# ViTAE-Transformer/MTP

Hardware: AMD Instinct MI355X
Metric: images/sec pretrain step (ViT-L+RVSA, 224^2, bf16) (higher is better)
Workload: dtype bf16; 1 GPU; ViT-L + RVSA backbone fwd+bwd + grad all-reduce + clip + AdamW, 224x224, batch 64 per GPU (BASELINE configs[2]/[3]); global_batch=64, parallelism=dp1, activation_checkpointing=False, heads=sum_i mean(f_i)

## Files before the change

### include/mtp_hip.h

```cpp
#ifndef MTP_HIP_H_
#define MTP_HIP_H_

#include <stddef.h>
#include <stdint.h>

#ifdef __cplusplus
extern "C" {
#endif

typedef void* mtp_stream_t;

typedef enum { MTP_F32 = 0, MTP_BF16 = 1, MTP_F64 = 2  } mtp_dtype;

enum { MTP_OK = 0, MTP_ERR_ARG = -1, MTP_ERR_UNSUPPORTED = -2 };

typedef enum {
    MTP_EPI_BIAS = 0,
    MTP_EPI_BIAS_GELU = 1,
    MTP_EPI_BIAS_RES = 2,
    MTP_EPI_DGELU = 3,
    MTP_EPI_BIAS_GELU_DG = 4,
    MTP_EPI_MUL = 5
} mtp_epilogue;

typedef enum {
    MTP_GEMM_NT_REG_STAGED = 1,
    MTP_GEMM_ORDER_SHIFT = 1,
    MTP_GEMM_ORDER_PLAIN = 1 << 1,
    MTP_GEMM_ORDER_GROUPED = 2 << 1,
    MTP_GEMM_ORDER_ROW_MAJOR = 3 << 1,
    MTP_GEMM_ORDER_MASK = 3 << 1,
    MTP_GEMM_TNG_PLAIN_ORDER = 1 << 1,
    MTP_GEMM_TN_REG_TRANSPOSE = 1 << 4,
    MTP_GEMM_NT_SB8 = 1 << 5,
    MTP_GEMM_NT_NO_SB8 = 1 << 6,
    MTP_GEMM_NT_P8 = 1 << 8,
    MTP_GEMM_NT_P8_224 = 2 << 8,
    MTP_GEMM_NT_P8_256 = 3 << 8,
    MTP_GEMM_NT_P8_MASK = 3 << 8,
    MTP_GEMM_NT_NO_P8 = 1 << 10,
    MTP_GEMM_NT_PERSIST = 1 << 15,
    MTP_GEMM_TN_TR_FULL_ONLY = 1 << 15,
    MTP_GEMM_NT_NO_PERSIST = 1 << 16,
    MTP_GEMM_NT_STRIP = 1 << 17,
    MTP_GEMM_NT_NO_STRIP = 1 << 18,
    MTP_GEMM_TNG_PLAIN_PHASES = 1 << 19,
    MTP_GEMM_STORE_SHIFT = 20,
    MTP_GEMM_STORE_NT = 1 << 20,
    MTP_GEMM_STORE_SC1 = 2 << 20,
    MTP_GEMM_STORE_PLAIN = 3 << 20,
    MTP_GEMM_STORE_MASK = 3 << 20
} mtp_gemm_variant;

typedef struct {
    const void* A;
    const void* B;
    void* C;
    int64_t M, N, K;
    int64_t lda, ldb, ldc;
    int in_dtype;
    int out_dtype;
    int epilogue;
    const float* bias;
    int64_t bias_mod;
    const float* res;
    int64_t res_ld, res_mod;
    const float* rowscale;
    int64_t rows_per_sample;
    void* aux;
    int64_t aux_ld;
    int split_k;
    int variant;
    float* colsum;
    int defer_sum;
    int pad_;
    void* workspace;
    int64_t workspace_bytes;
} mtp_gemm_args;

int mtp_gemm_nt(const mtp_gemm_args* args, mtp_stream_t stream);
typedef enum {
    MTP_GEMM_NT_FAMILY_SB = 0,
    MTP_GEMM_NT_FAMILY_SB8 = 1,
    MTP_GEMM_NT_FAMILY_REG = 2,
    MTP_GEMM_NT_FAMILY_P8 = 3,
    MTP_GEMM_NT_FAMILY_STRIP = 4
} mtp_gemm_nt_family;
struct mtp_gemm_nt_plan {
    int family;
    int tile_m;
    int order;
    int persistent;
    int store_policy;
};
int mtp_gemm_nt_plan(const mtp_gemm_args* args, int cus, struct mtp_gemm_nt_plan* out);
int mtp_gemm_nt_tile(const mtp_gemm_args* args);
int64_t mtp_gemm_nt_workspace_bytes(void);
int mtp_gemm_tn(const mtp_gemm_args* args, mtp_stream_t stream);
#define MTP_MAX_GROUPED_GEMMS 32
int mtp_gemm_tn_grouped(const mtp_gemm_args* args, int count, mtp_stream_t stream);
int mtp_sum_partials_batch(const float* const* parts, float* const* outs, const int64_t* numel, const int* splits, int count,
                           mtp_stream_t stream);

int mtp_layernorm_fwd(const void* x, int x_dtype, const float* gamma, const float* beta, void* y, int y_dtype,
                      float* mean, float* rstd, int64_t rows, int64_t C, float eps, int fuse_gelu, mtp_stream_t stream);
int64_t mtp_layernorm_bwd_partial_rows(int64_t rows);
int mtp_layernorm_bwd(const void* dy, int dy_dtype, const void* x, int x_dtype, const float* mean, const float* rstd,
                      const float* gamma, const float* beta, int fuse_gelu,
                      const float* dres, const float* extra, void* dx, int dx_dtype,
                      void* dx_copy, int copy_dtype, const float* copy_scale, int64_t rows_per_sample,
                      float* dgamma_part, float* dbeta_part, int64_t part_ld, int64_t rows, int64_t C, mtp_stream_t stream);
int mtp_layernorm_bwd_win(const void* dy, int dy_dtype, const void* x, int x_dtype, const float* mean, const float* rstd,
                          const float* gamma, const float* dres, const float* extra, void* dx, int dx_dtype,
                          void* dx_copy, int copy_dtype, const float* copy_scale, int64_t rows_per_sample,
                          float* dgamma_part, float* dbeta_part, int64_t part_ld, int64_t rows, int64_t C,
                          const float* win_add, int64_t B, int64_t Hp, int64_t Wp, mtp_stream_t stream);
int mtp_layernorm_residual_fwd(const void* h, int dtype, const float* gamma, const float* beta, const float* x, const float* layer_scale,
                               const float* sample_scale, int64_t rows_per_sample, float* out, void* out_act, float* mean, float* rstd,
                               int64_t rows, int64_t C, float eps, mtp_stream_t stream);
int mtp_layernorm_residual_bwd(const float* dout, const void* h, int dtype, const float* mean, const float* rstd, const float* gamma, const float* beta,
                               const float* layer_scale, const float* sample_scale, int64_t rows_per_sample, void* dh, float* part,
                               int64_t rows, int64_t C, mtp_stream_t stream);
int mtp_reduce_rows_f32(const float* part, int64_t ld, float* out, int64_t rows, int64_t C, int accumulate, mtp_stream_t stream);
#define MTP_REDUCE_BATCH_MAX 32
int mtp_reduce_rows_batched_f32(const float* const* parts, float* const* outs, int n, int64_t ld, int64_t rows, int64_t C, int accumulate,
                                mtp_stream_t stream);
int mtp_reduce_rows_t_f32(const float* part, int64_t ld, float* out, int64_t rows, int64_t R, int64_t C, int accumulate, mtp_stream_t stream);
int mtp_reduce_rows_t_batched_f32(const float* const* parts, float* const* outs, int n, int64_t ld, int64_t rows, int64_t R, int64_t C, int accumulate,
                                  mtp_stream_t stream);
int mtp_colsum(const void* dY, int dtype, int64_t ld, float* out, int64_t M, int64_t N, mtp_stream_t stream);
int mtp_colsum_acc(const void* dY, int dtype, int64_t ld, float* out, int64_t M, int64_t N, mtp_stream_t stream);

int mtp_patchify(const float* img, void* cols, int dtype, int64_t B, int64_t Cin, int64_t H, int64_t W, int64_t P, mtp_stream_t stream);
int mtp_unpatchify(const void* cols, int dtype, float* dimg, int64_t B, int64_t Cin, int64_t H, int64_t W, int64_t P, mtp_stream_t stream);
int mtp_preprocess_patchify(const uint8_t* img, void* cols, int dtype, int64_t B, int64_t H, int64_t W, int64_t P, int64_t pad_divisor,
                            const float* mean, const float* std, int bgr_to_rgb, float pad_value, mtp_stream_t stream);
int mtp_cast(const void* src, int src_dtype, void* dst, int dst_dtype, int64_t n, mtp_stream_t stream);
int mtp_transpose_cast(const float* src, void* dst, int dst_dtype, int64_t R, int64_t C, mtp_stream_t stream);
typedef struct {
    const float* src;
    void* w;
    void* wt;
    int64_t R, C;
    int64_t tile0;
    int32_t f32_out;
    float wd;
} mtp_wimg_desc;
int mtp_weight_images(const mtp_wimg_desc* descs_dev, int n, int64_t total_tiles, int act_dtype, mtp_stream_t stream);
int mtp_adamw_weight_images(const mtp_wimg_desc* descs_dev, int n, int64_t total_tiles, int act_dtype, float* p_base, const float* g_base, float* m_base, float* v_base,
                            const float* hyper, const float* sqnorm, float max_norm, float grad_scale, mtp_stream_t stream);
int mtp_adamw_weight_images_lr(const mtp_wimg_desc* descs_dev, const float* desc_lr, int n, int64_t total_tiles, int act_dtype, float* p_base, const float* g_base,
                               float* m_base, float* v_base, const float* hyper, const float* sqnorm, float max_norm, float grad_scale, mtp_stream_t stream);
int mtp_convt_pack(const float* w, void* wg, void* wgT, int dtype, int64_t Cin, int64_t Cout, mtp_stream_t stream);
int mtp_convt_unpack_grad(const float* dwg, float* dw, int64_t Cin, int64_t Cout, mtp_stream_t stream);
int mtp_tokens_to_nchw(const void* x, int x_dtype, void* out, int out_dtype, int64_t B, int64_t Hp, int64_t Wp, int64_t C, int levels, mtp_stream_t stream);
int mtp_nchw_to_tokens(const void* f, int f_dtype, void* out, int out_dtype, int64_t B, int64_t Hp, int64_t Wp, int64_t C, int levels, mtp_stream_t stream);
int mtp_maxpool2_tokens_fwd(const float* x, void* y, int y_dtype, int64_t B, int64_t Hp, int64_t Wp, int64_t C, mtp_stream_t stream);
int mtp_maxpool2_tokens_bwd(const float* x, const void* dy, int dy_dtype, float* dx, int accumulate, int64_t B, int64_t Hp, int64_t Wp, int64_t C, mtp_stream_t stream);
int mtp_axpy_f32(float* y, const float* x, float alpha, int64_t n, mtp_stream_t stream);
#define MTP_MAX_SEGMENTS 12
int mtp_copy_segments_f32(const float* const* src, float* const* dst, const int64_t* count, int n, mtp_stream_t stream);
int mtp_scale_rows_cast(const float* src, void* dst, int dst_dtype, const float* scale, int64_t rows_per_sample, int64_t rows, int64_t C, mtp_stream_t stream);

int mtp_im2col3x3(const void* x, int x_dtype, int64_t sN, int64_t sH, int64_t sW, int64_t sC, void* cols, int cols_dtype,
                  int64_t N, int64_t H, int64_t W, int64_t Cin, int64_t stride, int64_t Kp, mtp_stream_t stream);
int mtp_col2im3x3(const void* dcols, int cols_dtype, float* dx, int64_t sN, int64_t sH, int64_t sW, int64_t sC,
                  int64_t N, int64_t H, int64_t W, int64_t Cin, int64_t stride, int64_t Kp, int accumulate, mtp_stream_t stream);
int mtp_conv3x3_pack(const float* w, void* w2, void* w2t, int dtype, int64_t Cout, int64_t Cin, int64_t Kp, mtp_stream_t stream);
int mtp_conv3x3_unpack_grad(const float* dw2, float* dw, int64_t Cout, int64_t Cin, int64_t Kp, mtp_stream_t stream);
int mtp_pack_rows_padded(const float* w, void* wp, void* wpt, int dtype, int64_t R, int64_t C, int64_t Rp, mtp_stream_t stream);
int mtp_cast_pad_rows(const float* src, int64_t n, void* dst, int dst_dtype, int64_t ld, int64_t rows, mtp_stream_t stream);
int mtp_copy_rows(const void* src, int64_t src_ld, void* dst, int64_t dst_ld, int dtype, int64_t n, int64_t rows, mtp_stream_t stream);
int mtp_dwconv3x3_fwd(const void* x, const float* w, const float* bias, void* y, int dtype, int64_t N, int64_t H, int64_t W, int64_t C, mtp_stream_t stream);
int mtp_dwconv3x3_bwd_dx(const void* dy, int dtype, const float* w, float* dx, int accumulate, int64_t N, int64_t H, int64_t W, int64_t C, mtp_stream_t stream);
int64_t mtp_dwconv3x3_bwd_dw_partial_rows(int64_t N, int64_t H, int64_t W);
int mtp_dwconv3x3_bwd_dw(const void* dy, const void* x, int dtype, float* part, int64_t N, int64_t H, int64_t W, int64_t C, mtp_stream_t stream);
typedef enum { MTP_CONV_OP_IM2COL3X3 = 0, MTP_CONV_OP_COL2IM3X3 = 1, MTP_CONV_OP_DWCONV3X3_FWD = 2, MTP_CONV_OP_DWCONV3X3_BWD_DX = 3, MTP_CONV_OP_DWCONV3X3_BWD_DW = 4 } mtp_conv_op;
typedef enum {
    MTP_CONV_KERNEL_NONE = 0,
    MTP_CONV_KERNEL_ELEMENT = 1,
    MTP_CONV_KERNEL_V8 = 2,
    MTP_CONV_KERNEL_P8 = 3,
    MTP_CONV_KERNEL_PX4 = 4
} mtp_conv_kernel_family;
int mtp_conv_kernel(int op, const void* src, int src_dtype, int64_t sN, int64_t sH, int64_t sW, int64_t sC, const void* dst, int dst_dtype,
                    const float* w, const float* bias, int64_t N, int64_t H, int64_t W, int64_t C, int64_t stride, int64_t Kp);
int mtp_dwconv_fwd(const void* x, const float* w, const float* bias, void* y, int dtype, int64_t N, int64_t H, int64_t W, int64_t C, int k, mtp_stream_t stream);
int mtp_dwconv_bwd_dx(const void* dy, int dtype, const float* w, float* dx, int accumulate, int64_t N, int64_t H, int64_t W, int64_t C, int k, mtp_stream_t stream);
int mtp_dwconv_bwd_dw(const void* dy, const void* x, int dtype, float* dw, float* db, int64_t N, int64_t H, int64_t W, int64_t C, int k, mtp_stream_t stream);
int mtp_center_feature_scale_fwd(const void* y, const void* xp, const void* logits, int64_t ld, void* out, int dtype, int64_t rows, int64_t G, int64_t GC, mtp_stream_t stream);
int mtp_center_feature_scale_bwd(const void* dout, const void* y, const void* xp, const void* logits, int64_t ld, void* dy, float* dxp, void* dlogits, int dtype, int64_t rows,
                                 int64_t G, int64_t GC, mtp_stream_t stream);
int mtp_softmax_groups_fwd(const void* logits, int64_t ld, void* prob, int dtype, int64_t rows, int64_t G, int64_t P, mtp_stream_t stream);
int mtp_softmax_groups_bwd(const void* prob, const float* dprob, void* dlogits, int64_t ld, int dtype, int64_t rows, int64_t G, int64_t P, mtp_stream_t stream);
int mtp_scale_residual_fwd(const float* x, const void* z, int dtype, const float* gamma, const float* sample_scale, int64_t rows_per_sample,
                           float* out, void* out_act, int64_t rows, int64_t C, mtp_stream_t stream);
int64_t mtp_scale_residual_bwd_partial_rows(int64_t rows);
int mtp_scale_residual_bwd(const float* dout, const void* z, int dtype, const float* gamma, const float* sample_scale, int64_t rows_per_sample,
                           void* dz, float* part, int64_t rows, int64_t C, mtp_stream_t stream);

int mtp_full_attn_fwd(const void* qkv, void* o, float* lse, int dtype, const float* rel_h, const float* rel_w,
                      int64_t B, int64_t Hp, int64_t Wp, int64_t heads, int64_t hd, float scale, mtp_stream_t stream);
int64_t mtp_full_attn_bwd_workspace_floats(int64_t B, int64_t Hp, int64_t Wp, int64_t heads);
int mtp_full_attn_bwd(const void* qkv, const void* o, const void* dout, const float* lse, void* dqkv, int dtype,
                      const float* rel_h, const float* rel_w, float* drel_part, float* workspace,
                      int64_t B, int64_t Hp, int64_t Wp, int64_t heads, int64_t hd, float scale, mtp_stream_t stream);

enum {
    MTP_ATTN_KERNEL_NONE = 0,
    MTP_FULL_FWD_V3 = 1,
    MTP_FULL_FWD_FLASH128 = 3,
    MTP_FULL_FWD_FLASH256 = 4,
    MTP_FULL_FWD_GENERIC = 5,
    MTP_FULL_BWD_V3 = 1,
    MTP_FULL_BWD_FLASH = 3,
    MTP_FULL_BWD_THREE_PASS = 4,
    MTP_FULL_BWD_SINGLE_WG = 5,
    MTP_RVSA_FWD_GENERIC = 1,
    MTP_RVSA_FWD_MFMA = 2,
    MTP_RVSA_BWD_GENERIC = 1,
    MTP_RVSA_BWD_MFMA_DENSE = 2,
    MTP_RVSA_BWD_MFMA_ATOMIC = 3
};
int mtp_full_attn_kernel(int dtype, int64_t Hp, int64_t Wp, int backward);
int mtp_rvsa_attn_kernel(int dtype, int64_t Hp, int64_t Wp, int64_t heads, int backward);

int mtp_rvsa_pool_fwd(const void* x, int dtype, float* avg, float* pooled, int64_t B, int64_t Hp, int64_t Wp, int64_t C, mtp_stream_t stream);
int mtp_rvsa_pool_bwd(const float* dpooled, const float* avg, void* dx, int dtype, int accumulate, int64_t B, int64_t Hp, int64_t Wp, int64_t C, mtp_stream_t stream);
int mtp_rvsa_sampling_fwd(const void* x, int dtype, const float* w, const float* bias, float* avg, float* pooled, float* samp,
                          int64_t B, int64_t Hp, int64_t Wp, int64_t C, int64_t N, mtp_stream_t stream);
int mtp_rvsa_sampling_bwd(const float* dsamp, const float* w, const float* avg, void* dx, int dtype,
                          int64_t B, int64_t Hp, int64_t Wp, int64_t C, int64_t N, mtp_stream_t stream);
int mtp_rvsa_sampling_bwd_win(const float* dsamp, const float* w, const float* avg, float* g, int64_t windows, int64_t C, int64_t N, mtp_stream_t stream);
int mtp_small_linear_fwd(const float* x, const float* w, const float* b, float* y, int64_t R, int64_t N, int64_t K, mtp_stream_t stream);
int mtp_small_linear_bwd(const float* x, const float* w, const float* dy, float* dx, float* dw, float* db, int64_t R, int64_t N, int64_t K, mtp_stream_t stream);
int mtp_small_linear_dw_segments(const float* x, const float* dy, int64_t R, int64_t N, int64_t K, int nseg, const int64_t* seg_rows,
                                 float* const* dw, float* const* db, mtp_stream_t stream);
int mtp_small_linear_dw_segments_batched(const float* const* xs, const float* const* dys, int count, int64_t R, int64_t N, int64_t K, int nseg,
                                         const int64_t* seg_rows, float* const* dw, float* const* db, mtp_stream_t stream);
int mtp_rvsa_attn_fwd(const void* qkv, const float* samp, void* o, float* lse, int dtype,
                      const float* rel_h, const float* rel_w, const float* bias_table,
                      int64_t B, int64_t Hp, int64_t Wp, int64_t heads, int64_t hd, float scale, mtp_stream_t stream);
int mtp_rvsa_attn_bwd(const void* qkv, const float* samp, const void* o, const void* dout, const float* lse,
                      void* dqkv, float* dkv_f32, float* dsamp, float* rel_part, float* tab_part, int dtype,
                      const float* rel_h, const float* rel_w, const float* bias_table,
                      int64_t B, int64_t Hp, int64_t Wp, int64_t heads, int64_t hd, float scale, mtp_stream_t stream);

int mtp_zero_segments_f32(float* base, const int64_t* start, const int64_t* count, int n, mtp_stream_t stream);
int mtp_sqnorm_f32(const float* g, float* out, int64_t n, mtp_stream_t stream);
int mtp_sqnorm_segments_f32(const float* base, const int64_t* start, const int64_t* count, int n, float* out, mtp_stream_t stream);
int mtp_adamw_flat(float* p, const float* g, float* m, float* v, int64_t n, const int64_t* seg_start, const float* seg_wd, int nseg,
                   const float* hyper, const float* sqnorm, float max_norm, float grad_scale, mtp_stream_t stream);
int mtp_adamw_flat_lr(float* p, const float* g, float* m, float* v, int64_t n, const int64_t* seg_start, const float* seg_wd, const float* seg_lr, int nseg,
                      const float* hyper, const float* sqnorm, float max_norm, float grad_scale, mtp_stream_t stream);

typedef struct {
    int64_t N, H, W;
    int kernel_h, kernel_w, stride_h, stride_w, pad_h, pad_w, dilation_h, dilation_w;
    int group, group_channels;
    float offset_scale;
    int im2col_step;
    int remove_center;
    int variant;
} mtp_dcnv3_geom;
int mtp_dcnv3_out_size(const mtp_dcnv3_geom* geom, int64_t* Ho, int64_t* Wo);
int mtp_dcnv3_fwd(const void* input, const void* offset, const void* mask, void* output, int dtype, const mtp_dcnv3_geom* geom, mtp_stream_t stream);
int mtp_dcnv3_bwd(const void* input, const void* offset, const void* mask, const void* grad_output, int dtype, float* grad_input, float* grad_offset,
                  float* grad_mask, const mtp_dcnv3_geom* geom, mtp_stream_t stream);
int mtp_dcnv3_bwd_act(const void* input, const void* offset, const void* mask, const void* grad_output, int dtype, float* grad_input, float* grad_offset,
                      float* grad_mask, void* grad_offset_act, int64_t act_ld, const mtp_dcnv3_geom* geom, mtp_stream_t stream);

typedef enum {
    MTP_DCNV3_KERNEL_NONE = 0,
    MTP_DCNV3_FWD9 = 1,
    MTP_DCNV3_FWD_VEC8 = 2,
    MTP_DCNV3_FWD_SCALAR = 3,
    MTP_DCNV3_F64 = 4,
    MTP_DCNV3_BWD_WINDOW_R2 = 5,
    MTP_DCNV3_BWD_WINDOW_R3 = 6,
    MTP_DCNV3_BWD_3X3_OS1 = 7,
    MTP_DCNV3_BWD_3X3_OS2 = 8,
    MTP_DCNV3_BWD_SCATTER_SHFL = 9,
    MTP_DCNV3_BWD_SCATTER_ATOMIC = 10
} mtp_dcnv3_kernel_family;
int mtp_dcnv3_kernel(const void* input, const void* offset, const void* mask, const void* out, const float* grad_input, const float* grad_offset,
                     const float* grad_mask, int dtype, const mtp_dcnv3_geom* geom, int backward);

const char* mtp_version(void);

int mtp_stream_create_low_priority(mtp_stream_t* stream);
int mtp_stream_create_cu_mask(const uint32_t* mask, int words, mtp_stream_t* stream);
int mtp_probe_placement(int32_t* out, int blocks, int64_t spin_clocks, mtp_stream_t stream);
int mtp_stream_destroy(mtp_stream_t stream);

int mtp_comm_unique_id(void* id128);
int mtp_comm_init(const void* id128, int rank, int world, void** comm);
int mtp_comm_allreduce_bucket(void* comm, float* bucket, int64_t count, mtp_stream_t stream);
int mtp_comm_allreduce_bucket_dt(void* comm, void* bucket, int64_t count, int dtype, mtp_stream_t stream);
int mtp_comm_reduce_scatter_bucket(void* comm, void* bucket, int64_t count_per_rank, int rank, int dtype, mtp_stream_t stream);
int mtp_comm_allgather_bucket(void* comm, void* bucket, int64_t count_per_rank, int rank, int dtype, mtp_stream_t stream);
int mtp_comm_info(void* comm, int* info4);
int mtp_comm_destroy(void* comm);

int64_t mtp_bn_partial_rows(int64_t rows);
int mtp_bn_stats(const void* x, int dtype, int64_t ldx, const float* center, float* part, float* sums, int64_t rows, int64_t C, mtp_stream_t stream);
int mtp_bn_finalize(const float* sums, const float* center, double count, float* running_mean, float* running_var, float momentum, float eps, float* mean, float* rstd,
                    int64_t C, mtp_stream_t stream);
int mtp_bn_apply(const void* x, int x_dtype, int64_t ldx, const float* mean, const float* rstd, const float* gamma, const float* beta, int relu,
                 void* y, int y_dtype, int64_t ldy, int64_t rows, int64_t C, mtp_stream_t stream);
int mtp_bn_bwd_stats(const void* dy, int dy_dtype, int64_t lddy, const void* x, int x_dtype, int64_t ldx, const float* mean, const float* rstd,
                     const float* gamma, const float* beta, int relu, float* part, float* sums, int64_t rows, int64_t C, mtp_stream_t stream);
int mtp_bn_bwd_dx(const void* dy, int dy_dtype, int64_t lddy, const void* x, int x_dtype, int64_t ldx, const float* mean, const float* rstd,
                  const float* gamma, const float* beta, int relu, const float* sums, double count, void* dx, int dx_dtype, int64_t lddx,
                  int64_t rows, int64_t C, mtp_stream_t stream);
int mtp_resize_bilinear_fwd(const void* x, int x_dtype, int64_t ldx, void* y, int y_dtype, int64_t ldy, int64_t N, int64_t Hi, int64_t Wi,
                            int64_t Ho, int64_t Wo, int64_t C, int accumulate, mtp_stream_t stream);
int mtp_resize_bilinear_bwd(const void* dy, int dy_dtype, int64_t lddy, float* dx, int64_t lddx, int64_t N, int64_t Hi, int64_t Wi, int64_t Ho,
                            int64_t Wo, int64_t C, int accumulate, mtp_stream_t stream);
int mtp_adaptive_avg_pool_fwd(const void* x, int x_dtype, int64_t ldx, void* y, int y_dtype, int64_t N, int64_t H, int64_t W, int64_t C,
                              int64_t S, mtp_stream_t stream);
int mtp_adaptive_avg_pool_bwd(const void* dy, int dy_dtype, float* dx, int64_t lddx, int64_t N, int64_t H, int64_t W, int64_t C, int64_t S,
                              int accumulate, mtp_stream_t stream);
int mtp_channel_scale(const void* x, int x_dtype, int64_t ldx, const float* mask, int64_t rows_per_sample, void* y, int y_dtype, int64_t ldy,
                      int64_t rows, int64_t C, mtp_stream_t stream);
int64_t mtp_seg_ce_workspace_bytes(int64_t N, int64_t H, int64_t W, int64_t K);
int mtp_seg_ce(const void* logits, int dtype, int64_t ld, int64_t N, int64_t h, int64_t w, int64_t K, const void* labels, int label_bytes, int64_t H,
               int64_t W, int ignore_index, float loss_weight, float* loss, float* dlogits, int64_t ldd, void* workspace, int64_t workspace_bytes,
               mtp_stream_t stream);

int mtp_seg_window_accumulate(const void* logits, int dtype, int64_t ld, int64_t N, int64_t h, int64_t w, int64_t K, float* acc, int64_t lda,
                              int64_t H, int64_t W, int64_t y1, int64_t x1, int64_t Hc, int64_t Wc, mtp_stream_t stream);
int mtp_seg_argmax_areas(float* acc, int64_t lda, int64_t N, int64_t H, int64_t W, int64_t K, const int32_t* cy, const int32_t* cx, int write_back,
                         uint8_t* pred, float* seg_logits, const void* labels, int label_bytes, int ignore_index, int64_t* areas, mtp_stream_t stream);
int mtp_seg_areas(const void* pred, int pred_bytes, const void* labels, int label_bytes, int64_t pixels, int64_t K, int ignore_index, int64_t* areas,
                  mtp_stream_t stream);

typedef enum { MTP_FUSE_CONCAT = 0, MTP_FUSE_SUM = 1, MTP_FUSE_DIFF = 2, MTP_FUSE_ABS_DIFF = 3 } mtp_fuse_policy;
int mtp_fuse_pair_fwd(const void* f, int f_dtype, void* out, int out_dtype, int64_t ld, int64_t N, int64_t C, int64_t H, int64_t W, int policy,
                      mtp_stream_t stream);
int mtp_fuse_pair_bwd(const float* g, int64_t ldg, const void* f, int f_dtype, float* df, int64_t N, int64_t C, int64_t H, int64_t W, int policy,
                      mtp_stream_t stream);
int mtp_unet_up_cat_fwd(const void* x, int64_t ldx, int64_t Cx, const void* skip, int64_t lds, int64_t Cs, int in_dtype, void* y, int y_dtype, int64_t ldy,
                        int64_t N, int64_t h, int64_t w, int64_t hs, int64_t ws, mtp_stream_t stream);
int mtp_unet_up_cat_bwd(const float* dy, int64_t lddy, float* dx, int64_t lddx, int64_t Cx, float* dskip, int64_t ldds, int64_t Cs, int64_t N, int64_t h,
                        int64_t w, int64_t hs, int64_t ws, int accumulate, mtp_stream_t stream);

int mtp_gap_fwd(const void* x, int dtype, float* pooled, int64_t N, int64_t C, int64_t HW, mtp_stream_t stream);
int mtp_gap_bwd(const float* dpooled, void* dx, int dtype, int64_t N, int64_t C, int64_t HW, mtp_stream_t stream);
int mtp_cls_ce(const float* pooled, const float* w, const float* b, const int64_t* labels, float loss_weight, float* logits, float* prob,
               int64_t* pred, float* loss_rows, float* loss, float* dlogits, uint32_t* counter, int64_t N, int64_t C, int64_t K, mtp_stream_t stream);
int mtp_cls_head_bwd(const float* dlogits, const float* pooled, const float* w, float* dw, float* db, float* dpooled, int64_t N, int64_t C, int64_t K,
                     int accumulate, mtp_stream_t stream);
int mtp_cls_hits(const float* scores, const int64_t* labels, int64_t N, int64_t K, const int32_t* topk, int nk, float thr, int use_thr,
                 int64_t* counters, mtp_stream_t stream);

typedef enum { MTP_BOX_ALIGNED = 0 , MTP_BOX_ROTATED = 1  } mtp_box_kind;
typedef enum {
    MTP_ASSIGN_BOX = 0,
    MTP_ASSIGN_RBOX2HBOX = 1,
    MTP_ASSIGN_ROTATED = 2
} mtp_assign_calculator;
int mtp_box_iou(const float* boxes1, const float* boxes2, float* out, int64_t M, int64_t N, int kind, int iof, int aligned, float eps,
                mtp_stream_t stream);
int mtp_nms_mask(const float* boxes, const int64_t* groups, int64_t n, int kind, float iou_threshold, void* mask, int64_t mask_bytes,
                 mtp_stream_t stream);
int mtp_nms_scan(const void* mask, int64_t n, int64_t max_keep, int64_t* keep, int64_t* count, mtp_stream_t stream);
int mtp_max_iou_assign(const float* gts, const float* priors, const int64_t* gt_labels, int64_t K, int64_t N, int calculator, float pos_iou_thr,
                       float neg_iou_lo, float neg_iou_hi, float min_pos_iou, int match_low_quality, int gt_max_assign_all, int64_t* gt_inds,
                       float* max_overlaps, int64_t* labels, void* workspace, int64_t workspace_bytes, mtp_stream_t stream);

#ifdef __cplusplus
}
#endif
#endif
```

### mtp_amd/__init__.py

```python
import os as _os

_HWQ_BEFORE_IMPORT = _os.environ.get("GPU_MAX_HW_QUEUES")
_os.environ.setdefault("GPU_MAX_HW_QUEUES", "8")


def _hip_already_initialised():
    try:
        import torch as _torch
        return bool(_torch.cuda.is_initialized())
    except Exception:
        return False


_HIP_INIT_BEFORE_IMPORT = _hip_already_initialised()
_warned_hwq = False


def hw_queue_note():
    global _warned_hwq
    if _warned_hwq:
        return None
    val = _os.environ.get("GPU_MAX_HW_QUEUES")
    note = None
    if _HIP_INIT_BEFORE_IMPORT and _HWQ_BEFORE_IMPORT is None:
        note = ("HIP was initialised before `import mtp_amd`: GPU_MAX_HW_QUEUES=8 could not take effect, the weight-gradient side stream may share the "
                "compute stream's hardware queue (no overlap, nothing wrong); import mtp_amd or set GPU_MAX_HW_QUEUES=8 before the first CUDA call")
    elif val is not None and val.isdigit() and int(val) < 8:
        note = ("GPU_MAX_HW_QUEUES=%s (set by the environment): with fewer than 8 hardware queues the weight-gradient side stream may share the compute "
                "stream's queue next to the gradient exchange (no overlap, nothing wrong)" % val)
    _warned_hwq = True
    return note

from .backbone import (InternImage, internimage_xl, RVSA_MTP, RVSA_MTP_branches, RVSA_MTP_det, RVSA_MTP_taps, ViT_Win_RVSA_V3_WSZ7, vit_b_rvsa, vit_l_rvsa,
                       window_partition, window_reverse)
from .registry import BACKBONES, MODELS, TASK_UTILS, build_backbone
from .decode_heads import UNetHead, UPerHead
from .necks import FeatureFusionNeck, GlobalAveragePooling
from .cls_heads import LinearClsHead
from .classifiers import ImageClassifier
from .segmentors import EncoderDecoder, SiamEncoderDecoder
from .evaluation import Accuracy, IoUMetric
from .ops_box import batched_nms, bbox_overlaps, box_iou_rotated, nms, nms_rotated
from .task_modules import AssignResult, BboxOverlaps2D, MTP_RD_MaxIoUAssigner, MaxIoUAssigner, RBbox2HBboxOverlaps2D, RBboxOverlaps2D

__version__ = "0.6.0"
```

### mtp_amd/_lib.py

```python
import ctypes as C
import os

_HERE = os.path.dirname(os.path.abspath(__file__))
LIB_PATH = os.environ.get("MTP_HIP_LIB") or os.path.join(_HERE, "libmtp_hip.so")

MTP_F32, MTP_BF16, MTP_F64 = 0, 1, 2
EPI_BIAS, EPI_BIAS_GELU, EPI_BIAS_RES, EPI_DGELU, EPI_BIAS_GELU_DG, EPI_MUL = 0, 1, 2, 3, 4, 5

GEMM_NT_REG_STAGED = 1
GEMM_ORDER_SHIFT, GEMM_ORDER_PLAIN, GEMM_ORDER_GROUPED, GEMM_ORDER_ROW_MAJOR, GEMM_ORDER_MASK = 1, 1 << 1, 2 << 1, 3 << 1, 3 << 1
GEMM_TNG_PLAIN_ORDER = 1 << 1
GEMM_TN_REG_TRANSPOSE = 1 << 4
GEMM_NT_SB8, GEMM_NT_NO_SB8 = 1 << 5, 1 << 6
GEMM_NT_P8, GEMM_NT_P8_224, GEMM_NT_P8_256, GEMM_NT_P8_MASK, GEMM_NT_NO_P8 = 1 << 8, 2 << 8, 3 << 8, 3 << 8, 1 << 10
GEMM_NT_PERSIST, GEMM_TN_TR_FULL_ONLY, GEMM_NT_NO_PERSIST = 1 << 15, 1 << 15, 1 << 16
GEMM_NT_STRIP, GEMM_NT_NO_STRIP = 1 << 17, 1 << 18
GEMM_TNG_PLAIN_PHASES = 1 << 19
GEMM_STORE_SHIFT, GEMM_STORE_NT, GEMM_STORE_SC1, GEMM_STORE_PLAIN, GEMM_STORE_MASK = 20, 1 << 20, 2 << 20, 3 << 20, 3 << 20
GEMM_NT_FAMILY_SB, GEMM_NT_FAMILY_SB8, GEMM_NT_FAMILY_REG, GEMM_NT_FAMILY_P8, GEMM_NT_FAMILY_STRIP = 0, 1, 2, 3, 4

CONV_OP_IM2COL3X3, CONV_OP_COL2IM3X3, CONV_OP_DWCONV3X3_FWD, CONV_OP_DWCONV3X3_BWD_DX, CONV_OP_DWCONV3X3_BWD_DW = 0, 1, 2, 3, 4
CONV_KERNEL_NONE, CONV_KERNEL_ELEMENT, CONV_KERNEL_V8, CONV_KERNEL_P8, CONV_KERNEL_PX4 = 0, 1, 2, 3, 4
DCNV3_KERNEL_NONE, DCNV3_FWD9, DCNV3_FWD_VEC8, DCNV3_FWD_SCALAR, DCNV3_F64 = 0, 1, 2, 3, 4
DCNV3_BWD_WINDOW_R2, DCNV3_BWD_WINDOW_R3, DCNV3_BWD_3X3_OS1, DCNV3_BWD_3X3_OS2, DCNV3_BWD_SCATTER_SHFL, DCNV3_BWD_SCATTER_ATOMIC = 5, 6, 7, 8, 9, 10

BOX_ALIGNED, BOX_ROTATED = 0, 1
ASSIGN_BOX, ASSIGN_RBOX2HBOX, ASSIGN_ROTATED = 0, 1, 2

FUSE_CONCAT, FUSE_SUM, FUSE_DIFF, FUSE_ABS_DIFF = 0, 1, 2, 3

p, i64, i32, f32 = C.c_void_p, C.c_int64, C.c_int, C.c_float


class GemmArgs(C.Structure):
    _fields_ = [("A", p), ("B", p), ("C", p), ("M", i64), ("N", i64), ("K", i64),
                ("lda", i64), ("ldb", i64), ("ldc", i64),
                ("in_dtype", i32), ("out_dtype", i32), ("epilogue", i32),
                ("bias", p), ("bias_mod", i64), ("res", p), ("res_ld", i64), ("res_mod", i64),
                ("rowscale", p), ("rows_per_sample", i64), ("aux", p), ("aux_ld", i64),
                ("split_k", i32), ("variant", i32), ("colsum", p), ("defer_sum", i32), ("pad_", i32),
                ("workspace", p), ("workspace_bytes", i64)]


class GemmNtPlan(C.Structure):
    _fields_ = [("family", i32), ("tile_m", i32), ("order", i32), ("persistent", i32), ("store_policy", i32)]


class WimgDesc(C.Structure):
    _fields_ = [("src", p), ("w", p), ("wt", p), ("R", i64), ("C", i64), ("tile0", i64), ("f32_out", C.c_int32), ("wd", C.c_float)]


class Dcnv3Geom(C.Structure):
    _fields_ = [("N", i64), ("H", i64), ("W", i64), ("kernel_h", C.c_int32), ("kernel_w", C.c_int32), ("stride_h", C.c_int32), ("stride_w", C.c_int32),
                ("pad_h", C.c_int32), ("pad_w", C.c_int32), ("dilation_h", C.c_int32), ("dilation_w", C.c_int32), ("group", C.c_int32),
                ("group_channels", C.c_int32), ("offset_scale", C.c_float), ("im2col_step", C.c_int32), ("remove_center", C.c_int32), ("variant", C.c_int32)]


SIGNATURES = {
    "mtp_weight_images": (i32, [p, i32, i64, i32, p]),
    "mtp_dwconv_fwd": (i32, [p, p, p, p, i32, i64, i64, i64, i64, i32, p]),
    "mtp_dwconv_bwd_dx": (i32, [p, i32, p, p, i32, i64, i64, i64, i64, i32, p]),
    "mtp_dwconv_bwd_dw": (i32, [p, p, i32, p, p, i64, i64, i64, i64, i32, p]),
    "mtp_center_feature_scale_fwd": (i32, [p, p, p, i64, p, i32, i64, i64, i64, p]),
    "mtp_center_feature_scale_bwd": (i32, [p, p, p, p, i64, p, p, p, i32, i64, i64, i64, p]),
    "mtp_dcnv3_out_size": (i32, [C.POINTER(Dcnv3Geom), C.POINTER(i64), C.POINTER(i64)]),
    "mtp_dcnv3_fwd": (i32, [p, p, p, p, i32, C.POINTER(Dcnv3Geom), p]),
    "mtp_dcnv3_bwd": (i32, [p, p, p, p, i32, p, p, p, C.POINTER(Dcnv3Geom), p]),
    "mtp_dcnv3_bwd_act": (i32, [p, p, p, p, i32, p, p, p, p, i64, C.POINTER(Dcnv3Geom), p]),
    "mtp_dcnv3_kernel": (i32, [p, p, p, p, p, p, p, i32, C.POINTER(Dcnv3Geom), i32]),
    "mtp_conv_kernel": (i32, [i32, p, i32, i64, i64, i64, i64, p, i32, p, p, i64, i64, i64, i64, i64, i64]),
    "mtp_gemm_nt": (i32, [C.POINTER(GemmArgs), p]),
    "mtp_gemm_nt_plan": (i32, [C.POINTER(GemmArgs), i32, C.POINTER(GemmNtPlan)]),
    "mtp_gemm_nt_tile": (i32, [C.POINTER(GemmArgs)]),
    "mtp_gemm_nt_workspace_bytes": (i64, []),
    "mtp_gemm_tn": (i32, [C.POINTER(GemmArgs), p]),
    "mtp_gemm_tn_grouped": (i32, [C.POINTER(GemmArgs), i32, p]),
    "mtp_sum_partials_batch": (i32, [p, p, p, p, i32, p]),
    "mtp_layernorm_fwd": (i32, [p, i32, p, p, p, i32, p, p, i64, i64, f32, i32, p]),
    "mtp_layernorm_bwd_partial_rows": (i64, [i64]),
    "mtp_layernorm_bwd": (i32, [p, i32, p, i32, p, p, p, p, i32, p, p, p, i32, p, i32, p, i64, p, p, i64, i64, i64, p]),
    "mtp_reduce_rows_f32": (i32, [p, i64, p, i64, i64, i32, p]),
    "mtp_reduce_rows_batched_f32": (i32, [p, p, i32, i64, i64, i64, i32, p]),
    "mtp_reduce_rows_t_f32": (i32, [p, i64, p, i64, i64, i64, i32, p]),
    "mtp_reduce_rows_t_batched_f32": (i32, [p, p, i32, i64, i64, i64, i64, i32, p]),
    "mtp_copy_segments_f32": (i32, [p, p, p, i32, p]),
    "mtp_colsum": (i32, [p, i32, i64, p, i64, i64, p]),
    "mtp_colsum_acc": (i32, [p, i32, i64, p, i64, i64, p]),
    "mtp_patchify": (i32, [p, p, i32, i64, i64, i64, i64, i64, p]),
    "mtp_preprocess_patchify": (i32, [p, p, i32, i64, i64, i64, i64, i64, C.POINTER(f32), C.POINTER(f32), i32, f32, p]),
    "mtp_unpatchify": (i32, [p, i32, p, i64, i64, i64, i64, i64, p]),
    "mtp_cast": (i32, [p, i32, p, i32, i64, p]),
    "mtp_transpose_cast": (i32, [p, p, i32, i64, i64, p]),
    "mtp_convt_pack": (i32, [p, p, p, i32, i64, i64, p]),
    "mtp_convt_unpack_grad": (i32, [p, p, i64, i64, p]),
    "mtp_tokens_to_nchw": (i32, [p, i32, p, i32, i64, i64, i64, i64, i32, p]),
    "mtp_nchw_to_tokens": (i32, [p, i32, p, i32, i64, i64, i64, i64, i32, p]),
    "mtp_maxpool2_tokens_fwd": (i32, [p, p, i32, i64, i64, i64, i64, p]),
    "mtp_maxpool2_tokens_bwd": (i32, [p, p, i32, p, i32, i64, i64, i64, i64, p]),
    "mtp_axpy_f32": (i32, [p, p, f32, i64, p]),
    "mtp_scale_rows_cast": (i32, [p, p, i32, p, i64, i64, i64, p]),
    "mtp_im2col3x3": (i32, [p, i32, i64, i64, i64, i64, p, i32, i64, i64, i64, i64, i64, i64, p]),
    "mtp_col2im3x3": (i32, [p, i32, p, i64, i64, i64, i64, i64, i64, i64, i64, i64, i64, i32, p]),
    "mtp_conv3x3_pack": (i32, [p, p, p, i32, i64, i64, i64, p]),
    "mtp_conv3x3_unpack_grad": (i32, [p, p, i64, i64, i64, p]),
    "mtp_pack_rows_padded": (i32, [p, p, p, i32, i64, i64, i64, p]),
    "mtp_cast_pad_rows": (i32, [p, i64, p, i32, i64, i64, p]),
    "mtp_copy_rows": (i32, [p, i64, p, i64, i32, i64, i64, p]),
    "mtp_dwconv3x3_fwd": (i32, [p, p, p, p, i32, i64, i64, i64, i64, p]),
    "mtp_dwconv3x3_bwd_dx": (i32, [p, i32, p, p, i32, i64, i64, i64, i64, p]),
    "mtp_dwconv3x3_bwd_dw_partial_rows": (i64, [i64, i64, i64]),
    "mtp_dwconv3x3_bwd_dw": (i32, [p, p, i32, p, i64, i64, i64, i64, p]),
    "mtp_softmax_groups_fwd": (i32, [p, i64, p, i32, i64, i64, i64, p]),
    "mtp_softmax_groups_bwd": (i32, [p, p, p, i64, i32, i64, i64, i64, p]),
    "mtp_scale_residual_fwd": (i32, [p, p, i32, p, p, i64, p, p, i64, i64, p]),
    "mtp_scale_residual_bwd_partial_rows": (i64, [i64]),
    "mtp_scale_residual_bwd": (i32, [p, p, i32, p, p, i64, p, p, i64, i64, p]),
    "mtp_comm_unique_id": (i32, [p]),
    "mtp_comm_init": (i32, [p, i32, i32, C.POINTER(C.c_void_p)]),
    "mtp_comm_allreduce_bucket": (i32, [p, p, i64, p]),
    "mtp_comm_allreduce_bucket_dt": (i32, [p, p, i64, i32, p]),
    "mtp_comm_reduce_scatter_bucket": (i32, [p, p, i64, i32, i32, p]),
    "mtp_comm_allgather_bucket": (i32, [p, p, i64, i32, i32, p]),
    "mtp_comm_info": (i32, [p, p]),
    "mtp_comm_destroy": (i32, [p]),
    "mtp_full_attn_fwd": (i32, [p, p, p, i32, p, p, i64, i64, i64, i64, i64, f32, p]),
    "mtp_full_attn_bwd_workspace_floats": (i64, [i64, i64, i64, i64]),
    "mtp_full_attn_bwd": (i32, [p, p, p, p, p, i32, p, p, p, p, i64, i64, i64, i64, i64, f32, p]),
    "mtp_full_attn_kernel": (i32, [i32, i64, i64, i32]),
    "mtp_rvsa_attn_kernel": (i32, [i32, i64, i64, i64, i32]),
    "mtp_rvsa_pool_fwd": (i32, [p, i32, p, p, i64, i64, i64, i64, p]),
    "mtp_rvsa_pool_bwd": (i32, [p, p, p, i32, i32, i64, i64, i64, i64, p]),
    "mtp_rvsa_sampling_fwd": (i32, [p, i32, p, p, p, p, p, i64, i64, i64, i64, i64, p]),
    "mtp_rvsa_sampling_bwd": (i32, [p, p, p, p, i32, i64, i64, i64, i64, i64, p]),
    "mtp_rvsa_sampling_bwd_win": (i32, [p, p, p, p, i64, i64, i64, p]),
    "mtp_layernorm_residual_fwd": (i32, [p, i32, p, p, p, p, p, i64, p, p, p, p, i64, i64, f32, p]),
    "mtp_layernorm_residual_bwd": (i32, [p, p, i32, p, p, p, p, p, p, i64, p, p, i64, i64, p]),
    "mtp_layernorm_bwd_win": (i32, [p, i32, p, i32, p, p, p, p, p, p, i32, p, i32, p, i64, p, p, i64, i64, i64, p, i64, i64, i64, p]),
    "mtp_small_linear_fwd": (i32, [p, p, p, p, i64, i64, i64, p]),
    "mtp_small_linear_bwd": (i32, [p, p, p, p, p, p, i64, i64, i64, p]),
    "mtp_small_linear_dw_segments": (i32, [p, p, i64, i64, i64, i32, p, p, p, p]),
    "mtp_small_linear_dw_segments_batched": (i32, [p, p, i32, i64, i64, i64, i32, p, p, p, p]),
    "mtp_rvsa_attn_fwd": (i32, [p, p, p, p, i32, p, p, p, i64, i64, i64, i64, i64, f32, p]),
    "mtp_rvsa_attn_bwd": (i32, [p, p, p, p, p, p, p, p, p, p, i32, p, p, p, i64, i64, i64, i64, i64, f32, p]),
    "mtp_zero_segments_f32": (i32, [p, p, p, i32, p]),
    "mtp_sqnorm_f32": (i32, [p, p, i64, p]),
    "mtp_sqnorm_segments_f32": (i32, [p, p, p, i32, p, p]),
    "mtp_adamw_flat": (i32, [p, p, p, p, i64, p, p, i32, p, p, f32, f32, p]),
    "mtp_adamw_weight_images": (i32, [p, i32, i64, i32, p, p, p, p, p, p, f32, f32, p]),
    "mtp_adamw_flat_lr": (i32, [p, p, p, p, i64, p, p, p, i32, p, p, f32, f32, p]),
    "mtp_adamw_weight_images_lr": (i32, [p, p, i32, i64, i32, p, p, p, p, p, p, f32, f32, p]),
    "mtp_bn_partial_rows": (i64, [i64]),
    "mtp_bn_stats": (i32, [p, i32, i64, p, p, p, i64, i64, p]),
    "mtp_bn_finalize": (i32, [p, p, C.c_double, p, p, f32, f32, p, p, i64, p]),
    "mtp_bn_apply": (i32, [p, i32, i64, p, p, p, p, i32, p, i32, i64, i64, i64, p]),
    "mtp_bn_bwd_stats": (i32, [p, i32, i64, p, i32, i64, p, p, p, p, i32, p, p, i64, i64, p]),
    "mtp_bn_bwd_dx": (i32, [p, i32, i64, p, i32, i64, p, p, p, p, i32, p, C.c_double, p, i32, i64, i64, i64, p]),
    "mtp_resize_bilinear_fwd": (i32, [p, i32, i64, p, i32, i64, i64, i64, i64, i64, i64, i64, i32, p]),
    "mtp_resize_bilinear_bwd": (i32, [p, i32, i64, p, i64, i64, i64, i64, i64, i64, i64, i32, p]),
    "mtp_adaptive_avg_pool_fwd": (i32, [p, i32, i64, p, i32, i64, i64, i64, i64, i64, p]),
    "mtp_adaptive_avg_pool_bwd": (i32, [p, i32, p, i64, i64, i64, i64, i64, i64, i32, p]),
    "mtp_channel_scale": (i32, [p, i32, i64, p, i64, p, i32, i64, i64, i64, p]),
    "mtp_seg_ce_workspace_bytes": (i64, [i64, i64, i64, i64]),
    "mtp_seg_ce": (i32, [p, i32, i64, i64, i64, i64, i64, p, i32, i64, i64, i32, f32, p, p, i64, p, i64, p]),
    "mtp_seg_window_accumulate": (i32, [p, i32, i64, i64, i64, i64, i64, p, i64, i64, i64, i64, i64, i64, i64, p]),
    "mtp_seg_argmax_areas": (i32, [p, i64, i64, i64, i64, i64, p, p, i32, p, p, p, i32, i32, p, p]),
    "mtp_seg_areas": (i32, [p, i32, p, i32, i64, i64, i32, p, p]),
    "mtp_fuse_pair_fwd": (i32, [p, i32, p, i32, i64, i64, i64, i64, i64, i32, p]),
    "mtp_fuse_pair_bwd": (i32, [p, i64, p, i32, p, i64, i64, i64, i64, i32, p]),
    "mtp_unet_up_cat_fwd": (i32, [p, i64, i64, p, i64, i64, i32, p, i32, i64, i64, i64, i64, i64, i64, p]),
    "mtp_unet_up_cat_bwd": (i32, [p, i64, p, i64, i64, p, i64, i64, i64, i64, i64, i64, i64, i32, p]),
    "mtp_gap_fwd": (i32, [p, i32, p, i64, i64, i64, p]),
    "mtp_gap_bwd": (i32, [p, p, i32, i64, i64, i64, p]),
    "mtp_cls_ce": (i32, [p, p, p, p, f32, p, p, p, p, p, p, p, i64, i64, i64, p]),
    "mtp_cls_head_bwd": (i32, [p, p, p, p, p, p, i64, i64, i64, i32, p]),
    "mtp_cls_hits": (i32, [p, p, i64, i64, C.POINTER(C.c_int32), i32, f32, i32, p, p]),
    "mtp_box_iou": (i32, [p, p, p, i64, i64, i32, i32, i32, f32, p]),
    "mtp_nms_mask": (i32, [p, p, i64, i32, f32, p, i64, p]),
    "mtp_nms_scan": (i32, [p, i64, i64, p, p, p]),
    "mtp_max_iou_assign": (i32, [p, p, p, i64, i64, i32, f32, f32, f32, f32, i32, i32, p, p, p, p, i64, p]),
    "mtp_version": (C.c_char_p, []),
    "mtp_stream_create_low_priority": (i32, [p]),
    "mtp_stream_create_cu_mask": (i32, [p, i32, p]),
    "mtp_probe_placement": (i32, [p, i32, i64, p]),
    "mtp_stream_destroy": (i32, [p]),
}

_lib = None


class MtpHipError(RuntimeError):
    pass


def load():
    global _lib
    if _lib is not None:
        return _lib
    if not os.path.exists(LIB_PATH):
        raise MtpHipError("libmtp_hip.so not found at %s -- build it first (__graft_entry__.build() or make -C mtp_amd/csrc); "
                          "mtp_amd has no CPU/PyTorch fallback" % LIB_PATH)
    lib = C.CDLL(LIB_PATH)
    ab = bool(os.environ.get("MTP_HIP_LIB"))
    for name, (res, args) in SIGNATURES.items():
        if ab and not hasattr(lib, name):
            continue
        fn = getattr(lib, name)
        fn.restype = res
        fn.argtypes = args
    _lib = lib
    return lib


def check(rc, what):
    if rc != 0:
        kind = {-1: "invalid argument", -2: "unsupported configuration"}.get(rc, "hipError_t %d" % rc)
        raise MtpHipError("%s failed: %s" % (what, kind))
```

### mtp_amd/csrc/gemm.hip

```cpp
#include "gemm_common.h"

namespace {

constexpr int BM = 128;
constexpr int BN = 128;
constexpr int NT_THREADS = 256;
constexpr int ROW_BYTES = 128;
constexpr int OPER_BYTES = BM * ROW_BYTES;
constexpr int STAGE_BYTES = 2 * OPER_BYTES;
constexpr int LDS_BYTES = 2 * STAGE_BYTES;

__device__ __forceinline__ int lds_off(int row, int chunk) { return row * ROW_BYTES + ((chunk ^ (row & 7)) << 4); }

__global__ __launch_bounds__(256) void sum_partials_kernel(const float* __restrict__ part, float* __restrict__ out, int64_t n4, int split) {
    for (int64_t i = (int64_t)blockIdx.x * 256 + threadIdx.x; i < n4; i += (int64_t)gridDim.x * 256) {
        float4 s = *reinterpret_cast<const float4*>(part + 4 * i);
        for (int z = 1; z < split; ++z) {
            const float4 v = *reinterpret_cast<const float4*>(part + 4 * (i + (int64_t)z * n4));
            s.x += v.x; s.y += v.y; s.z += v.z; s.w += v.w;
        }
        *reinterpret_cast<float4*>(out + 4 * i) = s;
    }
}

// ... 320 lines not shown
        __builtin_amdgcn_sched_barrier(0);
        compute_stage<T>(cur, cur + OPER_BYTES, acc, wm, wn, lane);
        __builtin_amdgcn_sched_barrier(0);
        store_tn_regs<T>(r, nxt, tid);
    }
    epilogue<float, MTP_EPI_BIAS, 4>(p, acc, m0 + wm * 64, n0 + wn * 64, lane);
}

typedef short tr_v4s __attribute__((ext_vector_type(4)));
constexpr int TR_ROW_BYTES = 256;

__device__ __forceinline__ void stage_tn_glds(const KArgs& p, char* sA, char* sB, int m0, int n0, int kt, int wave, int lane) {
#pragma unroll
    for (int i = 0; i < 4; ++i) {
        const int rbase = wave * 16 + i * 4;
        const int row = rbase + (lane >> 4);
        const int f = (row & 3) | ((row >> 1) & 4);
        const int chunk = (lane & 15) ^ (f << 1);
        const int64_t t = (int64_t)kt * 64 + row;
        int ca = m0 + chunk * 8, cb = n0 + chunk * 8;
        ca = ca < p.M - 8 ? ca : p.M - 8;
        cb = cb < p.N - 8 ? cb : p.N - 8;
        const char* ga = p.A + (t * p.lda + ca) * 2;
        const char* gb = p.B + (t * p.ldb + cb) * 2;
        __builtin_amdgcn_global_load_lds((const __attribute__((address_space(1))) void*)ga,
                                         (__attribute__((address_space(3))) void*)(sA + rbase * TR_ROW_BYTES), 16, 0, 0);
        __builtin_amdgcn_global_load_lds((const __attribute__((address_space(1))) void*)gb,
                                         (__attribute__((address_space(3))) void*)(sB + rbase * TR_ROW_BYTES), 16, 0, 0);
    }
}

__device__ __forceinline__ uint4 tr_frag(const char* s, int off) {
    const tr_v4s lo = __builtin_amdgcn_ds_read_tr16_b64_v4i16((__attribute__((address_space(3))) tr_v4s*)(s + off));
    const tr_v4s hi = __builtin_amdgcn_ds_read_tr16_b64_v4i16((__attribute__((address_space(3))) tr_v4s*)(s + off + 4 * TR_ROW_BYTES));
    const uint2 l = __builtin_bit_cast(uint2, lo), h = __builtin_bit_cast(uint2, hi);
    return make_uint4(l.x, l.y, h.x, h.y);
}

__device__ __forceinline__ void compute_stage_tr(const char* sA, const char* sB, f32x4_t (&acc)[4][4], int wm, int wn, int lane) {
    const int i = lane & 15, g = lane >> 4;
    const int f = (i >> 2) | ((g & 1) << 2);
    const int rowoff = (8 * g + (i >> 2)) * TR_ROW_BYTES + ((i >> 1) & 1) * 16 + (i & 1) * 8;
#pragma unroll
    for (int ks = 0; ks < 2; ++ks) {
        uint4 a[4], b[4];
#pragma unroll
        for (int q = 0; q < 4; ++q) {
            a[q] = tr_frag(sA, rowoff + (((q | (wm << 2)) ^ f) << 5) + ks * 32 * TR_ROW_BYTES);
            b[q] = tr_frag(sB, rowoff + (((q | (wn << 2)) ^ f) << 5) + ks * 32 * TR_ROW_BYTES);
        }
#pragma unroll
        for (int ni = 0; ni < 4; ++ni)
#pragma unroll
            for (int mi = 0; mi < 4; ++mi) Mma<bf16_t>::run(acc[ni][mi], b[ni], a[mi]);
    }
}

__global__ __launch_bounds__(NT_THREADS) __attribute__((amdgpu_waves_per_eu(4, 4))) void gemm_tn_tr_kernel(KArgs p) {
    extern __shared__ __attribute__((aligned(16))) char smem[];
    const int tid = threadIdx.x, lane = tid & 63, wave = __builtin_amdgcn_readfirstlane(tid >> 6);
    const int wm = wave >> 1, wn = wave & 1;
    const int tile = (p.order & 1) ? (int)blockIdx.x : xcd_remap(blockIdx.x, gridDim.x);
    const int tiles_m = (int)gridDim.x / p.tiles_n;
    const int m0 = ((p.order & 2) ? tile % tiles_m : tile / p.tiles_n) * BM, n0 = ((p.order & 2) ? tile / tiles_m : tile % p.tiles_n) * BN;
    const int kt0 = blockIdx.y * p.k_tiles_per_split;
    int kt1 = kt0 + p.k_tiles_per_split;
    kt1 = kt1 < p.k_tiles ? kt1 : p.k_tiles;
    if (kt0 >= kt1) return;
    p.C += (int64_t)blockIdx.y * p.split_stride * (int64_t)sizeof(float);
    f32x4_t acc[4][4];
#pragma unroll
    for (int i = 0; i < 4; ++i)
#pragma unroll
        for (int j = 0; j < 4; ++j) acc[i][j] = f32x4_t{0.f, 0.f, 0.f, 0.f};
    const bool do_colsum = p.colsum != nullptr && n0 == 0;
    float cs[8] = {0.f, 0.f, 0.f, 0.f, 0.f, 0.f, 0.f, 0.f};
    for (int kt = kt0; kt < kt1; ++kt) {
        stage_tn_glds(p, smem, smem + OPER_BYTES, m0, n0, kt, wave, lane);
        asm volatile("s_waitcnt vmcnt(0)" ::: "memory");
        __syncthreads();
        compute_stage_tr(smem, smem + OPER_BYTES, acc, wm, wn, lane);
        if (do_colsum) {
#pragma unroll
            for (int j = 0; j < 4; ++j) {
                const uint4 v = *reinterpret_cast<const uint4*>(smem + ((tid >> 4) + 16 * j) * TR_ROW_BYTES + (tid & 15) * 16);
                const uint32_t w[4] = {v.x, v.y, v.z, v.w};
#pragma unroll
                for (int e = 0; e < 4; ++e) {
                    cs[2 * e] += __uint_as_float(w[e] << 16);
                    cs[2 * e + 1] += __uint_as_float(w[e] & 0xffff0000u);
                }
            }
        }
        __syncthreads();
    }
    if (do_colsum) {
        float* red = reinterpret_cast<float*>(smem);
        const int rg = tid >> 4, f = (rg & 3) | ((rg >> 1) & 4), chunk = (tid & 15) ^ (f << 1);
        *reinterpret_cast<float4*>(red + rg * BM + chunk * 8) = make_float4(cs[0], cs[1], cs[2], cs[3]);
        *reinterpret_cast<float4*>(red + rg * BM + chunk * 8 + 4) = make_float4(cs[4], cs[5], cs[6], cs[7]);
        __syncthreads();
        if (tid < BM) {
            float s = 0.f;
#pragma unroll
            for (int r = 0; r < 16; ++r) s += red[r * BM + tid];
            if (m0 + tid < p.M) atomicAdd(p.colsum + m0 + tid, s);
        }
    }
    epilogue<float, MTP_EPI_BIAS, 4>(p, acc, m0 + wm * 64, n0 + wn * 64, lane);
}

template <typename T>
int fill_common(const mtp_gemm_args* a, KArgs& k) {
    constexpr int E = Elem<T>::kPerChunk;
    if (!a->A || !a->B || !a->C || a->M <= 0 || a->N <= 0 || a->K <= 0) return MTP_ERR_ARG;
    if (a->M > INT32_MAX || a->N > INT32_MAX || a->K > INT32_MAX) return MTP_ERR_ARG;
    if ((a->lda % E) || (a->ldb % E) || (a->ldc % 4) || (a->N % 4)) return MTP_ERR_ARG;
    if (((uintptr_t)a->A | (uintptr_t)a->B | (uintptr_t)a->C) & 15) return MTP_ERR_ARG;
    k.A = (const char*)a->A; k.B = (const char*)a->B; k.C = (char*)a->C;
    k.M = (int)a->M; k.N = (int)a->N; k.K = (int)a->K;
    k.lda = a->lda; k.ldb = a->ldb; k.ldc = a->ldc;
    k.bias = a->bias; k.bias_mod = (int)a->bias_mod;
    k.res = a->res; k.res_ld = a->res_ld; k.res_mod = (int)a->res_mod;
    k.rowscale = a->rowscale; k.rows_per_sample = (int)(a->rows_per_sample > 0 ? a->rows_per_sample : 1);
    k.aux = (char*)a->aux; k.aux_ld = a->aux_ld;
    k.tiles_n = (int)((a->N + BN - 1) / BN);
    k.k_tiles = (int)((a->K + 8 * E - 1) / (8 * E));
    k.k_tiles_per_split = k.k_tiles;
    k.atomic_out = 0;
    k.order = 0;
    k.split_stride = 0;
    k.colsum = nullptr;
    return 0;
}

NtPlan nt_plan(const mtp_gemm_args* a, const KArgs& k, int cus) {
    const int ord = (a->variant & MTP_GEMM_ORDER_MASK) >> MTP_GEMM_ORDER_SHIFT;
    const int p8_forced = (a->variant & MTP_GEMM_NT_P8_MASK) / MTP_GEMM_NT_P8;
    const int sp_forced = (a->variant & MTP_GEMM_STORE_MASK) >> MTP_GEMM_STORE_SHIFT;
    const bool reg_staged = a->variant & MTP_GEMM_NT_REG_STAGED, sb8_force = a->variant & MTP_GEMM_NT_SB8, sb8_forbid = a->variant & MTP_GEMM_NT_NO_SB8;
    const bool p8_forbid = a->variant & MTP_GEMM_NT_NO_P8, persist_force = a->variant & MTP_GEMM_NT_PERSIST, persist_forbid = a->variant & MTP_GEMM_NT_NO_PERSIST;
    const bool s8_force = a->variant & MTP_GEMM_NT_STRIP, s8_forbid = a->variant & MTP_GEMM_NT_NO_STRIP;

    const bool bf16 = a->in_dtype == MTP_BF16;
    const int64_t tiles = ((a->M + 255) / 256) * ((a->N + 255) / 256) * 256 / cus;
    NtPlan p = {MTP_GEMM_NT_FAMILY_SB, BM, 0, 0, MTP_GEMM_STORE_PLAIN >> MTP_GEMM_STORE_SHIFT};

    if (bf16 && !p8_forbid && !s8_forbid && !p8_forced && mtp_nt_s8_fits(k, a->out_dtype, a->epilogue) && (s8_force || (tiles >= 40 && tiles <= 128))) {
        p.family = MTP_GEMM_NT_FAMILY_STRIP;
        p.order = ord == 1;
        p.persistent = 1;
        p.store_policy = mtp_nt_s8_store_policy(a->out_dtype);
        return p;
    }
    if (bf16 && !p8_forbid && mtp_nt_p8_fits(k, a->out_dtype, a->epilogue) && (p8_forced || tiles >= 72 || (tiles >= 40 && a->K >= 1536))) {
        p.family = MTP_GEMM_NT_FAMILY_P8;
        p.tile_m = p8_forced == 2 ? 224 : p8_forced == 3 ? 256 : mtp_nt_p8_pick_tile_m(k.M, k.N, cus);
        p.order = ord == 1;
        p.persistent = persist_force || (!persist_forbid && p.tile_m == 224 && mtp_nt_p8_tiles(k.M, k.N, p.tile_m) > cus);
        const int sp = sp_forced ? sp_forced : (a->epilogue == MTP_EPI_BIAS_RES ? 2 : 1);
        if (p.tile_m == 224) p.store_policy = sp;
        return p;
    }
    if (reg_staged || a->K % (8 * (bf16 ? 8 : 4))) {
        p.family = MTP_GEMM_NT_FAMILY_REG;
        p.order = ord;
        return p;
    }
    p.order = ord == 0 ? (k.tiles_n > 8 ? 2 : 0) : ord == 1 ? 1 : ord == 2 ? 2 : 0;
    const int tiles8 = ((k.M + NT8_BM - 1) / NT8_BM) * k.tiles_n;
    if (sb8_force || (tiles8 >= 256 && tiles8 <= 512 && !sb8_forbid)) {
        p.family = MTP_GEMM_NT_FAMILY_SB8;
        p.tile_m = NT8_BM;
    }
    return p;
}

template <typename T, typename Tout, int EPI>
int launch_nt(const mtp_gemm_args* a, hipStream_t stream) {
    constexpr int E = Elem<T>::kPerChunk;
    KArgs k;
    int rc = fill_common<T>(a, k);
    if (rc) return rc;
    if (a->K % E) return MTP_ERR_ARG;
    if (EPI == MTP_EPI_BIAS_RES && (!a->res || (a->res_ld % 4))) return MTP_ERR_ARG;
    if ((EPI == MTP_EPI_BIAS_GELU || EPI == MTP_EPI_DGELU || EPI == MTP_EPI_BIAS_GELU_DG || EPI == MTP_EPI_MUL) && (!a->aux || (a->aux_ld % 4))) return MTP_ERR_ARG;
    if (a->bias && a->bias_mod > 0 && (a->bias_mod % 4)) return MTP_ERR_ARG;
    const NtPlan plan = nt_plan(a, k, mtp_stream_cus(stream));
    k.order = plan.order;
    const int tiles = (k.M + plan.tile_m - 1) / plan.tile_m * k.tiles_n;
    switch (plan.family) {
        case MTP_GEMM_NT_FAMILY_STRIP: return mtp_nt_s8_launch(k, a->out_dtype, EPI, plan.order, stream);
        case MTP_GEMM_NT_FAMILY_P8: return mtp_nt_p8_launch(k, a->out_dtype, EPI, plan, stream);
        case MTP_GEMM_NT_FAMILY_SB8: hipLaunchKernelGGL((gemm_nt_sb8_kernel<T, Tout, EPI>), dim3(tiles), dim3(NT8_THREADS), NT8_STAGE_BYTES, stream, k); break;
        case MTP_GEMM_NT_FAMILY_REG: hipLaunchKernelGGL((gemm_nt_kernel<T, Tout, EPI>), dim3(tiles), dim3(NT_THREADS), LDS_BYTES, stream, k); break;
        default: hipLaunchKernelGGL((gemm_nt_sb_kernel<T, Tout, EPI>), dim3(tiles), dim3(NT_THREADS), STAGE_BYTES, stream, k);
    }
    return mtp_launch_status();
}

template <typename T>
int launch_tn(const mtp_gemm_args* a, hipStream_t stream) {
    constexpr int E = Elem<T>::kPerChunk;
    KArgs k;
    int rc = fill_common<T>(a, k);
    if (rc) return rc;
    if (a->out_dtype != MTP_F32 || (a->M % E) || (a->N % E)) return MTP_ERR_ARG;
    const int ord = (a->variant & MTP_GEMM_ORDER_MASK) >> MTP_GEMM_ORDER_SHIFT;
    const bool reg_transpose = a->variant & MTP_GEMM_TN_REG_TRANSPOSE, tr_full_only = a->variant & MTP_GEMM_TN_TR_FULL_ONLY;
    k.bias = nullptr;
    int split = a->split_k > 1 ? a->split_k : 1;
    if (split > k.k_tiles) split = k.k_tiles;
    k.k_tiles_per_split = (k.k_tiles + split - 1) / split;
    split = (k.k_tiles + k.k_tiles_per_split - 1) / k.k_tiles_per_split;
    const bool use_ws = split > 1 && a->aux != nullptr;
    k.atomic_out = split > 1 && !use_ws;
    k.split_stride = 0;
    if (split > 1) {
        if (a->ldc != a->N) return MTP_ERR_ARG;
        if (use_ws) {
            if ((uintptr_t)a->aux & 15) return MTP_ERR_ARG;
            k.C = (char*)a->aux;
            k.split_stride = (int64_t)a->M * a->N;
        } else {
            hipError_t e = hipMemsetAsync(a->C, 0, sizeof(float) * (size_t)a->M * (size_t)a->N, stream);
            if (e != hipSuccess) return (int)e;
        }
    }
    const int tiles_m = (k.M + BM - 1) / BM;
    dim3 grid(tiles_m * k.tiles_n, split), block(NT_THREADS);
    const bool full = (a->K % (8 * E) == 0) && (a->M % BM == 0) && (a->N % BN == 0);
    const bool tr = sizeof(T) == 2 && !reg_transpose && (full || ((a->K % 64 == 0) && (a->M % 8 == 0) && (a->N % 8 == 0) && a->M >= 8 && a->N >= 8 && !tr_full_only));
    k.order = ord;
    if (a->colsum && !tr) {
        rc = mtp_colsum_acc(a->A, a->in_dtype, a->lda, a->colsum, a->K, a->M, stream);
        if (rc) return rc;
    }
    if (tr) {
        k.colsum = a->colsum;
        k.order = ord == 0 ? (a->N > a->M ? 2 : 0) : ord == 1 ? 1 : ord == 2 ? 2 : 0;
        hipLaunchKernelGGL(gemm_tn_tr_kernel, grid, block, STAGE_BYTES, stream, k);
    } else if (full)
        hipLaunchKernelGGL((gemm_tn_kernel<T, true>), grid, block, LDS_BYTES, stream, k);
    else
        hipLaunchKernelGGL((gemm_tn_kernel<T, false>), grid, block, LDS_BYTES, stream, k);
    if (use_ws && !a->defer_sum) {
        const int64_t n4 = (int64_t)a->M * a->N / 4;
        int64_t nb = (n4 + 255) / 256;
        hipLaunchKernelGGL(sum_partials_kernel, dim3((unsigned)(nb > 4096 ? 4096 : nb)), dim3(256), 0, stream, (const float*)a->aux, (float*)a->C, n4, split);
    }
    return mtp_launch_status();
}

struct SumJobs {
    const float* part[MTP_MAX_SEGMENTS];
    float* out[MTP_MAX_SEGMENTS];
    int64_t n4[MTP_MAX_SEGMENTS];
    int split[MTP_MAX_SEGMENTS];
};
__global__ __launch_bounds__(256) void sum_partials_batch_kernel(SumJobs t) {
    const int j = blockIdx.y;
    const float* __restrict__ part = t.part[j];
    float* __restrict__ out = t.out[j];
    const int64_t n4 = t.n4[j];
    const int split = t.split[j];
    for (int64_t i = (int64_t)blockIdx.x * 256 + threadIdx.x; i < n4; i += (int64_t)gridDim.x * 256) {
        float4 s = *reinterpret_cast<const float4*>(part + 4 * i);
        for (int z = 1; z < split; ++z) {
            const float4 v = *reinterpret_cast<const float4*>(part + 4 * (i + (int64_t)z * n4));
            s.x += v.x; s.y += v.y; s.z += v.z; s.w += v.w;
        }
        *reinterpret_cast<float4*>(out + 4 * i) = s;
    }
}

template <typename T, typename Tout>
int dispatch_epi(const mtp_gemm_args* a, hipStream_t s) {
    switch (a->epilogue) {
        case MTP_EPI_BIAS: return launch_nt<T, Tout, MTP_EPI_BIAS>(a, s);
        case MTP_EPI_BIAS_GELU: return launch_nt<T, Tout, MTP_EPI_BIAS_GELU>(a, s);
        case MTP_EPI_DGELU: return launch_nt<T, Tout, MTP_EPI_DGELU>(a, s);
        case MTP_EPI_BIAS_GELU_DG: return launch_nt<T, Tout, MTP_EPI_BIAS_GELU_DG>(a, s);
        case MTP_EPI_MUL: return launch_nt<T, Tout, MTP_EPI_MUL>(a, s);
        default: return MTP_ERR_UNSUPPORTED;
    }
}

}

extern "C" int mtp_gemm_nt(const mtp_gemm_args* a, mtp_stream_t stream) {
    if (!a) return MTP_ERR_ARG;
    hipStream_t s = (hipStream_t)stream;
    if (a->epilogue == MTP_EPI_BIAS_RES) {
        if (a->out_dtype != MTP_F32) return MTP_ERR_ARG;
        return a->in_dtype == MTP_BF16 ? launch_nt<bf16_t, float, MTP_EPI_BIAS_RES>(a, s)
                                      : launch_nt<float, float, MTP_EPI_BIAS_RES>(a, s);
    }
    if (a->in_dtype == MTP_BF16 && a->out_dtype == MTP_BF16) return dispatch_epi<bf16_t, bf16_t>(a, s);
    if (a->in_dtype == MTP_F32 && a->out_dtype == MTP_F32) return dispatch_epi<float, float>(a, s);
    if (a->in_dtype == MTP_BF16 && a->out_dtype == MTP_F32 && a->epilogue == MTP_EPI_BIAS) return launch_nt<bf16_t, float, MTP_EPI_BIAS>(a, s);
    return MTP_ERR_UNSUPPORTED;
}

extern "C" int64_t mtp_gemm_nt_workspace_bytes(void) { return 0; }

extern "C" int mtp_gemm_nt_plan(const mtp_gemm_args* a, int cus, struct mtp_gemm_nt_plan* out) {
    if (!a || !out) return MTP_ERR_ARG;
    KArgs k;
    if (a->in_dtype == MTP_BF16 ? fill_common<bf16_t>(a, k) : fill_common<float>(a, k)) return MTP_ERR_ARG;
    *out = nt_plan(a, k, cus > 0 ? cus : mtp_stream_cus(nullptr));
    return 0;
}

extern "C" int mtp_gemm_nt_tile(const mtp_gemm_args* a) {
    NtPlan p;
    if (const int rc = mtp_gemm_nt_plan(a, 0, &p)) return rc;
    return p.family == MTP_GEMM_NT_FAMILY_P8 ? 256 : p.family == MTP_GEMM_NT_FAMILY_STRIP ? 64 : 128;
}

extern "C" int mtp_sum_partials_batch(const float* const* parts, float* const* outs, const int64_t* numel, const int* splits, int count, mtp_stream_t stream) {
    if (!parts || !outs || !numel || !splits || count <= 0 || count > MTP_MAX_SEGMENTS) return MTP_ERR_ARG;
    SumJobs t;
    int64_t mx = 0;
    for (int i = 0; i < count; ++i) {
        if (!parts[i] || !outs[i] || numel[i] <= 0 || (numel[i] % 4) || splits[i] < 1) return MTP_ERR_ARG;
        t.part[i] = parts[i]; t.out[i] = outs[i]; t.n4[i] = numel[i] / 4; t.split[i] = splits[i];
        mx = t.n4[i] > mx ? t.n4[i] : mx;
    }
    int64_t nb = (mx + 255) / 256;
    hipLaunchKernelGGL(sum_partials_batch_kernel, dim3((unsigned)(nb > 2048 ? 2048 : nb), (unsigned)count), dim3(256), 0, (hipStream_t)stream, t);
    return mtp_launch_status();
}

extern "C" int mtp_gemm_tn(const mtp_gemm_args* a, mtp_stream_t stream) {
    if (!a) return MTP_ERR_ARG;
    hipStream_t s = (hipStream_t)stream;
    return a->in_dtype == MTP_BF16 ? launch_tn<bf16_t>(a, s) : launch_tn<float>(a, s);
}
```

### mtp_amd/csrc/gemm_common.h

```cpp
#pragma once
#include "common.h"

struct KArgs {
    const char* A;
    const char* B;
    char* C;
    int M, N, K;
    int64_t lda, ldb, ldc;
    const float* bias;
    int bias_mod;
    const float* res;
    int64_t res_ld;
    int res_mod;
    const float* rowscale;
    int rows_per_sample;
    char* aux;
    int64_t aux_ld;
    int tiles_n;
    int k_tiles;
    int k_tiles_per_split;
    int atomic_out;
    int order;
    int64_t split_stride;
    float* colsum;
};

typedef struct mtp_gemm_nt_plan NtPlan;

int mtp_nt_p8_launch(const KArgs& k, int out_dtype, int epilogue, const NtPlan& plan, hipStream_t stream);
int mtp_nt_p8_fits(const KArgs& k, int out_dtype, int epilogue);
int mtp_nt_p8_tiles(int64_t M, int64_t N, int tile_m);
int mtp_nt_p8_pick_tile_m(int64_t M, int64_t N, int64_t cus);
int mtp_nt_s8_launch(const KArgs& k, int out_dtype, int epilogue, int order, hipStream_t stream);
int mtp_nt_s8_fits(const KArgs& k, int out_dtype, int epilogue);
int mtp_nt_s8_store_policy(int out_dtype);

namespace {

template <typename T>
struct Mma;
template <>
struct Mma<bf16_t> {
    __device__ static __forceinline__ void run(f32x4_t& acc, const uint4& a, const uint4& b) {
        acc = __builtin_amdgcn_mfma_f32_16x16x32_bf16(__builtin_bit_cast(bf16x8_t, a), __builtin_bit_cast(bf16x8_t, b), acc, 0, 0, 0);
    }
};
template <>
struct Mma<float> {
    __device__ static __forceinline__ void run(f32x4_t& acc, const uint4& a, const uint4& b) {
        acc = __builtin_amdgcn_mfma_f32_16x16x4f32(__uint_as_float(a.x), __uint_as_float(b.x), acc, 0, 0, 0);
        acc = __builtin_amdgcn_mfma_f32_16x16x4f32(__uint_as_float(a.y), __uint_as_float(b.y), acc, 0, 0, 0);
        acc = __builtin_amdgcn_mfma_f32_16x16x4f32(__uint_as_float(a.z), __uint_as_float(b.z), acc, 0, 0, 0);
        acc = __builtin_amdgcn_mfma_f32_16x16x4f32(__uint_as_float(a.w), __uint_as_float(b.w), acc, 0, 0, 0);
    }
};

__device__ __attribute__((aligned(16))) const uint4 g_zero16 = {0u, 0u, 0u, 0u};

__device__ __forceinline__ int xcd_remap(int bid, int nb) {
    int xcd = bid & 7, idx = bid >> 3, q = nb >> 3, r = nb & 7;
    return (xcd < r ? xcd * (q + 1) : r * (q + 1) + (xcd - r) * q) + idx;
}


template <typename Tout, int EPI, int MF>
__device__ __forceinline__ void epilogue(const KArgs& p, f32x4_t (&acc)[4][MF], int mrow0, int ncol0, int lane) {
    const int fr = lane & 15, g = lane >> 4;
    Tout* C = reinterpret_cast<Tout*>(p.C);
    int nn[4];
    bool nok[4];
    float4 bias[4];
#pragma unroll
    for (int ni = 0; ni < 4; ++ni) {
        const int n = ncol0 + ni * 16 + g * 4;
        nok[ni] = n < p.N;
        nn[ni] = nok[ni] ? n : 0;
        const float* bp = (EPI != MTP_EPI_DGELU && EPI != MTP_EPI_MUL && p.bias) ? p.bias + (p.bias_mod > 0 ? nn[ni] % p.bias_mod : nn[ni]) : reinterpret_cast<const float*>(&g_zero16);
        const uint4 b = ldg16(bp);
        bias[ni] = make_float4(__uint_as_float(b.x), __uint_as_float(b.y), __uint_as_float(b.z), __uint_as_float(b.w));
    }
#pragma unroll
    for (int mi = 0; mi < MF; ++mi) {
        const int m = mrow0 + mi * 16 + fr;
        const bool mok = m < p.M;
        const int mc = mok ? m : 0;
        if (p.atomic_out) {
#pragma unroll
            for (int ni = 0; ni < 4; ++ni)
                if (mok && nok[ni]) {
                    float* c = reinterpret_cast<float*>(p.C) + (int64_t)m * p.ldc + nn[ni];
                    atomicAdd(c + 0, acc[ni][mi][0]); atomicAdd(c + 1, acc[ni][mi][1]); atomicAdd(c + 2, acc[ni][mi][2]); atomicAdd(c + 3, acc[ni][mi][3]);
                }
            continue;
        }
        float rs = 1.0f;
        float4 side[4];
        if (EPI == MTP_EPI_BIAS_RES) {
            const float* rsp = p.rowscale ? p.rowscale + mc / p.rows_per_sample : nullptr;
            const float* resrow = p.res + (int64_t)(p.res_mod > 0 ? mc % p.res_mod : mc) * p.res_ld;
#pragma unroll
            for (int ni = 0; ni < 4; ++ni) {
                const uint4 r = ldg16(resrow + nn[ni]);
                side[ni] = make_float4(__uint_as_float(r.x), __uint_as_float(r.y), __uint_as_float(r.z), __uint_as_float(r.w));
            }
            if (rsp) rs = *rsp;
        } else if (EPI == MTP_EPI_DGELU || EPI == MTP_EPI_MUL) {
#pragma unroll
            for (int ni = 0; ni < 4; ++ni) side[ni] = load4(reinterpret_cast<const Tout*>(p.aux) + (int64_t)mc * p.aux_ld + nn[ni]);
        }
#pragma unroll
        for (int ni = 0; ni < 4; ++ni) {
            float4 v = make_float4(acc[ni][mi][0] + bias[ni].x, acc[ni][mi][1] + bias[ni].y, acc[ni][mi][2] + bias[ni].z, acc[ni][mi][3] + bias[ni].w);
            const bool ok = mok && nok[ni];
            if (EPI == MTP_EPI_BIAS_GELU) {
                if (ok) store4(reinterpret_cast<Tout*>(p.aux) + (int64_t)m * p.aux_ld + nn[ni], v);
                v = make_float4(gelu_f(v.x), gelu_f(v.y), gelu_f(v.z), gelu_f(v.w));
            } else if (EPI == MTP_EPI_BIAS_GELU_DG) {
                float4 d;
                gelu_pair_f(v.x, v.x, d.x); gelu_pair_f(v.y, v.y, d.y); gelu_pair_f(v.z, v.z, d.z); gelu_pair_f(v.w, v.w, d.w);
                if (ok) store4(reinterpret_cast<Tout*>(p.aux) + (int64_t)m * p.aux_ld + nn[ni], d);
            } else if (EPI == MTP_EPI_DGELU) {
                v = make_float4(v.x * dgelu_f(side[ni].x), v.y * dgelu_f(side[ni].y), v.z * dgelu_f(side[ni].z), v.w * dgelu_f(side[ni].w));
            } else if (EPI == MTP_EPI_MUL) {
                v = make_float4(v.x * side[ni].x, v.y * side[ni].y, v.z * side[ni].z, v.w * side[ni].w);
            } else if (EPI == MTP_EPI_BIAS_RES) {
                v = make_float4(side[ni].x + rs * v.x, side[ni].y + rs * v.y, side[ni].z + rs * v.z, side[ni].w + rs * v.w);
            }
            if (ok) store4(C + (int64_t)m * p.ldc + nn[ni], v);
        }
    }
}

}
```

### mtp_amd/csrc/gemm_p8.hip

```cpp
#include "gemm_p8.h"

namespace {

struct P8Ctx {
    uint32_t addrA[2][2];
    uint32_t addrA1[2][2];
    uint32_t addrB[2][2];
    uint32_t voffA, voffB;
    const char* pA[2][2];
    const char* pB[2][2];
    uint32_t m0base;
};

template <int IMM>
__device__ __forceinline__ void dsr(u32x4_t& d, uint32_t addr) {
    asm volatile("ds_read_b128 %0, %1 offset:%2" : "=v"(d) : "v"(addr), "i"(IMM));
}

template <int SK, int SBUF>
__device__ __forceinline__ void nt_stage(const P8Ctx& c) {
    constexpr int h = (SK == KA1 || SK == KB1) ? 1 : 0;
    const uint32_t l0 = c.m0base + SBUF * P8_BUF + SK * P8_HALF;
    if constexpr (SK == KA0 || SK == KA1)
        glds2(c.voffA, c.pA[h][0], c.pA[h][1], l0, l0 + 1024);
    else
        glds2(c.voffB, c.pB[h][0], c.pB[h][1], l0, l0 + 1024);
}

template <int K, int BUF, int MI>
__device__ __forceinline__ void nt_read_a(const P8Ctx& c, u32x4_t (&a)[2][4]) {
    constexpr int o = K * P8_HALF;
    const uint32_t a0 = K == KA1 ? c.addrA1[BUF][0] : c.addrA[BUF][0], a1 = K == KA1 ? c.addrA1[BUF][1] : c.addrA[BUF][1];
    dsr<o + 0 * 2048>(a[0][0], a0); dsr<o + 1 * 2048>(a[0][1], a0); dsr<o + 2 * 2048>(a[0][2], a0);
    if constexpr (MI == 4) dsr<o + 3 * 2048>(a[0][3], a0);
    dsr<o + 0 * 2048>(a[1][0], a1); dsr<o + 1 * 2048>(a[1][1], a1); dsr<o + 2 * 2048>(a[1][2], a1);
    if constexpr (MI == 4) dsr<o + 3 * 2048>(a[1][3], a1);
}
template <int K, int BUF>
__device__ __forceinline__ void nt_read_b(const P8Ctx& c, u32x4_t (&b)[2][2]) {
    constexpr int o = K * P8_HALF;
    dsr<o + 0 * 2048>(b[0][0], c.addrB[BUF][0]); dsr<o + 1 * 2048>(b[0][1], c.addrB[BUF][0]);
    dsr<o + 0 * 2048>(b[1][0], c.addrB[BUF][1]); dsr<o + 1 * 2048>(b[1][1], c.addrB[BUF][1]);
}
template <int MI>
__device__ __forceinline__ void wait_a(u32x4_t (&a)[2][4]) {
    if constexpr (MI == 4)
        asm volatile("s_waitcnt lgkmcnt(0)"
                     : "+v"(a[0][0]), "+v"(a[0][1]), "+v"(a[0][2]), "+v"(a[0][3]), "+v"(a[1][0]), "+v"(a[1][1]), "+v"(a[1][2]), "+v"(a[1][3]));
    else
        asm volatile("s_waitcnt lgkmcnt(0)" : "+v"(a[0][0]), "+v"(a[0][1]), "+v"(a[0][2]), "+v"(a[1][0]), "+v"(a[1][1]), "+v"(a[1][2]));
}
__device__ __forceinline__ void wait_b(u32x4_t (&b)[2][2]) {
    asm volatile("s_waitcnt lgkmcnt(0)" : "+v"(b[0][0]), "+v"(b[0][1]), "+v"(b[1][0]), "+v"(b[1][1]));
}

template <int MI1>
struct NtOps {
    typedef P8Ctx Ctx;
    static constexpr int kLoadsPerPiecePair = 2;
    static constexpr int kMi1 = MI1;
    template <int K, int BUF> static __device__ __forceinline__ void read_a(Ctx& c, u32x4_t (&a)[2][4]) { nt_read_a<K, BUF, (K == KA1 ? MI1 : 4)>(c, a); }
    template <int K, int BUF> static __device__ __forceinline__ void read_b(Ctx& c, u32x4_t (&b)[2][2]) { nt_read_b<K, BUF>(c, b); }
    template <int SK, int SBUF> static __device__ __forceinline__ void stage(Ctx& c) { nt_stage<SK, SBUF>(c); }
    template <int K, int BUF> static __device__ __forceinline__ void retire_a(Ctx&, u32x4_t (&a)[2][4]) { wait_a<(K == KA1 ? MI1 : 4)>(a); }
    static __device__ __forceinline__ void retire_b(u32x4_t (&b)[2][2]) { wait_b(b); }
    static __device__ __forceinline__ void next_ktile(Ctx& c) { c.voffA += 128; c.voffB += 128; }
};

template <int MI1>
__device__ __forceinline__ void p8_tile_sources(const KArgs& p, P8Ctx& c, int wave, int m0, int n0, uint32_t voffA0, uint32_t voffB0) {
    constexpr int WROWS = 64 + 16 * MI1;
#pragma unroll
    for (int i = 0; i < 2; ++i) {
        const int q = wave * 2 + i;
        int ra0 = m0 + (q >> 3) * WROWS + (q & 7) * 8;
        const int qw = q / (2 * MI1), qx = q - qw * (2 * MI1);
        int ra1 = qw < 2 ? m0 + qw * WROWS + 64 + qx * 8 : m0;
        ra0 = ra0 < p.M - 8 ? ra0 : p.M - 8;
        ra1 = ra1 < p.M - 8 ? ra1 : p.M - 8;
        c.pA[0][i] = p.A + (int64_t)ra0 * p.lda * 2;
        c.pA[1][i] = p.A + (int64_t)ra1 * p.lda * 2;
#pragma unroll
        for (int h = 0; h < 2; ++h) {
            int rb = n0 + (q >> 2) * 64 + h * 32 + (q & 3) * 8;
            rb = rb < p.N - 8 ? rb : p.N - 8;
            c.pB[h][i] = p.B + (int64_t)rb * p.ldb * 2;
        }
    }
    c.voffA = voffA0;
    c.voffB = voffB0;
}
__device__ __forceinline__ void p8_issue_prologue(P8Ctx& c) {
    nt_stage<KB1, 0>(c); nt_stage<KA0, 0>(c); nt_stage<KB0, 0>(c); nt_stage<KA1, 0>(c);
    c.voffA += 128; c.voffB += 128;
    nt_stage<KB0, 1>(c); nt_stage<KA0, 1>(c); nt_stage<KB1, 1>(c); nt_stage<KA1, 1>(c);
    c.voffA += 128; c.voffB += 128;
}

template <typename Tout, int EPI, int MI1, int XP, int PS, int SP = 0>
__global__ __launch_bounds__(P8_THREADS) __attribute__((amdgpu_waves_per_eu(2, 2))) void gemm_nt_p8_kernel(KArgs p) {
    extern __shared__ __attribute__((aligned(16))) char smem[];
    constexpr int WROWS = 64 + 16 * MI1, BM = 2 * WROWS;
    const int tid = threadIdx.x, lane = tid & 63;
    const int wave = __builtin_amdgcn_readfirstlane(tid >> 6);
    const int wr = wave >> 2, wc = wave & 3;
    const int fr = lane & 15, g = lane >> 4;
    const uint32_t lds0 = (uint32_t)(uintptr_t)(__attribute__((address_space(3))) char*)(smem);
    const int tiles_m = (p.M + BM - 1) / BM, tiles_n = p.tiles_n, ntiles = tiles_m * tiles_n;
    const int plain = p.order & 1;
    const int pairs = p.k_tiles >> 1;

    P8Ctx c;
    {
        const uint32_t lanepart = (uint32_t)(fr * 128 + ((g ^ (fr & 7)) << 4));
#pragma unroll
        for (int b = 0; b < 2; ++b) {
            c.addrA[b][0] = lds0 + b * P8_BUF + wr * 8192 + lanepart;
            c.addrA[b][1] = lds0 + b * P8_BUF + wr * 8192 + (lanepart ^ 64u);
            c.addrA1[b][0] = lds0 + b * P8_BUF + wr * (MI1 * 2048) + lanepart;
            c.addrA1[b][1] = lds0 + b * P8_BUF + wr * (MI1 * 2048) + (lanepart ^ 64u);
            c.addrB[b][0] = lds0 + b * P8_BUF + wc * 4096 + lanepart;
            c.addrB[b][1] = lds0 + b * P8_BUF + wc * 4096 + (lanepart ^ 64u);
        }
        c.m0base = lds0 + wave * 2048;
    }
    const uint32_t lanesrc = (uint32_t)(((lane & 7) ^ (lane >> 3)) << 4);
    const uint32_t voffA0 = (uint32_t)((lane >> 3) * (int)p.lda * 2) + lanesrc;
    const uint32_t voffB0 = (uint32_t)((lane >> 3) * (int)p.ldb * 2) + lanesrc;

    int tile = blockIdx.x;
    int tm, tn;
    tile_coords(plain ? tile : xcd_remap(tile, ntiles), tiles_m, tiles_n, plain, tm, tn);
    int m0 = tm * BM, n0 = tn * P8_BN;
    p8_tile_sources<MI1>(p, c, wave, m0, n0, voffA0, voffB0);
    p8_issue_prologue(c);

    u32x4_t a[2][4], b0[2][2], b1[2][2];
    f32x4_t acc[4][8];
    for (;;) {
#pragma unroll
        for (int i = 0; i < 4; ++i)
#pragma unroll
            for (int j = 0; j < 8; ++j) acc[i][j] = f32x4_t{0.f, 0.f, 0.f, 0.f};

        wait_vm<12>();
        __builtin_amdgcn_sched_barrier(0);
        __builtin_amdgcn_s_barrier();
        __builtin_amdgcn_sched_barrier(0);
        nt_read_b<KB1, 0>(c, b1);
        wait_b(b1);
        __builtin_amdgcn_sched_barrier(0);
        __builtin_amdgcn_s_barrier();
        if (!(XP & 2) && wr == 1) __builtin_amdgcn_s_barrier();
        __builtin_amdgcn_sched_barrier(0);

        for (int it = 0; it < pairs - 1; ++it) two_tiles<NtOps<MI1>, false, XP>(c, a, b0, b1, acc);
        two_tiles<NtOps<MI1>, true, XP>(c, a, b0, b1, acc);

        __builtin_amdgcn_sched_barrier(0);
        if (!(XP & 2) && wr == 0) __builtin_amdgcn_s_barrier();
        __builtin_amdgcn_sched_barrier(0);

        if constexpr (PS) {
            const int em0 = m0, en0 = n0;
            tile += gridDim.x;
            const bool more = tile < ntiles;
            if (more) {
                tile_coords(plain ? tile : xcd_remap(tile, ntiles), tiles_m, tiles_n, plain, tm, tn);
                m0 = tm * BM; n0 = tn * P8_BN;
                p8_tile_sources<MI1>(p, c, wave, m0, n0, voffA0, voffB0);
                p8_issue_prologue(c);
            }
            __builtin_amdgcn_sched_barrier(0);
            epilogue_lds16<Tout, EPI, WROWS, SP>(p, acc, smem + P8_LDS + wave * 4096, em0 + wr * WROWS, en0 + wc * 64, lane);
            if (!more) break;
            __builtin_amdgcn_sched_barrier(0);
            wait_vm<0>();
        } else {
            if constexpr (SP != 0) {
                epilogue_lds16<Tout, EPI, WROWS, SP>(p, acc, smem + P8_LDS + wave * 4096, m0 + wr * WROWS, n0 + wc * 64, lane);
            } else if (!(XP & 4) || p.M < 0) {
                if constexpr (XP & 16)
                    epilogue<Tout, EPI, 8>(p, acc, m0 + wr * 128, n0 + wc * 64, lane);
                else
                    epilogue_lds<Tout, EPI, 64, 32, WROWS>(p, acc, smem + wave * P8_HALF, m0 + wr * WROWS, n0 + wc * 64, lane);
            }
            break;
        }
    }
}

template <typename Tout, int EPI, int MI1, int XP, int PS = 0, int SP = 0>
int launch_p8_kernel(const KArgs& a, int ntiles, hipStream_t stream) {
    constexpr int LDS = P8_LDS + ((PS || SP) ? 8 * 4096 : 0);
    static unsigned long long optin = 0;
    if (const int e = mtp_optin_lds((const void*)gemm_nt_p8_kernel<Tout, EPI, MI1, XP, PS, SP>, LDS, optin)) return e;
    const int cus = mtp_stream_cus(stream);
    const int grid = PS ? (ntiles < cus ? ntiles : cus) : ntiles;
    hipLaunchKernelGGL((gemm_nt_p8_kernel<Tout, EPI, MI1, XP, PS, SP>), dim3(grid), dim3(P8_THREADS), LDS, stream, a);
    return mtp_launch_status();
}

template <typename Tout, int EPI>
int launch_p8(const KArgs& k, const NtPlan& plan, hipStream_t stream) {
    const int bm = plan.tile_m, sp = plan.store_policy;
    const bool persist = plan.persistent;
    KArgs a = k;
    a.tiles_n = (k.N + P8_BN - 1) / P8_BN;
    a.k_tiles = k.K / 64;
    a.order = plan.order;
    a.atomic_out = 0;
    const int ntiles = mtp_nt_p8_tiles(k.M, k.N, bm);
    if (bm == 224 && sp == 1) return persist ? launch_p8_kernel<Tout, EPI, 3, 0, 1, 1>(a, ntiles, stream) : launch_p8_kernel<Tout, EPI, 3, 0, 0, 1>(a, ntiles, stream);
    if (bm == 224 && sp == 2) return persist ? launch_p8_kernel<Tout, EPI, 3, 0, 1, 2>(a, ntiles, stream) : launch_p8_kernel<Tout, EPI, 3, 0, 0, 2>(a, ntiles, stream);
    if (persist) {
        if (bm == 224) return launch_p8_kernel<Tout, EPI, 3, 0, 1>(a, ntiles, stream);
        return launch_p8_kernel<Tout, EPI, 4, 0, 1>(a, ntiles, stream);
    }
    if (bm == 224) return launch_p8_kernel<Tout, EPI, 3, 0>(a, ntiles, stream);
    return launch_p8_kernel<Tout, EPI, 4, 0>(a, ntiles, stream);
}

template <typename Tout>
int dispatch_p8(const KArgs& k, int epi, const NtPlan& plan, hipStream_t s) {
    switch (epi) {
        case MTP_EPI_BIAS: return launch_p8<Tout, MTP_EPI_BIAS>(k, plan, s);
        case MTP_EPI_BIAS_GELU: return launch_p8<Tout, MTP_EPI_BIAS_GELU>(k, plan, s);
        case MTP_EPI_DGELU: return launch_p8<Tout, MTP_EPI_DGELU>(k, plan, s);
        case MTP_EPI_BIAS_GELU_DG: return launch_p8<Tout, MTP_EPI_BIAS_GELU_DG>(k, plan, s);
        case MTP_EPI_MUL: return launch_p8<Tout, MTP_EPI_MUL>(k, plan, s);
        default: return MTP_ERR_UNSUPPORTED;
    }
}

}

int mtp_nt_p8_fits(const KArgs& k, int out_dtype, int epi) {
    if (k.K < 128 || (k.K % 128) || (k.M % 8) || (k.N % 8) || k.M < 8 || k.N < 8) return 0;
    if ((uint64_t)k.lda * 2 * 8 + (uint64_t)k.K * 2 >= (1ull << 31) || (uint64_t)k.ldb * 2 * 8 + (uint64_t)k.K * 2 >= (1ull << 31)) return 0;
    if (epi == MTP_EPI_BIAS_RES) return out_dtype == MTP_F32;
    if (out_dtype == MTP_BF16) return epi == MTP_EPI_BIAS || epi == MTP_EPI_BIAS_GELU || epi == MTP_EPI_DGELU || epi == MTP_EPI_BIAS_GELU_DG || epi == MTP_EPI_MUL;
    return out_dtype == MTP_F32 && epi == MTP_EPI_BIAS;
}

int mtp_nt_p8_tiles(int64_t M, int64_t N, int tile_m) { return (int)(((M + tile_m - 1) / tile_m) * ((N + P8_BN - 1) / P8_BN)); }

int mtp_nt_p8_pick_tile_m(int64_t M, int64_t N, int64_t cus) {
    const int64_t t256 = mtp_nt_p8_tiles(M, N, 256), t224 = mtp_nt_p8_tiles(M, N, 224);
    const int64_t c256 = ((t256 + cus - 1) / cus) * 256, c224 = ((t224 + cus - 1) / cus) * 224;
    return c224 < c256 ? 224 : 256;
}

int mtp_nt_p8_launch(const KArgs& k, int out_dtype, int epi, const NtPlan& plan, hipStream_t stream) {
    if (!mtp_nt_p8_fits(k, out_dtype, epi)) return MTP_ERR_UNSUPPORTED;
    if (epi == MTP_EPI_BIAS_RES) return launch_p8<float, MTP_EPI_BIAS_RES>(k, plan, stream);
    if (out_dtype == MTP_BF16) return dispatch_p8<bf16_t>(k, epi, plan, stream);
    return launch_p8<float, MTP_EPI_BIAS>(k, plan, stream);
}
```

### mtp_amd/csrc/runtime.hip

```cpp
#include "common.h"
#include <atomic>
#include <mutex>

extern "C" const char* mtp_version(void) { return "mtp_hip 0.6 (gfx950)"; }

extern "C" int mtp_stream_create_low_priority(void** stream) {
    if (!stream) return MTP_ERR_ARG;
    int least = 0, greatest = 0;
    hipError_t e = hipDeviceGetStreamPriorityRange(&least, &greatest);
    if (e != hipSuccess) return (int)e;
    hipStream_t s = nullptr;
    e = hipStreamCreateWithPriority(&s, hipStreamNonBlocking, least);
    if (e != hipSuccess) return (int)e;
    *stream = (void*)s;
    return 0;
}
namespace {
constexpr int kMaskSlots = 16;
std::atomic<void*> g_mask_stream[kMaskSlots];
std::atomic<int> g_mask_cus[kMaskSlots];
std::mutex g_mask_mu;
int device_cus() {
    static std::atomic<int> ncu{0};
    int n = ncu.load(std::memory_order_relaxed);
    if (!n) {
        int dev = 0;
        hipDeviceProp_t prop;
        if (hipGetDevice(&dev) != hipSuccess || hipGetDeviceProperties(&prop, dev) != hipSuccess) return 256;
        n = prop.multiProcessorCount;
        ncu.store(n, std::memory_order_relaxed);
    }
    return n;
}
}

int mtp_stream_cus(hipStream_t stream) {
    if (stream)
        for (int i = 0; i < kMaskSlots; ++i)
            if (g_mask_stream[i].load(std::memory_order_acquire) == (void*)stream) return g_mask_cus[i].load(std::memory_order_relaxed);
    return device_cus();
}

extern "C" int mtp_stream_create_cu_mask(const uint32_t* mask, int words, void** stream) {
    if (!mask || !stream || words <= 0 || words > 32) return MTP_ERR_ARG;
    for (int x = 0; x < 8; ++x) {
        bool any = false;
        for (int i = x; i < words * 32 && i < 256; i += 8) any |= (mask[i / 32] >> (i % 32)) & 1u;
        if (!any) return MTP_ERR_ARG;
    }
    int cus = 0;
    for (int i = 0; i < words * 32 && i < 256; ++i) cus += (mask[i / 32] >> (i % 32)) & 1u;
    std::lock_guard<std::mutex> lock(g_mask_mu);
    int slot = -1;
    for (int i = 0; i < kMaskSlots && slot < 0; ++i)
        if (!g_mask_stream[i].load(std::memory_order_relaxed)) slot = i;
    if (slot < 0) return MTP_ERR_UNSUPPORTED;
    hipStream_t s = nullptr;
    hipError_t e = hipExtStreamCreateWithCUMask(&s, (uint32_t)words, mask);
    if (e != hipSuccess) return (int)e;
    g_mask_cus[slot].store(cus, std::memory_order_relaxed);
    g_mask_stream[slot].store((void*)s, std::memory_order_release);
    *stream = (void*)s;
    return 0;
}

namespace {
__global__ void __launch_bounds__(256) probe_placement_kernel(int32_t* __restrict__ out, long long spin) {
    const long long t0 = __builtin_readcyclecounter();
    if (threadIdx.x == 0) {
        out[2 * blockIdx.x + 0] = (int32_t)__builtin_amdgcn_s_getreg((31 << 11) | 20);
        out[2 * blockIdx.x + 1] = (int32_t)__builtin_amdgcn_s_getreg((31 << 11) | 4);
    }
    while (__builtin_readcyclecounter() - t0 < spin) __builtin_amdgcn_s_sleep(8);
}
}

extern "C" int mtp_probe_placement(int32_t* out, int blocks, int64_t spin_clocks, mtp_stream_t stream) {
    if (!out || blocks <= 0 || spin_clocks < 0 || spin_clocks > (1ll << 28)) return MTP_ERR_ARG;
    hipLaunchKernelGGL(probe_placement_kernel, dim3(blocks), dim3(256), 0, (hipStream_t)stream, out, (long long)spin_clocks);
    return mtp_launch_status();
}

extern "C" int mtp_stream_destroy(void* stream) {
    if (!stream) return MTP_ERR_ARG;
    {
        std::lock_guard<std::mutex> lock(g_mask_mu);
        for (int i = 0; i < kMaskSlots; ++i)
            if (g_mask_stream[i].load(std::memory_order_relaxed) == stream) g_mask_stream[i].store(nullptr, std::memory_order_release);
    }
    return (int)hipStreamDestroy((hipStream_t)stream);
}
```

### mtp_amd/csrc/rvsa_sampling.hip

```cpp
#include "common.h"

namespace {

template <typename T>
__global__ __launch_bounds__(256) void rvsa_pool_fwd_kernel(const T* __restrict__ x, float* __restrict__ avg, float* __restrict__ pooled,
                                                           int Hp, int Wp, int C, int pad_t, int pad_l, int nh, int nw) {
    const int win = blockIdx.x;
    const int j = win % nw, i = (win / nw) % nh, b = win / (nw * nh);
    for (int c4 = blockIdx.y * 256 + threadIdx.x; c4 < C / 4; c4 += gridDim.y * 256) {
        float4 s = make_float4(0, 0, 0, 0);
        for (int a = 0; a < 7; ++a) {
            const int y = i * 7 + a - pad_t;
            if (y < 0 || y >= Hp) continue;
            for (int bb = 0; bb < 7; ++bb) {
                const int xx = j * 7 + bb - pad_l;
                if (xx < 0 || xx >= Wp) continue;
                const float4 v = load4(x + (((int64_t)b * Hp + y) * Wp + xx) * C + 4 * c4);
                s.x += v.x; s.y += v.y; s.z += v.z; s.w += v.w;
            }
        }
        const float inv = 1.0f / 49.0f;
        s = make_float4(s.x * inv, s.y * inv, s.z * inv, s.w * inv);
        store4(avg + (int64_t)win * C + 4 * c4, s);
        store4(pooled + (int64_t)win * C + 4 * c4, make_float4(s.x > 0 ? s.x : 0.01f * s.x, s.y > 0 ? s.y : 0.01f * s.y,
                                                              s.z > 0 ? s.z : 0.01f * s.z, s.w > 0 ? s.w : 0.01f * s.w));
    }
}
template <typename T>
__global__ __launch_bounds__(256) void rvsa_pool_bwd_kernel(const float* __restrict__ dpooled, const float* __restrict__ avg, T* __restrict__ dx, int accumulate,
                                                           int B, int Hp, int Wp, int C, int pad_t, int pad_l, int nh, int nw) {
    const int C4 = C / 4;
    const int64_t total = (int64_t)B * Hp * Wp * C4;
    for (int64_t idx = (int64_t)blockIdx.x * 256 + threadIdx.x; idx < total; idx += (int64_t)gridDim.x * 256) {
        const int c4 = (int)(idx % C4);
        const int64_t t = idx / C4;
        const int xx = (int)(t % Wp), yy = (int)((t / Wp) % Hp), b = (int)(t / ((int64_t)Wp * Hp));
        const int win = (b * nh + (yy + pad_t) / 7) * nw + (xx + pad_l) / 7;
        const float4 d = load4(dpooled + (int64_t)win * C + 4 * c4), a = load4(avg + (int64_t)win * C + 4 * c4);
        const float k = 1.0f / 49.0f;
        float4 g = make_float4(d.x * (a.x > 0 ? k : 0.01f * k), d.y * (a.y > 0 ? k : 0.01f * k), d.z * (a.z > 0 ? k : 0.01f * k), d.w * (a.w > 0 ? k : 0.01f * k));
        T* p = dx + t * C + 4 * c4;
        if (accumulate) {
            const float4 o = load4(p);
            g.x += o.x; g.y += o.y; g.z += o.z; g.w += o.w;
        }
        store4(p, g);
    }
}

__global__ __launch_bounds__(256) void small_linear_fwd_generic_kernel(const float* __restrict__ x, const float* __restrict__ w, const float* __restrict__ bias,
                                                                      float* __restrict__ y, int N, int K) {
    const int r = blockIdx.x, lane = threadIdx.x & 63, wave = threadIdx.x >> 6;
    const float* xr = x + (int64_t)r * K;
    for (int n = wave; n < N; n += 4) {
        const float* wr = w + (int64_t)n * K;
        float s = 0.f;
        for (int k = lane * 4; k < K; k += 256) {
            const float4 a = load4(xr + k), b = load4(wr + k);
            s += a.x * b.x + a.y * b.y + a.z * b.z + a.w * b.w;
        }
        s = wave_sum(s);
        if (lane == 0) y[(int64_t)r * N + n] = s + (bias ? bias[n] : 0.f);
    }
}
template <int ROWS, int MAXJ>
__global__ __launch_bounds__(256) void small_linear_fwd_kernel(const float* __restrict__ x, const float* __restrict__ w, const float* __restrict__ bias,
                                                              float* __restrict__ y, int R, int N, int K) {
    const int lane = threadIdx.x & 63, wave = threadIdx.x >> 6;
    const int r0 = blockIdx.x * ROWS;
    const int K4 = K >> 2;
    float4 xs[ROWS][MAXJ];
#pragma unroll
    for (int i = 0; i < ROWS; ++i) {
        const float* xr = x + (int64_t)(r0 + i < R ? r0 + i : R - 1) * K;
#pragma unroll
        for (int j = 0; j < MAXJ; ++j) {
            const int k4 = lane + 64 * j;
            xs[i][j] = k4 < K4 ? load4(xr + 4 * k4) : make_float4(0.f, 0.f, 0.f, 0.f);
        }
    }
    const int per = (N + 3) / 4, n_lo = wave * per, n_hi = (n_lo + per) < N ? (n_lo + per) : N;
    for (int n = n_lo; n < n_hi; n += 4) {
        float s[4][ROWS];
#pragma unroll
        for (int q = 0; q < 4; ++q) {
            const int nn = n + q < n_hi ? n + q : n_hi - 1;
            const float* wr = w + (int64_t)nn * K;
#pragma unroll
            for (int i = 0; i < ROWS; ++i) s[q][i] = 0.f;
#pragma unroll
            for (int j = 0; j < MAXJ; ++j) {
                const int k4 = lane + 64 * j, k4c = k4 < K4 ? k4 : K4 - 1;
                const float4 b = load4(wr + 4 * k4c);
#pragma unroll
                for (int i = 0; i < ROWS; ++i) s[q][i] += xs[i][j].x * b.x + xs[i][j].y * b.y + xs[i][j].z * b.z + xs[i][j].w * b.w;
            }
        }
#pragma unroll
        for (int q = 0; q < 4; ++q)
#pragma unroll
            for (int i = 0; i < ROWS; ++i) s[q][i] = wave_sum(s[q][i]);
        if (lane == 0) {
#pragma unroll
            for (int q = 0; q < 4; ++q)
#pragma unroll
                for (int i = 0; i < ROWS; ++i)
                    if (n + q < n_hi && r0 + i < R) y[(int64_t)(r0 + i) * N + n + q] = s[q][i] + (bias ? bias[n + q] : 0.f);
        }
    }
}
__global__ __launch_bounds__(256) void small_linear_dx_kernel(const float* __restrict__ dy, const float* __restrict__ w, float* __restrict__ dx, int R, int N, int K) {
    const int k = (blockIdx.x * 256 + threadIdx.x) * 4, r0 = blockIdx.y * 4;
    if (k >= K) return;
    const float* d[4];
    float4 s[4];
#pragma unroll
    for (int i = 0; i < 4; ++i) {
        const int rr = r0 + i < R ? r0 + i : R - 1;
        d[i] = dy + (int64_t)rr * N;
        s[i] = make_float4(0.f, 0.f, 0.f, 0.f);
    }
#pragma unroll 4
    for (int n = 0; n < N; ++n) {
        const float4 ww = load4(w + (int64_t)n * K + k);
#pragma unroll
        for (int i = 0; i < 4; ++i) {
            const float dv = d[i][n];
            s[i].x += dv * ww.x; s[i].y += dv * ww.y; s[i].z += dv * ww.z; s[i].w += dv * ww.w;
        }
    }
#pragma unroll
    for (int i = 0; i < 4; ++i)
        if (r0 + i < R) store4(dx + (int64_t)(r0 + i) * K + k, s[i]);
}
constexpr int SL_DW_ROWS = 32;
struct SlSegs {
    float* dw[4];
    float* db[4];
    int row0[5];
    int nseg;
};
constexpr int SL_BATCH = 8;
struct SlBatch {
    const float* dy[SL_BATCH];
    const float* x[SL_BATCH];
    SlSegs seg[SL_BATCH];
    int zsplit;
};
template <bool SEG>
__device__ __forceinline__ void small_linear_dw_body(const float* __restrict__ dy, const float* __restrict__ x, float* __restrict__ dw, float* __restrict__ db, int R, int N, int K,
                                                     const SlSegs& seg, int zrow) {
    __shared__ float4 red[3][8][64];
    __shared__ float redb[3][8];
    const int lane = threadIdx.x & 63, wave = __builtin_amdgcn_readfirstlane(threadIdx.x >> 6);
    const int k = (blockIdx.x * 64 + lane) * 4, n0 = blockIdx.y * 8;
    const int r0 = (zrow * 4 + wave) * SL_DW_ROWS, r1 = (r0 + SL_DW_ROWS) < R ? (r0 + SL_DW_ROWS) : R;
    const bool kok = k < K;
    const int kc = kok ? k : 0;
    int nn[8];
    float4 s[8];
    float sb[8];
#pragma unroll
    for (int q = 0; q < 8; ++q) {
        nn[q] = n0 + q < N ? n0 + q : N - 1;
        s[q] = make_float4(0.f, 0.f, 0.f, 0.f);
        sb[q] = 0.f;
    }
#pragma unroll 8
    for (int r = r0; r < r1; ++r) {
        const float4 xv = load4(x + (int64_t)r * K + kc);
        const float* dr = dy + (int64_t)r * N;
#pragma unroll
        for (int q = 0; q < 8; ++q) {
            const float dv = dr[nn[q]];
            s[q].x += dv * xv.x; s[q].y += dv * xv.y; s[q].z += dv * xv.z; s[q].w += dv * xv.w;
            sb[q] += dv;
        }
    }
    if (wave > 0) {
#pragma unroll
        for (int q = 0; q < 8; ++q) {
            red[wave - 1][q][lane] = s[q];
            if (lane == 0) redb[wave - 1][q] = sb[q];
        }
    }
    __syncthreads();
    if (wave == 0) {
#pragma unroll
        for (int q = 0; q < 8; ++q) {
#pragma unroll
            for (int v = 0; v < 3; ++v) {
                const float4 o = red[v][q][lane];
                s[q].x += o.x; s[q].y += o.y; s[q].z += o.z; s[q].w += o.w;
                sb[q] += redb[v][q];
            }
            float* dwrow = dw + (int64_t)(n0 + q) * K;
            float* dbp = db ? db + n0 + q : nullptr;
            if constexpr (SEG) {
                int j = 0;
                const int n = n0 + q < N ? n0 + q : N - 1;
#pragma unroll
                for (int t = 1; t < 4; ++t) j += (t < seg.nseg && n >= seg.row0[t]) ? 1 : 0;
                dwrow = seg.dw[j] + (int64_t)(n - seg.row0[j]) * K;
                dbp = seg.db[j] ? seg.db[j] + (n - seg.row0[j]) : nullptr;
            }
            if (kok && n0 + q < N) {
                float* o = dwrow + k;
                atomicAdd(o, s[q].x); atomicAdd(o + 1, s[q].y); atomicAdd(o + 2, s[q].z); atomicAdd(o + 3, s[q].w);
            }
            if (dbp && blockIdx.x == 0 && lane == 0 && n0 + q < N) atomicAdd(dbp, sb[q]);
        }
    }
}
template <bool SEG>
__global__ __launch_bounds__(256) void small_linear_dw_kernel(const float* __restrict__ dy, const float* __restrict__ x, float* __restrict__ dw, float* __restrict__ db, int R, int N, int K, SlSegs seg) {
    small_linear_dw_body<SEG>(dy, x, dw, db, R, N, K, seg, (int)blockIdx.z);
}
__global__ __launch_bounds__(256) void small_linear_dw_batched_kernel(SlBatch t, int R, int N, int K) {
    const int pi = __builtin_amdgcn_readfirstlane((int)blockIdx.z / t.zsplit);
    small_linear_dw_body<true>(t.dy[pi], t.x[pi], nullptr, nullptr, R, N, K, t.seg[pi], (int)blockIdx.z - pi * t.zsplit);
}

}

template <typename T>
__global__ __launch_bounds__(256) void rvsa_sampling_fwd_kernel(const T* __restrict__ x, const float* __restrict__ w, const float* __restrict__ bias,
                                                               float* __restrict__ avg, float* __restrict__ pooled, float* __restrict__ samp,
                                                               int Hp, int Wp, int C, int N, int pad_t, int pad_l, int nh, int nw) {
    extern __shared__ __attribute__((aligned(16))) float pl[];
    const int win = blockIdx.x, lane = threadIdx.x & 63, wave = threadIdx.x >> 6;
    const int j = win % nw, i = (win / nw) % nh, b = win / (nw * nh);
    for (int c4 = threadIdx.x; c4 < C / 4; c4 += 256) {
        float4 s = make_float4(0, 0, 0, 0);
#pragma unroll
        for (int a = 0; a < 7; ++a) {
            const int y = i * 7 + a - pad_t;
            const bool yok = y >= 0 && y < Hp;
            const int yc = yok ? y : 0;
            float4 v[7];
#pragma unroll
            for (int bb = 0; bb < 7; ++bb) {
                const int xx = j * 7 + bb - pad_l;
                const int xc = (xx >= 0 && xx < Wp) ? xx : 0;
                v[bb] = load4(x + (((int64_t)b * Hp + yc) * Wp + xc) * C + 4 * c4);
            }
#pragma unroll
            for (int bb = 0; bb < 7; ++bb) {
                const int xx = j * 7 + bb - pad_l;
                const float m = (yok && xx >= 0 && xx < Wp) ? 1.f : 0.f;
                s.x += m * v[bb].x; s.y += m * v[bb].y; s.z += m * v[bb].z; s.w += m * v[bb].w;
            }
        }
        const float inv = 1.0f / 49.0f;
        s = make_float4(s.x * inv, s.y * inv, s.z * inv, s.w * inv);
        const float4 p = make_float4(s.x > 0 ? s.x : 0.01f * s.x, s.y > 0 ? s.y : 0.01f * s.y, s.z > 0 ? s.z : 0.01f * s.z, s.w > 0 ? s.w : 0.01f * s.w);
        if (blockIdx.y == 0) {
            store4(avg + (int64_t)win * C + 4 * c4, s);
            store4(pooled + (int64_t)win * C + 4 * c4, p);
        }
        *reinterpret_cast<float4*>(pl + 4 * c4) = p;
    }
    __syncthreads();
    const int nper = ((N + (int)gridDim.y - 1) / (int)gridDim.y + 3) / 4 * 4, nlo = (int)blockIdx.y * nper, nhi = (nlo + nper) < N ? (nlo + nper) : N;
    for (int n0 = nlo + 4 * wave; n0 < nhi; n0 += 16) {
        float acc[4] = {0.f, 0.f, 0.f, 0.f};
        for (int k0 = lane * 4; k0 < C; k0 += 1024) {
            float4 ww[4][4], a[4];
#pragma unroll
            for (int kk = 0; kk < 4; ++kk) {
                const int k = k0 + 256 * kk, kc = k < C ? k : 0;
                a[kk] = k < C ? *reinterpret_cast<const float4*>(pl + kc) : make_float4(0.f, 0.f, 0.f, 0.f);
#pragma unroll
                for (int q = 0; q < 4; ++q) {
                    const int n = n0 + q < N ? n0 + q : N - 1;
                    ww[kk][q] = load4(w + (int64_t)n * C + kc);
                }
            }
#pragma unroll
            for (int kk = 0; kk < 4; ++kk)
#pragma unroll
                for (int q = 0; q < 4; ++q) acc[q] += a[kk].x * ww[kk][q].x + a[kk].y * ww[kk][q].y + a[kk].z * ww[kk][q].z + a[kk].w * ww[kk][q].w;
        }
#pragma unroll
        for (int q = 0; q < 4; ++q) {
            const float t = wave_sum(acc[q]);
            if (lane == 0 && n0 + q < nhi) samp[(int64_t)win * N + n0 + q] = t + (bias ? bias[n0 + q] : 0.f);
        }
    }
}

template <typename T>
__global__ __launch_bounds__(256) void rvsa_sampling_bwd_kernel(const float* __restrict__ dsamp, const float* __restrict__ w, const float* __restrict__ avg,
                                                               T* __restrict__ dx, int Hp, int Wp, int C, int N, int pad_t, int pad_l, int nh, int nw) {
    extern __shared__ __attribute__((aligned(16))) float ds[];
    __shared__ float4 part[4][64];
    const int win = blockIdx.x;
    const int j = win % nw, i = (win / nw) % nh, b = win / (nw * nh);
    const int lane = threadIdx.x & 63, q = threadIdx.x >> 6;
    const int c4 = blockIdx.y * 64 + lane;
    const bool live = c4 < C / 4;
    for (int n = threadIdx.x; n < N; n += 256) ds[n] = dsamp[(int64_t)win * N + n];
    __syncthreads();
    const int nq = (N + 3) / 4, n0 = q * nq, n1 = (n0 + nq) < N ? (n0 + nq) : N;
    float4 d = make_float4(0, 0, 0, 0);
    if (live) {
#pragma unroll 4
        for (int n = n0; n < n1; ++n) {
            const float4 ww = load4(w + (int64_t)n * C + 4 * c4);
            const float t = ds[n];
            d.x += t * ww.x; d.y += t * ww.y; d.z += t * ww.z; d.w += t * ww.w;
        }
    }
    part[q][lane] = d;
    __syncthreads();
    if (!live) return;
    const float4 p0 = part[0][lane], p1 = part[1][lane], p2 = part[2][lane], p3 = part[3][lane];
    d = make_float4((p0.x + p1.x) + (p2.x + p3.x), (p0.y + p1.y) + (p2.y + p3.y), (p0.z + p1.z) + (p2.z + p3.z), (p0.w + p1.w) + (p2.w + p3.w));
    const float4 a = load4(avg + (int64_t)win * C + 4 * c4);
    const float k = 1.0f / 49.0f;
    const float4 g = make_float4(d.x * (a.x > 0 ? k : 0.01f * k), d.y * (a.y > 0 ? k : 0.01f * k), d.z * (a.z > 0 ? k : 0.01f * k), d.w * (a.w > 0 ? k : 0.01f * k));
#pragma unroll 1
    for (int aa = q; aa < 7; aa += 4) {
        const int y = i * 7 + aa - pad_t;
        if (y < 0 || y >= Hp) continue;
        float4 o[7];
#pragma unroll
        for (int bb = 0; bb < 7; ++bb) {
            const int xx = j * 7 + bb - pad_l;
            const int xc = (xx >= 0 && xx < Wp) ? xx : 0;
            o[bb] = load4(dx + (((int64_t)b * Hp + y) * Wp + xc) * C + 4 * c4);
        }
#pragma unroll
        for (int bb = 0; bb < 7; ++bb) {
            const int xx = j * 7 + bb - pad_l;
            if (xx >= 0 && xx < Wp)
                store4(dx + (((int64_t)b * Hp + y) * Wp + xx) * C + 4 * c4, make_float4(o[bb].x + g.x, o[bb].y + g.y, o[bb].z + g.z, o[bb].w + g.w));
        }
    }
}

__global__ __launch_bounds__(256) void rvsa_sampling_bwd_win_kernel(const float* __restrict__ dsamp, const float* __restrict__ w, const float* __restrict__ avg,
                                                                   float* __restrict__ g, int C, int N) {
    extern __shared__ __attribute__((aligned(16))) float ds[];
    __shared__ float4 part[4][64];
    const int win = blockIdx.x;
    const int lane = threadIdx.x & 63, q = threadIdx.x >> 6;
    const int c4 = blockIdx.y * 64 + lane;
    const bool live = c4 < C / 4;
    for (int n = threadIdx.x; n < N; n += 256) ds[n] = dsamp[(int64_t)win * N + n];
    __syncthreads();
    const int nq = (N + 3) / 4, n0 = q * nq, n1 = (n0 + nq) < N ? (n0 + nq) : N;
    float4 d = make_float4(0, 0, 0, 0);
    if (live) {
#pragma unroll 10
        for (int n = n0; n < n1; ++n) {
            const float4 ww = load4(w + (int64_t)n * C + 4 * c4);
            const float t = ds[n];
            d.x += t * ww.x; d.y += t * ww.y; d.z += t * ww.z; d.w += t * ww.w;
        }
    }
    part[q][lane] = d;
    __syncthreads();
    if (!live || q) return;
    const float4 p0 = part[0][lane], p1 = part[1][lane], p2 = part[2][lane], p3 = part[3][lane];
    d = make_float4((p0.x + p1.x) + (p2.x + p3.x), (p0.y + p1.y) + (p2.y + p3.y), (p0.z + p1.z) + (p2.z + p3.z), (p0.w + p1.w) + (p2.w + p3.w));
    const float4 a = load4(avg + (int64_t)win * C + 4 * c4);
    const float k = 1.0f / 49.0f;
    *reinterpret_cast<float4*>(g + (int64_t)win * C + 4 * c4) =
        make_float4(d.x * (a.x > 0 ? k : 0.01f * k), d.y * (a.y > 0 ? k : 0.01f * k), d.z * (a.z > 0 ? k : 0.01f * k), d.w * (a.w > 0 ? k : 0.01f * k));
}

extern "C" int mtp_rvsa_sampling_bwd_win(const float* dsamp, const float* w, const float* avg, float* g, int64_t windows, int64_t C, int64_t N, mtp_stream_t stream) {
    if (!dsamp || !w || !avg || !g || windows <= 0 || C <= 0 || (C % 4) || N <= 0 || N > 4096) return MTP_ERR_ARG;
    const dim3 grid((unsigned)windows, (unsigned)((C / 4 + 63) / 64)), block(256);
    rvsa_sampling_bwd_win_kernel<<<grid, block, sizeof(float) * (size_t)N, (hipStream_t)stream>>>(dsamp, w, avg, g, (int)C, (int)N);
    return mtp_launch_status();
}

extern "C" int mtp_rvsa_sampling_fwd(const void* x, int dtype, const float* w, const float* bias, float* avg, float* pooled, float* samp,
                                     int64_t B, int64_t Hp, int64_t Wp, int64_t C, int64_t N, mtp_stream_t stream) {
    if (!x || !w || !avg || !pooled || !samp || B <= 0 || Hp <= 0 || Wp <= 0 || C <= 0 || (C % 4) || C > 8192 || N <= 0) return MTP_ERR_ARG;
    const RvsaWindows win(Hp, Wp);
    constexpr int ysplit = 2;
    const dim3 grid((unsigned)(B * win.nh * win.nw), (unsigned)(N >= 16 * ysplit ? ysplit : 1)), block(256);
    const size_t lds = sizeof(float) * (size_t)C;
    return for_act(dtype, [&](auto t) {
        using T = decltype(t);
        rvsa_sampling_fwd_kernel<T><<<grid, block, lds, (hipStream_t)stream>>>((const T*)x, w, bias, avg, pooled, samp, (int)Hp, (int)Wp, (int)C, (int)N, win.pad_t, win.pad_l, win.nh, win.nw);
    });
}
extern "C" int mtp_rvsa_sampling_bwd(const float* dsamp, const float* w, const float* avg, void* dx, int dtype,
                                     int64_t B, int64_t Hp, int64_t Wp, int64_t C, int64_t N, mtp_stream_t stream) {
    if (!dsamp || !w || !avg || !dx || B <= 0 || Hp <= 0 || Wp <= 0 || C <= 0 || (C % 4) || N <= 0 || N > 4096) return MTP_ERR_ARG;
    const RvsaWindows win(Hp, Wp);
    const dim3 grid((unsigned)(B * win.nh * win.nw), (unsigned)((C / 4 + 63) / 64)), block(256);
    const size_t lds = sizeof(float) * (size_t)N;
    return for_act(dtype, [&](auto t) {
        using T = decltype(t);
        rvsa_sampling_bwd_kernel<T><<<grid, block, lds, (hipStream_t)stream>>>(dsamp, w, avg, (T*)dx, (int)Hp, (int)Wp, (int)C, (int)N, win.pad_t, win.pad_l, win.nh, win.nw);
    });
}

extern "C" int mtp_rvsa_pool_fwd(const void* x, int dtype, float* avg, float* pooled, int64_t B, int64_t Hp, int64_t Wp, int64_t C, mtp_stream_t stream) {
    if (!x || !avg || !pooled || B <= 0 || (C % 4)) return MTP_ERR_ARG;
    const RvsaWindows win(Hp, Wp);
    const dim3 grid((unsigned)(B * win.nh * win.nw), (unsigned)((C / 4 + 255) / 256));
    return for_act(dtype, [&](auto t) {
        using T = decltype(t);
        rvsa_pool_fwd_kernel<T><<<grid, kThreads, 0, (hipStream_t)stream>>>((const T*)x, avg, pooled, (int)Hp, (int)Wp, (int)C, win.pad_t, win.pad_l, win.nh, win.nw);
    });
}
extern "C" int mtp_rvsa_pool_bwd(const float* dpooled, const float* avg, void* dx, int dtype, int accumulate, int64_t B, int64_t Hp, int64_t Wp, int64_t C, mtp_stream_t stream) {
    if (!dpooled || !avg || !dx || B <= 0 || (C % 4)) return MTP_ERR_ARG;
    const RvsaWindows win(Hp, Wp);
    return for_act(dtype, [&](auto t) {
        using T = decltype(t);
        rvsa_pool_bwd_kernel<T><<<blocks_for(B * Hp * Wp * C / 4, kThreads, 8192), kThreads, 0, (hipStream_t)stream>>>(dpooled, avg, (T*)dx, accumulate, (int)B, (int)Hp, (int)Wp, (int)C,
                                                                                                                      win.pad_t, win.pad_l, win.nh, win.nw);
    });
}

extern "C" int mtp_small_linear_fwd(const float* x, const float* w, const float* b, float* y, int64_t R, int64_t N, int64_t K, mtp_stream_t stream) {
    if (!x || !w || !y || R <= 0 || N <= 0 || (K % 4)) return MTP_ERR_ARG;
    if (K <= 1024)
        small_linear_fwd_kernel<4, 4><<<dim3((unsigned)((R + 3) / 4)), kThreads, 0, (hipStream_t)stream>>>(x, w, b, y, (int)R, (int)N, (int)K);
    else if (K <= 2048)
        small_linear_fwd_kernel<2, 8><<<dim3((unsigned)((R + 1) / 2)), kThreads, 0, (hipStream_t)stream>>>(x, w, b, y, (int)R, (int)N, (int)K);
    else
        small_linear_fwd_generic_kernel<<<(unsigned)R, kThreads, 0, (hipStream_t)stream>>>(x, w, b, y, (int)N, (int)K);
    return mtp_launch_status();
}
extern "C" int mtp_small_linear_bwd(const float* x, const float* w, const float* dy, float* dx, float* dw, float* db, int64_t R, int64_t N, int64_t K, mtp_stream_t stream) {
    if (!x || !w || !dy || R <= 0 || N <= 0 || (K % 4)) return MTP_ERR_ARG;
    hipStream_t s = (hipStream_t)stream;
    if (dx) small_linear_dx_kernel<<<dim3((unsigned)((K + 1023) / 1024), (unsigned)((R + 3) / 4)), kThreads, 0, s>>>(dy, w, dx, (int)R, (int)N, (int)K);
    if (dw) {
        if (db == dw + N * K) {
            (void)hipMemsetAsync(dw, 0, sizeof(float) * (size_t)(N * K + N), s);
        } else {
            (void)hipMemsetAsync(dw, 0, sizeof(float) * (size_t)(N * K), s);
            if (db) (void)hipMemsetAsync(db, 0, sizeof(float) * (size_t)N, s);
        }
        const dim3 grid((unsigned)((K + 255) / 256), (unsigned)((N + 7) / 8), (unsigned)((R + 4 * SL_DW_ROWS - 1) / (4 * SL_DW_ROWS)));
        small_linear_dw_kernel<false><<<grid, kThreads, 0, s>>>(dy, x, dw, db, (int)R, (int)N, (int)K, SlSegs{});
    }
    return mtp_launch_status();
}
extern "C" int mtp_small_linear_dw_segments(const float* x, const float* dy, int64_t R, int64_t N, int64_t K, int nseg, const int64_t* seg_rows,
                                            float* const* dw, float* const* db, mtp_stream_t stream) {
    if (!x || !dy || !seg_rows || !dw || R <= 0 || N <= 0 || K <= 0 || (K % 4) || nseg < 1 || nseg > 4) return MTP_ERR_ARG;
    SlSegs seg{};
    int64_t r = 0;
    for (int j = 0; j < nseg; ++j) {
        if (!dw[j] || seg_rows[j] <= 0) return MTP_ERR_ARG;
        seg.dw[j] = dw[j];
        seg.db[j] = db ? db[j] : nullptr;
        seg.row0[j] = (int)r;
        r += seg_rows[j];
    }
    if (r != N) return MTP_ERR_ARG;
    seg.row0[nseg] = (int)N;
    seg.nseg = nseg;
    const dim3 grid((unsigned)((K + 255) / 256), (unsigned)((N + 7) / 8), (unsigned)((R + 4 * SL_DW_ROWS - 1) / (4 * SL_DW_ROWS)));
    small_linear_dw_kernel<true><<<grid, kThreads, 0, (hipStream_t)stream>>>(dy, x, (float*)nullptr, (float*)nullptr, (int)R, (int)N, (int)K, seg);
    return mtp_launch_status();
}

extern "C" int mtp_small_linear_dw_segments_batched(const float* const* xs, const float* const* dys, int count, int64_t R, int64_t N, int64_t K, int nseg,
                                                    const int64_t* seg_rows, float* const* dw, float* const* db, mtp_stream_t stream) {
    if (!xs || !dys || !seg_rows || !dw || count <= 0 || count > SL_BATCH || R <= 0 || N <= 0 || K <= 0 || (K % 4) || nseg < 1 || nseg > 4) return MTP_ERR_ARG;
    SlBatch t{};
    for (int i = 0; i < count; ++i) {
        if (!xs[i] || !dys[i]) return MTP_ERR_ARG;
        t.x[i] = xs[i];
        t.dy[i] = dys[i];
        int64_t r = 0;
        for (int j = 0; j < nseg; ++j) {
            if (!dw[i * nseg + j] || seg_rows[j] <= 0) return MTP_ERR_ARG;
            t.seg[i].dw[j] = dw[i * nseg + j];
            t.seg[i].db[j] = db ? db[i * nseg + j] : nullptr;
            t.seg[i].row0[j] = (int)r;
            r += seg_rows[j];
        }
        if (r != N) return MTP_ERR_ARG;
        t.seg[i].row0[nseg] = (int)N;
        t.seg[i].nseg = nseg;
    }
    t.zsplit = (int)((R + 4 * SL_DW_ROWS - 1) / (4 * SL_DW_ROWS));
    small_linear_dw_batched_kernel<<<dim3((unsigned)((K + 255) / 256), (unsigned)((N + 7) / 8), (unsigned)(t.zsplit * count)), kThreads, 0, (hipStream_t)stream>>>(t, (int)R, (int)N, (int)K);
    return mtp_launch_status();
}
```

### mtp_amd/engine.py

```python
import os

import torch

from . import ops
from .engine_base import EngineBase

F32 = torch.float32


class _Blk:
    __slots__ = ("window", "pre", "wqkv", "wqkvT", "wproj", "wprojT", "w1", "w1T", "w2", "w2T", "wsamp", "bsamp", "bproj", "b2", "wproj_s", "w2_s")


class BackboneEngine(EngineBase):
    def __init__(self, module, act_dtype=torch.bfloat16):
        super().__init__(module, act_dtype)
        self.C = module.embed_dim
        self.depth = len(module.blocks)
        self.heads = module.num_heads
        self.hd = self.C // self.heads
        self.scale = module.qk_scale if module.qk_scale is not None else self.hd ** -0.5
        self.window = [bool(w) for w in module.window_blocks]
        self.out_indices = list(module.out_indices)
        self._blk = None
        self._fpn = None
        self._pe = None
        self._ls = []
        self._zero_rel = {}

    def _fold_sources(self, P):
        with torch.no_grad():
            for pre, b in self._ls:
                g1, g2 = P[pre + "gamma_1"].detach(), P[pre + "gamma_2"].detach()
                torch.mul(P[pre + "attn.proj.weight"].detach(), g1[:, None], out=b.wproj_s)
                torch.mul(P[pre + "mlp.fc2.weight"].detach(), g2[:, None], out=b.w2_s)
                torch.mul(P[pre + "attn.proj.bias"].detach(), g1, out=b.bproj)
                torch.mul(P[pre + "mlp.fc2.bias"].detach(), g2, out=b.b2)

    def _pack_weights(self, P):
        for name, (wg, wgT) in self._fpn.items():
            ops.convt_pack(P[name + ".weight"].detach().contiguous(), wg, wgT)

    def fusable_images(self):
        return None if self._ls else self._wimg

    def _build_weight_images(self, P):
        dev = P["patch_embed.proj.weight"].device
        act, H, C = self.act, self.heads, self.C
        entries = []

        def both(w2d):
            w2d = w2d.detach()
            assert w2d.is_contiguous()
            R, Cc = w2d.shape
            wt = torch.empty(Cc, R, device=dev, dtype=act)
            w = w2d if act == F32 else torch.empty(R, Cc, device=dev, dtype=act)
            entries.append((w2d, None if act == F32 else w, wt, False))
            return w, wt

        ls = getattr(self.m, "init_values", None) is not None
        self._ls = []

        blks = []
        for i in range(self.depth):
            b = _Blk()
            b.window = self.window[i]
            b.pre = pre = "blocks.%d." % i
            b.wqkv, b.wqkvT = both(P[pre + "attn.qkv.weight"])
            b.bproj, b.b2 = P[pre + "attn.proj.bias"].detach(), P[pre + "mlp.fc2.bias"].detach()
            if ls:
                b.wproj_s, b.w2_s = torch.empty_like(P[pre + "attn.proj.weight"]), torch.empty_like(P[pre + "mlp.fc2.weight"])
                b.bproj, b.b2 = torch.empty_like(P[pre + "attn.proj.bias"]), torch.empty_like(P[pre + "mlp.fc2.bias"])
                self._ls.append((pre, b))
                b.wproj, b.wprojT = both(b.wproj_s)
            else:
                b.wproj, b.wprojT = both(P[pre + "attn.proj.weight"])
            b.w1, b.w1T = both(P[pre + "mlp.fc1.weight"])
            b.w2, b.w2T = both(b.w2_s if ls else P[pre + "mlp.fc2.weight"])
            if b.window:
                b.wsamp = torch.empty(5 * H, C, device=dev, dtype=F32)
                b.bsamp = torch.empty(5 * H, device=dev, dtype=F32)
                r0 = 0
                for head, rows in (("sampling_offsets", 2 * H), ("sampling_scales", 2 * H), ("sampling_angles", H)):
                    entries.append((P[pre + "attn.%s.2.weight" % head].detach().view(rows, C), b.wsamp[r0:r0 + rows], None, True))
                    entries.append((P[pre + "attn.%s.2.bias" % head].detach().view(1, rows), b.bsamp[r0:r0 + rows], None, True))
                    r0 += rows
            blks.append(b)
        self._blk = blks
        wpe = P["patch_embed.proj.weight"].detach()
        self._pe = both(wpe.view(wpe.shape[0], -1))
        fpn = {}
        for name in ("fpn1.0", "fpn1.3", "fpn2.0"):
            if name + ".weight" in P:
                Cin, Cout = P[name + ".weight"].shape[:2]
                fpn[name] = (torch.empty(4 * Cout, Cin, device=dev, dtype=act), torch.empty(Cin, 4 * Cout, device=dev, dtype=act))
        self._fpn = fpn
        self._wimg = ops.WeightImages(entries, act)

    wgrad_side_stream = True
    wgrad_max_jobs = 8
    wgrad_keep = 2

    @staticmethod
    def _colsum(dy, out):
        return ops.colsum(dy, out, accumulate=True)

    def _ln_bwd(self, *args, **kw):
        return ops.layernorm_bwd(*args, accumulate=True, defer=self._ln_parts, **kw)

    def _full_rel(self, pre, Hp, Wp):
        h = self.P.get(pre + "attn.full_attn_rel_pos_h")
        if h is not None:
            w = self.P[pre + "attn.full_attn_rel_pos_w"]
            if h.shape[0] < 2 * Hp - 1 or w.shape[0] < 2 * Wp - 1:
                raise ValueError("%sattn.full_attn_rel_pos_h/w have %d / %d rows, a %d x %d token grid needs %d / %d (resize them like "
                                 "init_weights does, or build the model for this input size)" % (pre, h.shape[0], w.shape[0], Hp, Wp, 2 * Hp - 1, 2 * Wp - 1))
            return h[:2 * Hp - 1], w[:2 * Wp - 1]
        key = (Hp, Wp)
        if self._zero_rel.get(key) is None:
            self._zero_rel[key] = (torch.zeros(2 * Hp - 1, self.hd, device=self.dev, dtype=F32),
                                   torch.zeros(2 * Wp - 1, self.hd, device=self.dev, dtype=F32))
        return self._zero_rel[key]

    def _drop_scales(self, B, training):
        rates = [float(self.m.drop_path_rates[i]) for i in range(self.depth)]
        live = [training and r > 0.0 and self.m.blocks[i].training for i, r in enumerate(rates)]
        if not any(live):
            return [(None, None)] * self.depth
        keep = torch.tensor([1.0 - r for r in rates], dtype=F32).to(self.dev, non_blocking=True).view(self.depth, 1, 1)
        s = torch.floor(keep + torch.rand(self.depth, 2, B, device=self.dev, dtype=F32)) / keep
        return [(s[i, 0], s[i, 1]) if live[i] else (None, None) for i in range(self.depth)]

    def _block_fwd(self, i, x, B, Hp, Wp, dps, save):
        P, b, C, T, N = self.P, self._blk[i], self.C, x.shape[0], Hp * Wp
        pre = b.pre
        s = {}
        mean1, rstd1 = self._e(T, dtype=F32), self._e(T, dtype=F32)
        ln1 = ops.layernorm_fwd(x, P[pre + "norm1.weight"], P[pre + "norm1.bias"], self._e(T, C), mean1, rstd1)
        if b.window:
            nh, nw = ops.rvsa_windows(Hp, Wp)
            R = B * nh * nw
            avg, pooled = self._e(R, C, dtype=F32), self._e(R, C, dtype=F32)
            samp = ops.rvsa_sampling_fwd(ln1, b.wsamp, b.bsamp, avg, pooled, self._e(R, 5 * self.heads, dtype=F32), B, Hp, Wp)
        qkv = ops.gemm_nt(ln1, b.wqkv, self._e(T, 3 * C), bias=P[pre + "attn.qkv.bias"])
        o = self._e(T, C)
        if b.window:
            lse = self._e(R * self.heads * 49, dtype=F32)
            ops.rvsa_attn_fwd(qkv, samp, o, lse, P[pre + "attn.rel_pos_h"], P[pre + "attn.rel_pos_w"],
                              P[pre + "attn.relative_position_bias_table"], B, Hp, Wp, self.heads, self.scale)
            s.update(avg=avg, pooled=pooled, samp=samp)
        else:
            lse = self._e(B * self.heads * N, dtype=F32)
            rel_h, rel_w = self._full_rel(pre, Hp, Wp)
            ops.full_attn_fwd(qkv, o, lse, rel_h, rel_w, B, Hp, Wp, self.heads, self.scale)
        x1 = ops.gemm_nt(o, b.wproj, self._e(T, C, dtype=F32), epi=ops.EPI_BIAS_RES, bias=b.bproj, res=x,
                         rowscale=dps[0], rows_per_sample=N)
        mean2, rstd2 = self._e(T, dtype=F32), self._e(T, dtype=F32)
        ln2 = ops.layernorm_fwd(x1, P[pre + "norm2.weight"], P[pre + "norm2.bias"], self._e(T, C), mean2, rstd2)
        u = self._e(T, 4 * C)
        h = ops.gemm_nt(ln2, b.w1, self._e(T, 4 * C), epi=ops.EPI_BIAS_GELU_DG, bias=P[pre + "mlp.fc1.bias"], aux=u)
        x2 = ops.gemm_nt(h, b.w2, self._e(T, C, dtype=F32), epi=ops.EPI_BIAS_RES, bias=b.b2, res=x1,
                         rowscale=dps[1], rows_per_sample=N)
        if save:
            s.update(x=x, mean1=mean1, rstd1=rstd1, ln1=ln1, qkv=qkv, o=o, lse=lse, x1=x1, mean2=mean2, rstd2=rstd2, ln2=ln2, u=u, h=h)
        return x2, s

    def _layer_scale_grads(self, pre, lin, gname, G):
        P = self.P
        gw, gb, gam = G[pre + lin + ".weight"], G[pre + lin + ".bias"], P[pre + gname]
        G[pre + gname].add_((gw * P[pre + lin + ".weight"]).sum(1) + gb * P[pre + lin + ".bias"])
        gw.mul_(gam[:, None])
        gb.mul_(gam)

    def _block_bwd(self, i, s, dx2, dx2_act, B, Hp, Wp, dps, G, extra, prev_scale):
        P, b, C, N = self.P, self._blk[i], self.C, Hp * Wp
        pre = b.pre
        T = dx2.shape[0]
        wq = self._wq
        ls = pre + "gamma_1" in G
        wq.add(dx2_act, s["h"], G[pre + "mlp.fc2.weight"], G[pre + "mlp.fc2.bias"], after=(lambda: self._layer_scale_grads(pre, "mlp.fc2", "gamma_2", G)) if ls else None,
               norm_ok=not ls)
        du = ops.gemm_nt(dx2_act, b.w2T, self._e(T, 4 * C), epi=ops.EPI_MUL, aux=s["u"])
        wq.add(du, s["ln2"], G[pre + "mlp.fc1.weight"], G[pre + "mlp.fc1.bias"])
        dln2 = ops.gemm_nt(du, b.w1T, self._e(T, C))
        del du
        dx1, dx1_act = self._e(T, C, dtype=F32), self._e(T, C)
        self._ln_bwd(dln2, s["x1"], s["mean2"], s["rstd2"], P[pre + "norm2.weight"], dx1, G[pre + "norm2.weight"], G[pre + "norm2.bias"],
                          dres=dx2, dx_copy=dx1_act, copy_scale=dps[0], rows_per_sample=N)
        wq.add(dx1_act, s["o"], G[pre + "attn.proj.weight"], G[pre + "attn.proj.bias"], after=(lambda: self._layer_scale_grads(pre, "attn.proj", "gamma_1", G)) if ls else None,
               norm_ok=not ls)
        do = ops.gemm_nt(dx1_act, b.wprojT, self._e(T, C))
        dqkv = self._e(T, 3 * C)
        if b.window:
            nh, nw = ops.rvsa_windows(Hp, Wp)
            R = B * nh * nw
            H = self.heads
            dsamp = self._e(R, 5 * H, dtype=F32)
            ops.rvsa_attn_bwd(s["qkv"], s["samp"], s["o"], do, s["lse"], dqkv, dsamp,
                              P[pre + "attn.rel_pos_h"], P[pre + "attn.rel_pos_w"], P[pre + "attn.relative_position_bias_table"],
                              G[pre + "attn.rel_pos_h"], G[pre + "attn.rel_pos_w"], G[pre + "attn.relative_position_bias_table"],
                              B, Hp, Wp, H, self.scale, accumulate=True, defer=self._ln_parts)
            names = ("sampling_offsets", "sampling_scales", "sampling_angles")
            self._sl_jobs.append((s["pooled"], dsamp, [G[pre + "attn.%s.2.weight" % n].view(-1, C) for n in names],
                                  [G[pre + "attn.%s.2.bias" % n] for n in names]))
        else:
            rel_h, rel_w = self._full_rel(pre, Hp, Wp)
            if pre + "attn.full_attn_rel_pos_h" in G:
                drel_h, drel_w = G[pre + "attn.full_attn_rel_pos_h"][:2 * Hp - 1], G[pre + "attn.full_attn_rel_pos_w"][:2 * Wp - 1]
            else:
                drel_h, drel_w = self._e(*rel_h.shape, dtype=F32), self._e(*rel_w.shape, dtype=F32)
            ops.full_attn_bwd(s["qkv"], s["o"], do, s["lse"], dqkv, rel_h, rel_w, drel_h, drel_w, B, Hp, Wp, self.heads, self.scale,
                              accumulate=True, defer=self._ln_parts)
        wq.add(dqkv, s["ln1"], G[pre + "attn.qkv.weight"], G[pre + "attn.qkv.bias"])
        win_add = None
        if b.window:
            win_add = ops.rvsa_sampling_bwd_win(dsamp, b.wsamp, s["avg"], self._e(*s["avg"].shape, dtype=F32))
        dln1 = ops.gemm_nt(dqkv, b.wqkvT, self._e(T, C))
        dx0, dx0_act = self._e(T, C, dtype=F32), self._e(T, C)
        self._ln_bwd(dln1, s["x"], s["mean1"], s["rstd1"], P[pre + "norm1.weight"], dx0, G[pre + "norm1.weight"], G[pre + "norm1.bias"],
                          dres=dx1, extra=extra, dx_copy=dx0_act, copy_scale=prev_scale, rows_per_sample=N,
                          **(dict(win_add=win_add, grid=(B, Hp, Wp)) if win_add is not None else {}))
        return dx0, dx0_act

    def forward(self, img, training=False, need_grad=False, feature_dtype=None):
        m = self.m
        self.dev = img.device
        self.prepare_weights()
        self.P = P = {k: v.detach() for k, v in self.params().items()}
        C, act = self.C, self.act
        ps = m.patch_size
        fdt = feature_dtype or act
        if img.dtype == torch.uint8:
            pp = getattr(m, "data_preprocessor", None)
            if pp is None:
                raise ValueError("uint8 input needs ViT_Win_RVSA_V3_WSZ7.set_data_preprocessor(mean, std, ...)")
            B, H, W, Cin = img.shape
            Hp, Wp = ops.padded_grid(H, W, ps, pp["pad_size_divisor"])
            N, T = Hp * Wp, B * Hp * Wp
            cols = ops.preprocess_patchify(img.contiguous(), self._e(T, Cin * ps * ps), ps, pp["mean"], pp["std"], pp["bgr_to_rgb"],
                                           pp["pad_size_divisor"], pp["pad_value"])
            H, W = Hp * ps, Wp * ps
        else:
            B, Cin, H, W = img.shape
            Hp, Wp = H // ps, W // ps
            N, T = Hp * Wp, B * Hp * Wp
            img = img.contiguous()
            if img.dtype != F32:
                img = img.float()
            cols = ops.patchify(img, self._e(T, Cin * ps * ps), ps)
        pos = P.get("pos_embed")
        if pos is not None:
            assert pos.shape[1] == N, "pos_embed does not match the input size"
            x = ops.gemm_nt(cols, self._pe[0], self._e(T, C, dtype=F32), epi=ops.EPI_BIAS_RES, bias=P["patch_embed.proj.bias"],
                            res=pos.reshape(N, C), res_mod=N)
        else:
            x = ops.gemm_nt(cols, self._pe[0], self._e(T, C, dtype=F32), bias=P["patch_embed.proj.bias"])
        dps = self._drop_scales(B, training)
        ckpt = bool(m.use_checkpoint) and need_grad
        saved, taps = [], {}
        vitdet = bool(getattr(m, "_vitdet", False))
        last = self.depth - 1 if vitdet else max(self.out_indices)
        for i in range(self.depth):
            if i > last:
                break
            xin = x
            x, s = self._block_fwd(i, x, B, Hp, Wp, dps[i], save=need_grad and not ckpt)
            saved.append(s if (need_grad and not ckpt) else ({"x": xin} if need_grad else None))
            if i in self.out_indices:
                taps[i] = x
        final = None
        if vitdet:
            fm, fr = self._e(T, dtype=F32), self._e(T, dtype=F32)
            xn = ops.layernorm_fwd(x, P["norm.weight"], P["norm.bias"], self._e(T, C, dtype=F32), fm, fr)
            final = (x, fm, fr)
            tap_list = [xn, xn, xn, xn]
        else:
            tap_list = [taps[i] for i in self.out_indices]
        if getattr(m, "_taps_only", False):
            feats = [ops.tokens_to_nchw(t, self._e(B, C, Hp, Wp, dtype=fdt), B, Hp, Wp, 0) for t in tap_list]
            fctx = {"taps_only": True}
        else:
            feats, fctx = self._fpn_fwd(tap_list, B, Hp, Wp, fdt, need_grad)
        ctx = None
        if need_grad:
            ctx = dict(saved=saved, dps=dps, fctx=fctx, cols=cols, geom=(B, Cin, H, W, Hp, Wp), ckpt=ckpt, last=last, final=final)
        return feats, ctx

    def _fpn_fwd(self, taps, B, Hp, Wp, fdt, need_grad):
        P, C, T = self.P, self.C, B * Hp * Wp
        m = self.m
        feats, fctx = [], {}
        if m.patch_size == 8:
            t0 = taps[0] if self.act == F32 else ops.cast(taps[0], self._e(T, C))
            z = ops.gemm_nt(t0, self._fpn["fpn1.0"][0], self._e(T, 4 * C), bias=P["fpn1.0.bias"], bias_mod=C)
            feats.append(ops.tokens_to_nchw(z.view(4 * T, C), self._e(B, C, 2 * Hp, 2 * Wp, dtype=fdt), B, Hp, Wp, 1))
            feats.append(ops.tokens_to_nchw(taps[1], self._e(B, C, Hp, Wp, dtype=fdt), B, Hp, Wp, 0))
            H2, W2, H4, W4 = Hp // 2, Wp // 2, Hp // 4, Wp // 4
            p3 = ops.maxpool2_tokens_fwd(taps[2], self._e(B * H2 * W2, C), B, Hp, Wp)
            feats.append(ops.tokens_to_nchw(p3, self._e(B, C, H2, W2, dtype=fdt), B, H2, W2, 0))
            q1 = ops.maxpool2_tokens_fwd(taps[3], self._e(B * H2 * W2, C, dtype=F32), B, Hp, Wp)
            q2 = ops.maxpool2_tokens_fwd(q1, self._e(B * H4 * W4, C), B, H2, W2)
            feats.append(ops.tokens_to_nchw(q2, self._e(B, C, H4, W4, dtype=fdt), B, H4, W4, 0))
            if need_grad:
                fctx = dict(p8=True, t0=t0, tap2=taps[2], tap3=taps[3], q1=q1)
            return feats, fctx
        if m.patch_size != 16:
            raise NotImplementedError("the reference defines the FPN tail for patch_size 16 and 8 only (VIT:640-670)")
        t0 = taps[0] if self.act == F32 else ops.cast(taps[0], self._e(T, C))
        y1 = ops.gemm_nt(t0, self._fpn["fpn1.0"][0], self._e(T, 4 * C), bias=P["fpn1.0.bias"], bias_mod=C)
        mean, rstd = self._e(4 * T, dtype=F32), self._e(4 * T, dtype=F32)
        g1 = ops.layernorm_fwd(y1.view(4 * T, C), P["fpn1.1.ln.weight"], P["fpn1.1.ln.bias"], self._e(4 * T, C), mean, rstd, gelu=True)
        y2 = ops.gemm_nt(g1, self._fpn["fpn1.3"][0], self._e(4 * T, 4 * C), bias=P["fpn1.3.bias"], bias_mod=C)
        feats.append(ops.tokens_to_nchw(y2.view(16 * T, C), self._e(B, C, 4 * Hp, 4 * Wp, dtype=fdt), B, Hp, Wp, 2))
        t1 = taps[1] if self.act == F32 else ops.cast(taps[1], self._e(T, C))
        z = ops.gemm_nt(t1, self._fpn["fpn2.0"][0], self._e(T, 4 * C), bias=P["fpn2.0.bias"], bias_mod=C)
        feats.append(ops.tokens_to_nchw(z.view(4 * T, C), self._e(B, C, 2 * Hp, 2 * Wp, dtype=fdt), B, Hp, Wp, 1))
        feats.append(ops.tokens_to_nchw(taps[2], self._e(B, C, Hp, Wp, dtype=fdt), B, Hp, Wp, 0))
        Ho, Wo = Hp // 2, Wp // 2
        pooled = ops.maxpool2_tokens_fwd(taps[3], self._e(B * Ho * Wo, C), B, Hp, Wp)
        feats.append(ops.tokens_to_nchw(pooled, self._e(B, C, Ho, Wo, dtype=fdt), B, Ho, Wo, 0))
        if need_grad:
            fctx = dict(t0=t0, y1=y1, mean=mean, rstd=rstd, g1=g1, t1=t1, tap3=taps[3])
        return feats, fctx

    def _convt_wgrad(self, dy, x, gw):
        dwg = self._e(dy.shape[1], x.shape[1], dtype=F32)
        self._wq.add(dy, x, dwg, after=lambda: ops.convt_unpack_grad(dwg, gw), norm_of=gw)

    def _fpn_bwd(self, dfeats, fctx, B, Hp, Wp, G):
        P, C, T, act = self.P, self.C, B * Hp * Wp, self.act
        out = [None] * 4

        def as_in(df):
            df = df.contiguous()
            return df if df.dtype in (F32, torch.bfloat16) else df.float()

        if fctx.get("p8"):
            H2, W2, H4, W4 = Hp // 2, Wp // 2, Hp // 4, Wp // 4
            if dfeats[0] is not None:
                dz = ops.nchw_to_tokens(as_in(dfeats[0]), self._e(4 * T, C), B, Hp, Wp, 1)
                self._convt_wgrad(dz.view(T, 4 * C), fctx["t0"], G["fpn1.0.weight"])
                self._colsum(dz, G["fpn1.0.bias"])
                out[0] = ops.gemm_nt(dz.view(T, 4 * C), self._fpn["fpn1.0"][1], self._e(T, C, dtype=F32))
            if dfeats[1] is not None:
                out[1] = ops.nchw_to_tokens(as_in(dfeats[1]), self._e(T, C, dtype=F32), B, Hp, Wp, 0)
            if dfeats[2] is not None:
                dp = ops.nchw_to_tokens(as_in(dfeats[2]), self._e(B * H2 * W2, C, dtype=F32), B, H2, W2, 0)
                out[2] = ops.maxpool2_tokens_bwd(fctx["tap2"], dp, self._e(T, C, dtype=F32), B, Hp, Wp)
            if dfeats[3] is not None:
                dq2 = ops.nchw_to_tokens(as_in(dfeats[3]), self._e(B * H4 * W4, C, dtype=F32), B, H4, W4, 0)
                dq1 = ops.maxpool2_tokens_bwd(fctx["q1"], dq2, self._e(B * H2 * W2, C, dtype=F32), B, H2, W2)
                out[3] = ops.maxpool2_tokens_bwd(fctx["tap3"], dq1, self._e(T, C, dtype=F32), B, Hp, Wp)
            return out

        if dfeats[0] is not None:
            dy2 = ops.nchw_to_tokens(as_in(dfeats[0]), self._e(16 * T, C), B, Hp, Wp, 2)
            self._convt_wgrad(dy2.view(4 * T, 4 * C), fctx["g1"], G["fpn1.3.weight"])
            self._colsum(dy2, G["fpn1.3.bias"])
            dg1 = ops.gemm_nt(dy2.view(4 * T, 4 * C), self._fpn["fpn1.3"][1], self._e(4 * T, C))
            dy1 = self._e(4 * T, C)
            self._ln_bwd(dg1, fctx["y1"].view(4 * T, C), fctx["mean"], fctx["rstd"], P["fpn1.1.ln.weight"], dy1,
                              G["fpn1.1.ln.weight"], G["fpn1.1.ln.bias"], beta=P["fpn1.1.ln.bias"], gelu=True)
            self._convt_wgrad(dy1.view(T, 4 * C), fctx["t0"], G["fpn1.0.weight"])
            self._colsum(dy1, G["fpn1.0.bias"])
            out[0] = ops.gemm_nt(dy1.view(T, 4 * C), self._fpn["fpn1.0"][1], self._e(T, C, dtype=F32))
        if dfeats[1] is not None:
            dz = ops.nchw_to_tokens(as_in(dfeats[1]), self._e(4 * T, C), B, Hp, Wp, 1)
            self._convt_wgrad(dz.view(T, 4 * C), fctx["t1"], G["fpn2.0.weight"])
            self._colsum(dz, G["fpn2.0.bias"])
            out[1] = ops.gemm_nt(dz.view(T, 4 * C), self._fpn["fpn2.0"][1], self._e(T, C, dtype=F32))
        if dfeats[2] is not None:
            out[2] = ops.nchw_to_tokens(as_in(dfeats[2]), self._e(T, C, dtype=F32), B, Hp, Wp, 0)
        if dfeats[3] is not None:
            Ho, Wo = Hp // 2, Wp // 2
            dp = ops.nchw_to_tokens(as_in(dfeats[3]), self._e(B * Ho * Wo, C, dtype=F32), B, Ho, Wo, 0)
            out[3] = ops.maxpool2_tokens_bwd(fctx["tap3"], dp, self._e(T, C, dtype=F32), B, Hp, Wp)
        return out

    def backward(self, ctx, dfeats, G, need_input_grad=False, on_block_done=None, split_last=False, sqn=None):
        B, Cin, H, W, Hp, Wp = ctx["geom"]
        C, N, T = self.C, Hp * Wp, B * Hp * Wp
        P = self.P
        self.dev = ctx["cols"].device
        wq = self._begin_backward(sqn)
        if ctx["fctx"].get("taps_only"):
            dtaps = [None if d is None else ops.nchw_to_tokens((d.contiguous() if d.dtype in (F32, torch.bfloat16) else d.float().contiguous()),
                                                               self._e(T, C, dtype=F32), B, Hp, Wp, 0) for d in dfeats]
        else:
            dtaps = self._fpn_bwd(dfeats, ctx["fctx"], B, Hp, Wp, G)
        tapgrad = {}
        last, dps, saved = ctx["last"], ctx["dps"], ctx["saved"]
        if ctx.get("final") is not None:
            dsum = None
            for d in dtaps:
                if d is None:
                    continue
                if dsum is None:
                    dsum = d
                else:
                    ops.axpy(dsum, d)
            if dsum is not None:
                xl, fm, fr = ctx["final"]
                tapgrad[last] = self._ln_bwd(dsum, xl, fm, fr, P["norm.weight"], self._e(T, C, dtype=F32), G["norm.weight"], G["norm.bias"])
        else:
            for idx, d in zip(self.out_indices, dtaps):
                if d is None:
                    continue
                if idx in tapgrad:
                    ops.axpy(tapgrad[idx], d)
                else:
                    tapgrad[idx] = d
        self._ln_flush()
        if on_block_done is not None and not wq.jobs:
            on_block_done(self.depth)
        if last not in tapgrad:
            tapgrad[last] = torch.zeros(T, C, device=self.dev, dtype=F32)
        dx = tapgrad[last]
        dx_act = self._scaled_copy(dx, dps[last][1], N)
        for i in range(last, -1, -1):
            s = saved[i]
            if ctx["ckpt"]:
                _, s = self._block_fwd(i, s["x"], B, Hp, Wp, dps[i], save=True)
            extra = tapgrad.get(i - 1) if i > 0 else None
            prev_scale = dps[i - 1][1] if i > 0 else None
            dx, dx_act = self._block_bwd(i, s, dx, dx_act, B, Hp, Wp, dps[i], G, extra, prev_scale)
            saved[i] = None
            if i == 0:
                wq.add(dx_act, ctx["cols"], G["patch_embed.proj.weight"].view(C, -1), G["patch_embed.proj.bias"])
            if i == 0 or wq.should_flush() or not wq.jobs or (split_last and i == 1):
                self._burst_out(i, on_block_done)
        self._wait_bursts()
        self._report_pending(on_block_done)
        if "pos_embed" in G:
            ops.reduce_rows(dx.view(B, N * C), G["pos_embed"])
        dimg = None
        if need_input_grad:
            dcols = ops.gemm_nt(dx_act, self._pe[1], self._e(T, ctx["cols"].shape[1]))
            dimg = ops.unpatchify(dcols, self._e(B, Cin, H, W, dtype=F32), self.m.patch_size)
        if on_block_done is not None:
            on_block_done(-1)
        return dimg

    def _scaled_copy(self, dx, scale, N):
        return ops.scale_rows_cast(dx, self._e(*dx.shape), scale, N)
```

### mtp_amd/ops.py

```python
import ctypes as C

import torch

from . import _lib
from ._lib import (EPI_BIAS, EPI_BIAS_GELU, EPI_BIAS_GELU_DG, EPI_BIAS_RES, EPI_DGELU, EPI_MUL, MTP_BF16, MTP_F32, GemmArgs,
                   check)
from ._lib import (GEMM_NT_FAMILY_P8, GEMM_NT_FAMILY_REG, GEMM_NT_FAMILY_SB, GEMM_NT_FAMILY_SB8, GEMM_NT_FAMILY_STRIP, GEMM_NT_NO_P8,
                   GEMM_NT_NO_PERSIST, GEMM_NT_NO_SB8, GEMM_NT_NO_STRIP, GEMM_NT_P8, GEMM_NT_P8_224, GEMM_NT_P8_256, GEMM_NT_PERSIST,
                   GEMM_NT_REG_STAGED, GEMM_NT_SB8, GEMM_NT_STRIP, GEMM_ORDER_GROUPED, GEMM_ORDER_PLAIN, GEMM_ORDER_ROW_MAJOR, GEMM_STORE_NT,
                   GEMM_STORE_PLAIN, GEMM_STORE_SC1, GEMM_TN_REG_TRANSPOSE, GEMM_TN_TR_FULL_ONLY, GEMM_TNG_PLAIN_ORDER, GEMM_TNG_PLAIN_PHASES)

_DT = {torch.float32: MTP_F32, torch.bfloat16: MTP_BF16}
def lib():
    return _lib.load()


def _dt(t):
    try:
        return _DT[t.dtype]
    except KeyError:
        raise TypeError("mtp_amd ops take float32 / bfloat16 tensors, got %s" % t.dtype)


def _p(t):
    if t is None:
        return None
    if not t.is_cuda:
        raise RuntimeError("mtp_amd ops run only on an MI355X device tensor (no CPU fallback)")
    if not t.is_contiguous():
        raise RuntimeError("mtp_amd ops need contiguous tensors")
    if t.device.index != torch.cuda.current_device():
        raise RuntimeError("mtp_amd ops: tensor on %s but the current device is cuda:%d -- call torch.cuda.set_device(%d) (or use "
                           "`with torch.cuda.device(...)`) before running the backbone" % (t.device, torch.cuda.current_device(), t.device.index))
    return t.data_ptr()


def _s():
    return torch.cuda.current_stream().cuda_stream


def _scratch(shape, device, dtype):
    return torch.empty(shape, device=device, dtype=dtype)


def _f32(t):
    if t is not None and t.dtype != torch.float32:
        raise TypeError("expected a float32 tensor")
    return _p(t)


def _nt_args(a, w, out, epi, bias, bias_mod, res, res_mod, rowscale, rows_per_sample, aux, variant, n=None):
    M, K = a.shape
    N = w.shape[0] if n is None else n
    assert w.shape[1] == K and out.shape[0] == M and out.shape[1] >= N and w.shape[0] >= N and a.dtype == w.dtype
    assert n is not None or out.shape[1] == N
    g = GemmArgs()
    g.A, g.B, g.C = _p(a), _p(w), _p(out)
    g.M, g.N, g.K = M, N, K
    g.lda, g.ldb, g.ldc = K, K, out.shape[1]
    g.in_dtype, g.out_dtype, g.epilogue = _dt(a), _dt(out), epi
    g.bias, g.bias_mod = _f32(bias), bias_mod
    g.res, g.res_ld, g.res_mod = _f32(res), (res.shape[-1] if res is not None else 0), res_mod
    g.rowscale, g.rows_per_sample = _f32(rowscale), rows_per_sample
    g.aux, g.aux_ld = _p(aux), (aux.shape[-1] if aux is not None else 0)
    if aux is not None:
        assert aux.dtype == out.dtype and tuple(aux.shape) == (M, N) and out.shape[1] == N
    g.split_k, g.variant = 1, variant
    return g


def gemm_nt(a, w, out, epi=EPI_BIAS, bias=None, bias_mod=0, res=None, res_mod=0, rowscale=None, rows_per_sample=0,
            aux=None, variant=0, n=None):
    g = _nt_args(a, w, out, epi, bias, bias_mod, res, res_mod, rowscale, rows_per_sample, aux, variant, n)
    check(lib().mtp_gemm_nt(C.byref(g), _s()), "mtp_gemm_nt")
    return out


def gemm_nt_tile(a, w, out, epi=EPI_BIAS, bias=None, bias_mod=0, res=None, res_mod=0, rowscale=None, rows_per_sample=0,
                 aux=None, variant=0, n=None):
    g = _nt_args(a, w, out, epi, bias, bias_mod, res, res_mod, rowscale, rows_per_sample, aux, variant, n)
    rc = lib().mtp_gemm_nt_tile(C.byref(g))
    if rc < 0:
        check(rc, "mtp_gemm_nt_tile")
    return rc


def gemm_nt_plan(a, w, out, epi=EPI_BIAS, bias=None, bias_mod=0, res=None, res_mod=0, rowscale=None, rows_per_sample=0,
                 aux=None, variant=0, n=None, cus=0):
    g = _nt_args(a, w, out, epi, bias, bias_mod, res, res_mod, rowscale, rows_per_sample, aux, variant, n)
    plan = _lib.GemmNtPlan()
    check(lib().mtp_gemm_nt_plan(C.byref(g), cus, C.byref(plan)), "mtp_gemm_nt_plan")
    return plan


def pick_split_k(M, N, K):
    tiles = ((M + 127) // 128) * ((N + 127) // 128)
    split = max(1, min(16, round(512 / tiles)))
    if split > 1 and split % 2:
        split += 1
    return max(1, min(split, K // 1024))


def effective_split_k(K, dtype, split):
    k_tiles = -(-K // (64 if dtype == torch.bfloat16 else 32))
    split = max(1, min(int(split), k_tiles))
    per = -(-k_tiles // split)
    return -(-k_tiles // per)


def gemm_tn(a, b, out, split_k=None, use_workspace=True, variant=0, colsum=None, defer=None, m=None):
    K, M = a.shape
    lda = M
    if m is not None:
        assert m <= M
        M = m
    N = b.shape[1]
    assert b.shape[0] == K and out.dtype == torch.float32 and out.numel() == M * N and a.dtype == b.dtype
    g = GemmArgs()
    if colsum is not None:
        assert colsum.dtype == torch.float32 and colsum.numel() == M and colsum.is_contiguous()
        g.colsum = _p(colsum)
    g.A, g.B, g.C = _p(a), _p(b), _p(out)
    g.M, g.N, g.K = M, N, K
    g.lda, g.ldb, g.ldc = lda, N, N
    g.in_dtype, g.out_dtype, g.epilogue = _dt(a), MTP_F32, EPI_BIAS
    g.split_k = effective_split_k(K, a.dtype, pick_split_k(M, N, K) if split_k is None else split_k)
    g.variant = variant
    if g.split_k > 1 and use_workspace:
        ws = _scratch((g.split_k * M * N,), out.device, torch.float32)
        g.aux = _p(ws)
        if defer is not None:
            g.defer_sum = 1
            defer.append((ws, out, M * N, g.split_k))
    check(lib().mtp_gemm_tn(C.byref(g), _s()), "mtp_gemm_tn")
    return out


MAX_GROUPED = 32


def grouped_tiles(M, N):
    return -(-M // 256) * -(-N // 256) if M % 8 == 0 and N % 8 == 0 and M >= 8 and N >= 8 else 0


def grouped_splits(K, tiles):
    if K < 16384:
        return 1
    return max(1, min(64, K // 4096, 256 // tiles))


_low_streams = {}


def low_priority_stream(device):
    device = torch.device(device)
    idx = device.index if device.index is not None else torch.cuda.current_device()
    st = _low_streams.get(idx)
    if st is None:
        h = C.c_void_p()
        with torch.cuda.device(idx):
            check(lib().mtp_stream_create_low_priority(C.byref(h)), "mtp_stream_create_low_priority")
        st = _low_streams[idx] = torch.cuda.ExternalStream(h.value, device=torch.device("cuda", idx))
    return st


_mask_streams = {}


def cu_mask_words(kind, part, parts=2, cus_per_xcc=32, xccs=8):
    words = [0] * (cus_per_xcc * xccs // 32)
    for i in range(cus_per_xcc * xccs):
        j = i // xccs
        mine = (j % parts == part) if kind == "interleaved" else (j * parts // cus_per_xcc == part)
        if mine:
            words[i // 32] |= 1 << (i % 32)
    return words


def cu_mask_stream(device, words):
    device = torch.device(device)
    idx = device.index if device.index is not None else torch.cuda.current_device()
    key = (idx, tuple(words))
    st = _mask_streams.get(key)
    if st is None:
        h = C.c_void_p()
        arr = (C.c_uint32 * len(words))(*words)
        with torch.cuda.device(idx):
            check(lib().mtp_stream_create_cu_mask(arr, len(words), C.byref(h)), "mtp_stream_create_cu_mask")
        st = _mask_streams[key] = torch.cuda.ExternalStream(h.value, device=torch.device("cuda", idx))
    return st


class WgradQueue:

    def __init__(self, cus=256, variant=0, stream=None):
        self.jobs, self.tiles, self.cus, self.variant = [], 0, cus, variant
        self.stream, self.inflight = stream, []
        self.max_jobs = 0
        self.launched = 0
        self.after = []
        self.sqn, self.covered = None, []

    def add(self, dy, x, dw, colsum=None, after=None, norm_of=None, norm_ok=True):
        K, M = dy.shape
        N = x.shape[1]
        t = grouped_tiles(M, N)
        fits = (K * M * 2 < (1 << 32) and K * N * 2 < (1 << 32) and dy.data_ptr() % 16 == 0 and x.data_ptr() % 16 == 0 and dw.data_ptr() % 16 == 0
                and dy.is_contiguous() and x.is_contiguous())
        if t == 0 or K % 128 or dy.dtype != torch.bfloat16 or x.dtype != torch.bfloat16 or not fits:
            gemm_tn(dy, x, dw, colsum=colsum)
            if after is not None:
                after()
            return False
        assert x.shape[0] == K and dw.dtype == torch.float32 and dw.numel() == M * N and dw.is_contiguous()
        splits = grouped_splits(K, t)
        part = _scratch((splits, M, N), dw.device, torch.float32) if splits > 1 else None
        use_sqn = self.sqn is not None and splits == 1 and norm_ok
        self.jobs.append((dy, x, dw, colsum, splits, part, use_sqn))
        if use_sqn:
            self.covered.append(dw if norm_of is None else norm_of)
        if after is not None:
            self.after.append(after)
        self.tiles += t * splits
        return True

    def should_flush(self, next_tiles=0, next_jobs=4):
        if not self.jobs:
            return False
        if len(self.jobs) + next_jobs > MAX_GROUPED or (self.max_jobs and len(self.jobs) >= self.max_jobs):
            return True
        rounds = -(-self.tiles // self.cus)
        return self.tiles / (rounds * self.cus) >= 0.93

    def flush(self):
        if self.stream is None or not self.jobs:
            return self._launch()
        ready = torch.cuda.Event()
        ready.record()
        held = list(self.jobs)
        with torch.cuda.stream(self.stream):
            self.stream.wait_event(ready)
            self._launch()
            done = torch.cuda.Event()
            done.record()
        self.inflight.append((done, held))
        self.launched += 1

    def wait(self, keep=0):
        while len(self.inflight) > keep:
            done, _ = self.inflight.pop(0)
            torch.cuda.current_stream().wait_event(done)

    def _launch(self):
        while self.jobs:
            chunk, self.jobs = self.jobs[:MAX_GROUPED], self.jobs[MAX_GROUPED:]
            arr = (GemmArgs * len(chunk))()
            for g, (dy, x, dw, cs, splits, part, use_sqn) in zip(arr, chunk):
                K, M = dy.shape
                N = x.shape[1]
                g.A, g.B, g.C = _p(dy), _p(x), _p(dw)
                g.M, g.N, g.K = M, N, K
                g.lda, g.ldb, g.ldc = M, N, N
                g.in_dtype, g.out_dtype, g.variant = MTP_BF16, MTP_F32, self.variant
                if splits > 1:
                    g.split_k, g.aux = splits, _p(part)
                if use_sqn:
                    g.workspace, g.workspace_bytes = _p(self.sqn), 4
                if cs is not None:
                    assert cs.dtype == torch.float32 and cs.numel() == M and cs.is_contiguous()
                    g.colsum = _p(cs)
            check(lib().mtp_gemm_tn_grouped(arr, len(chunk), _s()), "mtp_gemm_tn_grouped")
        after, self.after = self.after, []
        for fn in after:
            fn()
        self.tiles = 0


def sum_partials(jobs):
    while jobs:
        chunk, jobs[:] = jobs[:12], jobs[12:]
        n = len(chunk)
        P = C.c_void_p * n
        parts, outs = P(*[j[0].data_ptr() for j in chunk]), P(*[j[1].data_ptr() for j in chunk])
        numel, splits = (C.c_int64 * n)(*[j[2] for j in chunk]), (C.c_int * n)(*[j[3] for j in chunk])
        check(lib().mtp_sum_partials_batch(parts, outs, numel, splits, n, _s()), "mtp_sum_partials_batch")


def layernorm_fwd(x, gamma, beta, y, mean=None, rstd=None, eps=1e-6, gelu=False):
    rows, Cc = x.shape
    check(lib().mtp_layernorm_fwd(_p(x), _dt(x), _f32(gamma), _f32(beta), _p(y), _dt(y), _f32(mean), _f32(rstd),
                                  rows, Cc, eps, int(gelu), _s()), "mtp_layernorm_fwd")
    return y


def layernorm_bwd(dy, x, mean, rstd, gamma, dx, dgamma, dbeta, beta=None, gelu=False, dres=None, extra=None,
                  dx_copy=None, copy_scale=None, rows_per_sample=0, accumulate=False, defer=None, win_add=None, grid=None):
    rows, Cc = x.shape
    nblk = lib().mtp_layernorm_bwd_partial_rows(rows)
    part = _scratch((nblk, 2 * Cc), x.device, torch.float32)
    if win_add is not None:
        B, Hp, Wp = grid
        nh, nw = rvsa_windows(Hp, Wp)
        assert not gelu and tuple(win_add.shape) == (B * nh * nw, Cc) and B * Hp * Wp == rows
        check(lib().mtp_layernorm_bwd_win(_p(dy), _dt(dy), _p(x), _dt(x), _f32(mean), _f32(rstd), _f32(gamma), _f32(dres), _f32(extra), _p(dx), _dt(dx),
                                          _p(dx_copy), (_dt(dx_copy) if dx_copy is not None else 0), _f32(copy_scale), rows_per_sample,
                                          part.data_ptr(), part.data_ptr() + 4 * Cc, 2 * Cc, rows, Cc, _f32(win_add), B, Hp, Wp, _s()), "mtp_layernorm_bwd_win")
    else:
        check(lib().mtp_layernorm_bwd(_p(dy), _dt(dy), _p(x), _dt(x), _f32(mean), _f32(rstd), _f32(gamma), _f32(beta), int(gelu),
                                      _f32(dres), _f32(extra), _p(dx), _dt(dx), _p(dx_copy), (_dt(dx_copy) if dx_copy is not None else 0),
                                      _f32(copy_scale), rows_per_sample, part.data_ptr(), part.data_ptr() + 4 * Cc, 2 * Cc, rows, Cc, _s()),
              "mtp_layernorm_bwd")
    if defer is not None and _adjacent(dgamma, dbeta) and dgamma.numel() == Cc:
        defer.append((part, dgamma, accumulate))
    else:
        _reduce_pair(part, Cc, dgamma, dbeta, accumulate)
    return dx


def layernorm_residual_fwd(h, gamma, beta, x, layer_scale, out, out_act, mean, rstd, sample_scale=None, rows_per_sample=0, eps=1e-6):
    rows, Cc = h.shape
    check(lib().mtp_layernorm_residual_fwd(_p(h), _dt(h), _f32(gamma), _f32(beta), _f32(x), _f32(layer_scale), _f32(sample_scale), rows_per_sample,
                                           _f32(out), _p(out_act), _f32(mean), _f32(rstd), rows, Cc, eps, _s()), "mtp_layernorm_residual_fwd")
    return out


def layernorm_residual_bwd(dout, h, mean, rstd, gamma, beta, layer_scale, dh, dgamma, dbeta, dls, sample_scale=None, rows_per_sample=0, defer=None):
    rows, Cc = h.shape
    nblk = lib().mtp_layernorm_bwd_partial_rows(rows)
    part = _scratch((nblk, 3 * Cc), h.device, torch.float32)
    check(lib().mtp_layernorm_residual_bwd(_f32(dout), _p(h), _dt(h), _f32(mean), _f32(rstd), _f32(gamma), _f32(beta), _f32(layer_scale), _f32(sample_scale),
                                           rows_per_sample, _p(dh), part.data_ptr(), rows, Cc, _s()), "mtp_layernorm_residual_bwd")
    pair = _adjacent(dgamma, dbeta) and dgamma.numel() == Cc
    if defer is not None and pair:
        defer.append((part[:, :2 * Cc], dgamma, True))
        defer.append((part[:, 2 * Cc:], dls, True))
    else:
        _reduce_pair(part[:, :2 * Cc], Cc, dgamma, dbeta, True)
        reduce_rows(part[:, 2 * Cc:], dls, True)
    return dh


REDUCE_BATCH_MAX = 32


def reduce_rows_deferred(items):
    groups = {}
    for it in items:
        part, out, acc = it[:3]
        tr = it[3] if len(it) > 3 else None
        groups.setdefault((tuple(part.shape), part.stride(0), bool(acc), tr), []).append((part, out))
    for ((rows, cols), ld, acc, tr), g in groups.items():
        for i0 in range(0, len(g), REDUCE_BATCH_MAX):
            chunk = g[i0:i0 + REDUCE_BATCH_MAX]
            n = len(chunk)
            P = C.c_void_p * n
            if tr is None:
                check(lib().mtp_reduce_rows_batched_f32(P(*[c[0].data_ptr() for c in chunk]), P(*[c[1].data_ptr() for c in chunk]), n, ld, rows, cols,
                                                        int(acc), _s()), "mtp_reduce_rows_batched_f32")
            else:
                check(lib().mtp_reduce_rows_t_batched_f32(P(*[c[0].data_ptr() for c in chunk]), P(*[c[1].data_ptr() for c in chunk]), n, ld, rows, tr[0], tr[1],
                                                          int(acc), _s()), "mtp_reduce_rows_t_batched_f32")
    del items[:]


def reduce_rows(part, out, accumulate=False):
    if not part.is_cuda:
        raise RuntimeError("mtp_amd ops run only on an MI355X device tensor (no CPU fallback)")
    assert part.dim() == 2 and part.stride(1) == 1 and part.dtype == torch.float32
    rows, cols = part.shape
    assert out.numel() == cols
    check(lib().mtp_reduce_rows_f32(part.data_ptr(), part.stride(0), _f32(out), rows, cols, int(accumulate), _s()), "mtp_reduce_rows_f32")
    return out


def _adjacent(a, b):
    return (a.is_contiguous() and b.is_contiguous() and b.data_ptr() == a.data_ptr() + 4 * a.numel()
            and a.untyped_storage().data_ptr() == b.untyped_storage().data_ptr())
# ... 897 lines not shown
```

Baseline: 1886 images/sec.

## Run RVSA sampling fwd/bwd as rider workgroups on idle CUs of P8 GEMM

Adds a rider mode to the P8 NT GEMM kernel. Extra workgroups beyond the GEMM tiles run the RVSA window pooling and sampling-head computation in the forward pass, and the sampling backward in the backward pass, alongside the qkv GEMM and its transpose GEMM. This uses CUs the GEMM leaves idle and removes a separate kernel launch and its serialization. The sampling code is moved into a shared device header so both paths use it. When the plan does not fit the rider constraints, it falls back to running the GEMM and then the separate kernels in sequence.

Measured after the change: 1911 images/sec (median of 6 runs). 1.01x the previous value.

```diff
diff --git a/include/mtp_hip.h b/include/mtp_hip.h
--- a/include/mtp_hip.h
+++ b/include/mtp_hip.h
@@ -96,6 +96,24 @@
 int mtp_gemm_nt_plan(const mtp_gemm_args* args, int cus, struct mtp_gemm_nt_plan* out);
 int mtp_gemm_nt_tile(const mtp_gemm_args* args);
 int64_t mtp_gemm_nt_workspace_bytes(void);
+enum { MTP_NT_RIDER_NONE = 0, MTP_NT_RIDER_SAMPLING_FWD = 1, MTP_NT_RIDER_SAMPLING_BWD_WIN = 2 };
+struct mtp_nt_rider {
+    int kind;
+    int act_dtype;
+    const void* x;
+    const float* dsamp;
+    const float* w;
+    const float* bias;
+    float* avg;
+    float* pooled;
+    float* samp;
+    float* g;
+    int64_t B, Hp, Wp;
+    int64_t windows;
+    int64_t C, N;
+};
+int mtp_gemm_nt_rider(const mtp_gemm_args* args, const struct mtp_nt_rider* rider, mtp_stream_t stream);
+int mtp_nt_p8_gemm_wgs(int ntiles, int cus);
 int mtp_gemm_tn(const mtp_gemm_args* args, mtp_stream_t stream);
 #define MTP_MAX_GROUPED_GEMMS 32
 int mtp_gemm_tn_grouped(const mtp_gemm_args* args, int count, mtp_stream_t stream);
diff --git a/mtp_amd/__init__.py b/mtp_amd/__init__.py
--- a/mtp_amd/__init__.py
+++ b/mtp_amd/__init__.py
@@ -43,4 +43,4 @@
 from .ops_box import batched_nms, bbox_overlaps, box_iou_rotated, nms, nms_rotated
 from .task_modules import AssignResult, BboxOverlaps2D, MTP_RD_MaxIoUAssigner, MaxIoUAssigner, RBbox2HBboxOverlaps2D, RBboxOverlaps2D
 
-__version__ = "0.6.0"
+__version__ = "0.6.1"
diff --git a/mtp_amd/_lib.py b/mtp_amd/_lib.py
--- a/mtp_amd/_lib.py
+++ b/mtp_amd/_lib.py
@@ -44,6 +44,14 @@
 
 class GemmNtPlan(C.Structure):
     _fields_ = [("family", i32), ("tile_m", i32), ("order", i32), ("persistent", i32), ("store_policy", i32)]
+
+
+NT_RIDER_NONE, NT_RIDER_SAMPLING_FWD, NT_RIDER_SAMPLING_BWD_WIN = 0, 1, 2
+
+
+class NtRider(C.Structure):
+    _fields_ = [("kind", i32), ("act_dtype", i32), ("x", p), ("dsamp", p), ("w", p), ("bias", p), ("avg", p), ("pooled", p), ("samp", p), ("g", p),
+                ("B", i64), ("Hp", i64), ("Wp", i64), ("windows", i64), ("C", i64), ("N", i64)]
 
 
 class WimgDesc(C.Structure):
@@ -73,6 +81,8 @@
     "mtp_gemm_nt_plan": (i32, [C.POINTER(GemmArgs), i32, C.POINTER(GemmNtPlan)]),
     "mtp_gemm_nt_tile": (i32, [C.POINTER(GemmArgs)]),
     "mtp_gemm_nt_workspace_bytes": (i64, []),
+    "mtp_gemm_nt_rider": (i32, [C.POINTER(GemmArgs), C.POINTER(NtRider), p]),
+    "mtp_nt_p8_gemm_wgs": (i32, [i32, i32]),
     "mtp_gemm_tn": (i32, [C.POINTER(GemmArgs), p]),
     "mtp_gemm_tn_grouped": (i32, [C.POINTER(GemmArgs), i32, p]),
     "mtp_sum_partials_batch": (i32, [p, p, p, p, i32, p]),
diff --git a/mtp_amd/csrc/gemm.hip b/mtp_amd/csrc/gemm.hip
--- a/mtp_amd/csrc/gemm.hip
+++ b/mtp_amd/csrc/gemm.hip
@@ -646,6 +646,41 @@
     return MTP_ERR_UNSUPPORTED;
 }
 
+extern "C" int mtp_gemm_nt_rider(const mtp_gemm_args* a, const struct mtp_nt_rider* r, mtp_stream_t stream) {
+    if (!a || !r) return MTP_ERR_ARG;
+    P8Rider k8{};
+    if (r->kind == MTP_NT_RIDER_SAMPLING_FWD) {
+        if (!r->x || !r->w || !r->avg || !r->pooled || !r->samp || r->B <= 0 || r->Hp <= 0 || r->Wp <= 0 || r->C <= 0 || (r->C % 4) || r->C > 8192 || r->N <= 0) return MTP_ERR_ARG;
+        if (r->act_dtype != MTP_BF16) return MTP_ERR_UNSUPPORTED;
+        const RvsaWindows win(r->Hp, r->Wp);
+        if (r->B * win.nh * win.nw > INT32_MAX || r->N > INT32_MAX) return MTP_ERR_ARG;
+        k8.windows = (int)(r->B * win.nh * win.nw);
+        k8.Hp = (int)r->Hp; k8.Wp = (int)r->Wp; k8.pad_t = win.pad_t; k8.pad_l = win.pad_l; k8.nh = win.nh; k8.nw = win.nw;
+    } else if (r->kind == MTP_NT_RIDER_SAMPLING_BWD_WIN) {
+        if (!r->dsamp || !r->w || !r->avg || !r->g || r->windows <= 0 || r->windows > INT32_MAX || r->C <= 0 || (r->C % 4) || r->C > INT32_MAX || r->N <= 0 || r->N > 4096) return MTP_ERR_ARG;
+        k8.windows = (int)r->windows;
+    } else if (r->kind != MTP_NT_RIDER_NONE) {
+        return MTP_ERR_ARG;
+    }
+    k8.C = (int)r->C; k8.N = (int)r->N;
+    k8.x = r->x; k8.dsamp = r->dsamp; k8.w = r->w; k8.bias = r->bias; k8.avg = r->avg; k8.pooled = r->pooled; k8.samp = r->samp; k8.g = r->g;
+    hipStream_t s = (hipStream_t)stream;
+    if (a->in_dtype == MTP_BF16 && a->out_dtype == MTP_BF16 && a->epilogue == MTP_EPI_BIAS) {
+        KArgs k;
+        if (const int rc = fill_common<bf16_t>(a, k)) return rc;
+        if ((a->K % Elem<bf16_t>::kPerChunk) || (a->bias && a->bias_mod > 0 && (a->bias_mod % 4))) return MTP_ERR_ARG;
+        const NtPlan plan = nt_plan(a, k, mtp_stream_cus(s));
+        if (plan.family == MTP_GEMM_NT_FAMILY_P8) {
+            const int rc = mtp_nt_p8_launch_rider(k, a->out_dtype, a->epilogue, plan, r->kind, k8, s);
+            if (rc != MTP_ERR_UNSUPPORTED) return rc;
+        }
+    }
+    if (const int rc = mtp_gemm_nt(a, stream)) return rc;
+    if (r->kind == MTP_NT_RIDER_SAMPLING_FWD) return mtp_rvsa_sampling_fwd(r->x, r->act_dtype, r->w, r->bias, r->avg, r->pooled, r->samp, r->B, r->Hp, r->Wp, r->C, r->N, stream);
+    if (r->kind == MTP_NT_RIDER_SAMPLING_BWD_WIN) return mtp_rvsa_sampling_bwd_win(r->dsamp, r->w, r->avg, r->g, r->windows, r->C, r->N, stream);
+    return 0;
+}
+
 extern "C" int64_t mtp_gemm_nt_workspace_bytes(void) { return 0; }
 
 extern "C" int mtp_gemm_nt_plan(const mtp_gemm_args* a, int cus, struct mtp_gemm_nt_plan* out) {
diff --git a/mtp_amd/csrc/gemm_common.h b/mtp_amd/csrc/gemm_common.h
--- a/mtp_amd/csrc/gemm_common.h
+++ b/mtp_amd/csrc/gemm_common.h
@@ -25,12 +25,27 @@
     float* colsum;
 };
 
+struct P8Rider {
+    int gemm_wgs, riders;
+    int windows;
+    int Hp, Wp, C, N, pad_t, pad_l, nh, nw;
+    const void* x;
+    const float* dsamp;
+    const float* w;
+    const float* bias;
+    float* avg;
+    float* pooled;
+    float* samp;
+    float* g;
+};
+
 typedef struct mtp_gemm_nt_plan NtPlan;
 
 int mtp_nt_p8_launch(const KArgs& k, int out_dtype, int epilogue, const NtPlan& plan, hipStream_t stream);
 int mtp_nt_p8_fits(const KArgs& k, int out_dtype, int epilogue);
 int mtp_nt_p8_tiles(int64_t M, int64_t N, int tile_m);
 int mtp_nt_p8_pick_tile_m(int64_t M, int64_t N, int64_t cus);
+int mtp_nt_p8_launch_rider(const KArgs& k, int out_dtype, int epilogue, const NtPlan& plan, int kind, const P8Rider& rider, hipStream_t stream);
 int mtp_nt_s8_launch(const KArgs& k, int out_dtype, int epilogue, int order, hipStream_t stream);
 int mtp_nt_s8_fits(const KArgs& k, int out_dtype, int epilogue);
 int mtp_nt_s8_store_policy(int out_dtype);
diff --git a/mtp_amd/csrc/gemm_p8.hip b/mtp_amd/csrc/gemm_p8.hip
--- a/mtp_amd/csrc/gemm_p8.hip
+++ b/mtp_amd/csrc/gemm_p8.hip
@@ -1,4 +1,5 @@
 #include "gemm_p8.h"
+#include "rvsa_sampling_body.h"
 
 namespace {
 
@@ -97,9 +98,50 @@
     c.voffA += 128; c.voffB += 128;
 }
 
-template <typename Tout, int EPI, int MI1, int XP, int PS, int SP = 0>
-__global__ __launch_bounds__(P8_THREADS) __attribute__((amdgpu_waves_per_eu(2, 2))) void gemm_nt_p8_kernel(KArgs p) {
+constexpr int P8_RIDER_ROWS = 4;
+template <int KIND>
+__device__ __forceinline__ void p8_rider_run(const P8Rider& r, int rider, char* smem) {
+    const int half = __builtin_amdgcn_readfirstlane((int)threadIdx.x >> 8), tid = (int)threadIdx.x & 255;
+    const int per = (r.windows + r.riders - 1) / r.riders;
+    if constexpr (KIND == 1) {
+        float* pl = reinterpret_cast<float*>(smem);
+        for (int s0 = 0; s0 < per; s0 += 2) {
+            const int item = rider + (s0 + half) * r.riders;
+            const bool live = s0 + half < per && item < r.windows;
+            rvsa_pool_window<bf16_t, 4>((const bf16_t*)r.x, r.avg, r.pooled, r.Hp, r.Wp, r.C, r.pad_t, r.pad_l, r.nh, r.nw, live ? item : r.windows - 1, live, tid,
+                                        pl + (int64_t)(s0 + half) * r.C);
+        }
+        __syncthreads();
+        for (int g0 = 0; g0 < per; g0 += P8_RIDER_ROWS)
+            rvsa_heads<P8_RIDER_ROWS>(r.w, r.bias, r.samp, r.C, r.N, 0, r.N, (int)threadIdx.x >> 6, 8, (int)threadIdx.x & 63, pl + (int64_t)g0 * r.C,
+                                      rider + g0 * r.riders, r.riders, r.windows);
+    } else {
+        char* mine = smem + half * (4096 + ((r.N * 4 + 15) & ~15));
+        for (int it = 0; it < (per + 1) / 2; ++it) {
+            const int item = rider + (2 * it + half) * r.riders;
+            const bool live = item < r.windows;
+            for (int c4base = 0; c4base < r.C / 4; c4base += 64)
+                rvsa_sampling_bwd_win_body(r.dsamp, r.w, r.avg, r.g, r.C, r.N, live ? item : r.windows - 1, c4base, live, tid, reinterpret_cast<float*>(mine + 4096),
+                                           reinterpret_cast<float4*>(mine));
+        }
+    }
+}
+
+struct P8RiderKArgs : KArgs {
+    P8Rider rider;
+};
+template <int RK> struct P8KArgs { typedef P8RiderKArgs type; };
+template <> struct P8KArgs<0> { typedef KArgs type; };
+
+template <typename Tout, int EPI, int MI1, int XP, int PS, int SP = 0, int RK = 0>
+__global__ __launch_bounds__(P8_THREADS) __attribute__((amdgpu_waves_per_eu(2, 2))) void gemm_nt_p8_kernel(typename P8KArgs<RK>::type p) {
     extern __shared__ __attribute__((aligned(16))) char smem[];
+    if constexpr (RK != 0) {
+        if ((int)blockIdx.x >= p.rider.gemm_wgs) {
+            p8_rider_run<RK>(p.rider, (int)blockIdx.x - p.rider.gemm_wgs, smem);
+            return;
+        }
+    }
     constexpr int WROWS = 64 + 16 * MI1, BM = 2 * WROWS;
     const int tid = threadIdx.x, lane = tid & 63;
     const int wave = __builtin_amdgcn_readfirstlane(tid >> 6);
@@ -163,7 +205,8 @@
 
         if constexpr (PS) {
             const int em0 = m0, en0 = n0;
-            tile += gridDim.x;
+            if constexpr (RK != 0) tile += p.rider.gemm_wgs;
+            else tile += gridDim.x;
             const bool more = tile < ntiles;
             if (more) {
                 tile_coords(plain ? tile : xcd_remap(tile, ntiles), tiles_m, tiles_n, plain, tm, tn);
@@ -201,6 +244,18 @@
     return mtp_launch_status();
 }
 
+template <int PS, int RK>
+int launch_p8_rider_kernel(const KArgs& k, const P8Rider& r, hipStream_t stream) {
+    constexpr int LDS = P8_LDS + 8 * 4096;
+    static unsigned long long optin = 0;
+    if (const int e = mtp_optin_lds((const void*)gemm_nt_p8_kernel<bf16_t, MTP_EPI_BIAS, 3, 0, PS, 1, RK>, LDS, optin)) return e;
+    P8RiderKArgs a;
+    static_cast<KArgs&>(a) = k;
+    a.rider = r;
+    hipLaunchKernelGGL((gemm_nt_p8_kernel<bf16_t, MTP_EPI_BIAS, 3, 0, PS, 1, RK>), dim3(r.gemm_wgs + r.riders), dim3(P8_THREADS), LDS, stream, a);
+    return mtp_launch_status();
+}
+
 template <typename Tout, int EPI>
 int launch_p8(const KArgs& k, const NtPlan& plan, hipStream_t stream) {
     const int bm = plan.tile_m, sp = plan.store_policy;
@@ -251,6 +306,36 @@
     return c224 < c256 ? 224 : 256;
 }
 
+extern "C" int mtp_nt_p8_gemm_wgs(int ntiles, int cus) {
+    if (ntiles <= 0 || cus <= 0) return MTP_ERR_ARG;
+    const int rounds = (ntiles + cus - 1) / cus;
+    return (ntiles + rounds - 1) / rounds;
+}
+
+int mtp_nt_p8_launch_rider(const KArgs& k, int out_dtype, int epi, const NtPlan& plan, int kind, const P8Rider& rider, hipStream_t stream) {
+    if (!mtp_nt_p8_fits(k, out_dtype, epi) || out_dtype != MTP_BF16 || epi != MTP_EPI_BIAS || plan.tile_m != 224 || plan.store_policy != 1) return MTP_ERR_UNSUPPORTED;
+    if ((kind == MTP_NT_RIDER_SAMPLING_BWD_WIN) == (plan.persistent != 0)) return MTP_ERR_UNSUPPORTED;
+    KArgs a = k;
+    a.tiles_n = (k.N + P8_BN - 1) / P8_BN;
+    a.k_tiles = k.K / 64;
+    a.order = plan.order;
+    a.atomic_out = 0;
+    const int ntiles = mtp_nt_p8_tiles(k.M, k.N, 224), cus = mtp_stream_cus(stream);
+    if (!plan.persistent && ntiles > cus) return MTP_ERR_UNSUPPORTED;
+    P8Rider r = rider;
+    r.gemm_wgs = plan.persistent ? mtp_nt_p8_gemm_wgs(ntiles, cus) : ntiles;
+    const int spare = cus - r.gemm_wgs;
+    r.riders = kind == MTP_NT_RIDER_NONE ? 0 : (spare < 32 ? spare : 32) < r.windows ? (spare < 32 ? spare : 32) : r.windows;
+    if (kind != MTP_NT_RIDER_NONE) {
+        if (r.riders <= 0) return MTP_ERR_UNSUPPORTED;
+        const int64_t rows = ((r.windows + r.riders - 1) / r.riders + P8_RIDER_ROWS - 1) / P8_RIDER_ROWS * P8_RIDER_ROWS;
+        const int64_t scratch = kind == MTP_NT_RIDER_SAMPLING_FWD ? rows * 4 * (int64_t)r.C : 2 * (4096 + (((int64_t)r.N * 4 + 15) & ~15ll));
+        if (scratch > P8_LDS + 8 * 4096) return MTP_ERR_UNSUPPORTED;
+    }
+    if (kind == MTP_NT_RIDER_SAMPLING_BWD_WIN) return launch_p8_rider_kernel<0, 2>(a, r, stream);
+    return launch_p8_rider_kernel<1, 1>(a, r, stream);
+}
+
 int mtp_nt_p8_launch(const KArgs& k, int out_dtype, int epi, const NtPlan& plan, hipStream_t stream) {
     if (!mtp_nt_p8_fits(k, out_dtype, epi)) return MTP_ERR_UNSUPPORTED;
     if (epi == MTP_EPI_BIAS_RES) return launch_p8<float, MTP_EPI_BIAS_RES>(k, plan, stream);
diff --git a/mtp_amd/csrc/runtime.hip b/mtp_amd/csrc/runtime.hip
--- a/mtp_amd/csrc/runtime.hip
+++ b/mtp_amd/csrc/runtime.hip
@@ -2,7 +2,7 @@
 #include <atomic>
 #include <mutex>
 
-extern "C" const char* mtp_version(void) { return "mtp_hip 0.6 (gfx950)"; }
+extern "C" const char* mtp_version(void) { return "mtp_hip 0.6.1 (gfx950)"; }
 
 extern "C" int mtp_stream_create_low_priority(void** stream) {
     if (!stream) return MTP_ERR_ARG;
diff --git a/mtp_amd/csrc/rvsa_sampling.hip b/mtp_amd/csrc/rvsa_sampling.hip
--- a/mtp_amd/csrc/rvsa_sampling.hip
+++ b/mtp_amd/csrc/rvsa_sampling.hip
@@ -1,4 +1,5 @@
 #include "common.h"
+#include "rvsa_sampling_body.h"
 
 namespace {
 
@@ -228,65 +229,10 @@
                                                                float* __restrict__ avg, float* __restrict__ pooled, float* __restrict__ samp,
                                                                int Hp, int Wp, int C, int N, int pad_t, int pad_l, int nh, int nw) {
     extern __shared__ __attribute__((aligned(16))) float pl[];
-    const int win = blockIdx.x, lane = threadIdx.x & 63, wave = threadIdx.x >> 6;
-    const int j = win % nw, i = (win / nw) % nh, b = win / (nw * nh);
-    for (int c4 = threadIdx.x; c4 < C / 4; c4 += 256) {
-        float4 s = make_float4(0, 0, 0, 0);
-#pragma unroll
-        for (int a = 0; a < 7; ++a) {
-            const int y = i * 7 + a - pad_t;
-            const bool yok = y >= 0 && y < Hp;
-            const int yc = yok ? y : 0;
-            float4 v[7];
-#pragma unroll
-            for (int bb = 0; bb < 7; ++bb) {
-                const int xx = j * 7 + bb - pad_l;
-                const int xc = (xx >= 0 && xx < Wp) ? xx : 0;
-                v[bb] = load4(x + (((int64_t)b * Hp + yc) * Wp + xc) * C + 4 * c4);
-            }
-#pragma unroll
-            for (int bb = 0; bb < 7; ++bb) {
-                const int xx = j * 7 + bb - pad_l;
-                const float m = (yok && xx >= 0 && xx < Wp) ? 1.f : 0.f;
-                s.x += m * v[bb].x; s.y += m * v[bb].y; s.z += m * v[bb].z; s.w += m * v[bb].w;
-            }
-        }
-        const float inv = 1.0f / 49.0f;
-        s = make_float4(s.x * inv, s.y * inv, s.z * inv, s.w * inv);
-        const float4 p = make_float4(s.x > 0 ? s.x : 0.01f * s.x, s.y > 0 ? s.y : 0.01f * s.y, s.z > 0 ? s.z : 0.01f * s.z, s.w > 0 ? s.w : 0.01f * s.w);
-        if (blockIdx.y == 0) {
-            store4(avg + (int64_t)win * C + 4 * c4, s);
-            store4(pooled + (int64_t)win * C + 4 * c4, p);
-        }
-        *reinterpret_cast<float4*>(pl + 4 * c4) = p;
-    }
+    const int nper = ((N + (int)gridDim.y - 1) / (int)gridDim.y + 3) / 4 * 4, nlo = (int)blockIdx.y * nper, nhi = (nlo + nper) < N ? (nlo + nper) : N;
+    rvsa_pool_window<T>(x, avg, pooled, Hp, Wp, C, pad_t, pad_l, nh, nw, (int)blockIdx.x, blockIdx.y == 0, (int)threadIdx.x, pl);
     __syncthreads();
-    const int nper = ((N + (int)gridDim.y - 1) / (int)gridDim.y + 3) / 4 * 4, nlo = (int)blockIdx.y * nper, nhi = (nlo + nper) < N ? (nlo + nper) : N;
-    for (int n0 = nlo + 4 * wave; n0 < nhi; n0 += 16) {
-        float acc[4] = {0.f, 0.f, 0.f, 0.f};
-        for (int k0 = lane * 4; k0 < C; k0 += 1024) {
-            float4 ww[4][4], a[4];
-#pragma unroll
-            for (int kk = 0; kk < 4; ++kk) {
-                const int k = k0 + 256 * kk, kc = k < C ? k : 0;
-                a[kk] = k < C ? *reinterpret_cast<const float4*>(pl + kc) : make_float4(0.f, 0.f, 0.f, 0.f);
-#pragma unroll
-                for (int q = 0; q < 4; ++q) {
-                    const int n = n0 + q < N ? n0 + q : N - 1;
-                    ww[kk][q] = load4(w + (int64_t)n * C + kc);
-                }
-            }
-#pragma unroll
-            for (int kk = 0; kk < 4; ++kk)
-#pragma unroll
-                for (int q = 0; q < 4; ++q) acc[q] += a[kk].x * ww[kk][q].x + a[kk].y * ww[kk][q].y + a[kk].z * ww[kk][q].z + a[kk].w * ww[kk][q].w;
-        }
-#pragma unroll
-        for (int q = 0; q < 4; ++q) {
-            const float t = wave_sum(acc[q]);
-            if (lane == 0 && n0 + q < nhi) samp[(int64_t)win * N + n0 + q] = t + (bias ? bias[n0 + q] : 0.f);
-        }
-    }
+    rvsa_heads<1>(w, bias, samp, C, N, nlo, nhi, (int)threadIdx.x >> 6, 4, (int)threadIdx.x & 63, pl, (int)blockIdx.x, 0, (int)gridDim.x);
 }
 
 template <typename T>
@@ -342,32 +288,8 @@
 __global__ __launch_bounds__(256) void rvsa_sampling_bwd_win_kernel(const float* __restrict__ dsamp, const float* __restrict__ w, const float* __restrict__ avg,
                                                                    float* __restrict__ g, int C, int N) {
     extern __shared__ __attribute__((aligned(16))) float ds[];
-    __shared__ float4 part[4][64];
-    const int win = blockIdx.x;
-    const int lane = threadIdx.x & 63, q = threadIdx.x >> 6;
-    const int c4 = blockIdx.y * 64 + lane;
-    const bool live = c4 < C / 4;
-    for (int n = threadIdx.x; n < N; n += 256) ds[n] = dsamp[(int64_t)win * N + n];
-    __syncthreads();
-    const int nq = (N + 3) / 4, n0 = q * nq, n1 = (n0 + nq) < N ? (n0 + nq) : N;
-    float4 d = make_float4(0, 0, 0, 0);
-    if (live) {
-#pragma unroll 10
-        for (int n = n0; n < n1; ++n) {
-            const float4 ww = load4(w + (int64_t)n * C + 4 * c4);
-            const float t = ds[n];
-            d.x += t * ww.x; d.y += t * ww.y; d.z += t * ww.z; d.w += t * ww.w;
-        }
-    }
-    part[q][lane] = d;
-    __syncthreads();
-    if (!live || q) return;
-    const float4 p0 = part[0][lane], p1 = part[1][lane], p2 = part[2][lane], p3 = part[3][lane];
-    d = make_float4((p0.x + p1.x) + (p2.x + p3.x), (p0.y + p1.y) + (p2.y + p3.y), (p0.z + p1.z) + (p2.z + p3.z), (p0.w + p1.w) + (p2.w + p3.w));
-    const float4 a = load4(avg + (int64_t)win * C + 4 * c4);
-    const float k = 1.0f / 49.0f;
-    *reinterpret_cast<float4*>(g + (int64_t)win * C + 4 * c4) =
-        make_float4(d.x * (a.x > 0 ? k : 0.01f * k), d.y * (a.y > 0 ? k : 0.01f * k), d.z * (a.z > 0 ? k : 0.01f * k), d.w * (a.w > 0 ? k : 0.01f * k));
+    __shared__ float4 part[4 * 64];
+    rvsa_sampling_bwd_win_body(dsamp, w, avg, g, C, N, (int)blockIdx.x, (int)blockIdx.y * 64, true, (int)threadIdx.x, ds, part);
 }
 
 extern "C" int mtp_rvsa_sampling_bwd_win(const float* dsamp, const float* w, const float* avg, float* g, int64_t windows, int64_t C, int64_t N, mtp_stream_t stream) {
diff --git a/mtp_amd/csrc/rvsa_sampling_body.h b/mtp_amd/csrc/rvsa_sampling_body.h
--- /dev/null
+++ b/mtp_amd/csrc/rvsa_sampling_body.h
@@ -0,0 +1,126 @@
+#pragma once
+#include "common.h"
+
+namespace {
+
+template <typename T, int RB = 7>
+__device__ __forceinline__ void rvsa_pool_window(const T* __restrict__ x, float* __restrict__ avg, float* __restrict__ pooled, int Hp, int Wp, int C,
+                                                 int pad_t, int pad_l, int nh, int nw, int win, bool store, int tid, float* __restrict__ pl) {
+    const int j = win % nw, i = (win / nw) % nh, b = win / (nw * nh);
+    for (int c4 = tid; c4 < C / 4; c4 += 256) {
+        float4 s = make_float4(0, 0, 0, 0);
+#pragma unroll
+        for (int a = 0; a < 7; ++a) {
+            if (RB < 7 && a == RB) __builtin_amdgcn_sched_barrier(0);
+            const int y = i * 7 + a - pad_t;
+            const bool yok = y >= 0 && y < Hp;
+            const int yc = yok ? y : 0;
+            float4 v[7];
+#pragma unroll
+            for (int bb = 0; bb < 7; ++bb) {
+                const int xx = j * 7 + bb - pad_l;
+                const int xc = (xx >= 0 && xx < Wp) ? xx : 0;
+                v[bb] = load4(x + (((int64_t)b * Hp + yc) * Wp + xc) * C + 4 * c4);
+            }
+#pragma unroll
+            for (int bb = 0; bb < 7; ++bb) {
+                const int xx = j * 7 + bb - pad_l;
+                const float m = (yok && xx >= 0 && xx < Wp) ? 1.f : 0.f;
+                s.x += m * v[bb].x; s.y += m * v[bb].y; s.z += m * v[bb].z; s.w += m * v[bb].w;
+            }
+        }
+        const float inv = 1.0f / 49.0f;
+        s = make_float4(s.x * inv, s.y * inv, s.z * inv, s.w * inv);
+        const float4 p = make_float4(s.x > 0 ? s.x : 0.01f * s.x, s.y > 0 ? s.y : 0.01f * s.y, s.z > 0 ? s.z : 0.01f * s.z, s.w > 0 ? s.w : 0.01f * s.w);
+        if (store) {
+            store4(avg + (int64_t)win * C + 4 * c4, s);
+            store4(pooled + (int64_t)win * C + 4 * c4, p);
+        }
+        *reinterpret_cast<float4*>(pl + 4 * c4) = p;
+    }
+}
+
+template <int W>
+__device__ __forceinline__ void rvsa_heads(const float* __restrict__ w, const float* __restrict__ bias, float* __restrict__ samp, int C, int N, int nlo, int nhi,
+                                           int wave, int nwaves, int lane, const float* __restrict__ pl, int win0, int wstep, int windows) {
+#pragma clang fp contract(off)
+    for (int n0 = nlo + 4 * wave; n0 < nhi; n0 += 4 * nwaves) {
+        float acc[W][4];
+#pragma unroll
+        for (int i = 0; i < W; ++i)
+#pragma unroll
+            for (int q = 0; q < 4; ++q) acc[i][q] = 0.f;
+        for (int k0 = lane * 4; k0 < C; k0 += 1024) {
+            float4 ww[4][4];
+#pragma unroll
+            for (int kk = 0; kk < 4; ++kk) {
+                const int k = k0 + 256 * kk, kc = k < C ? k : 0;
+#pragma unroll
+                for (int q = 0; q < 4; ++q) {
+                    const int n = n0 + q < N ? n0 + q : N - 1;
+                    ww[kk][q] = load4(w + (int64_t)n * C + kc);
+                }
+            }
+#pragma unroll
+            for (int i = 0; i < W; ++i) {
+                if (W > 1) __builtin_amdgcn_sched_barrier(0);
+                float4 a[4];
+#pragma unroll
+                for (int kk = 0; kk < 4; ++kk) {
+                    const int k = k0 + 256 * kk, kc = k < C ? k : 0;
+                    a[kk] = k < C ? *reinterpret_cast<const float4*>(pl + (int64_t)i * C + kc) : make_float4(0.f, 0.f, 0.f, 0.f);
+                }
+#pragma unroll
+                for (int kk = 0; kk < 4; ++kk)
+#pragma unroll
+                    for (int q = 0; q < 4; ++q) {
+                        float t = (q & 1) ? a[kk].y * ww[kk][q].y : a[kk].x * ww[kk][q].x;
+                        t = (q & 1) ? fmaf(a[kk].x, ww[kk][q].x, t) : fmaf(a[kk].y, ww[kk][q].y, t);
+                        t = fmaf(a[kk].z, ww[kk][q].z, t);
+                        t = fmaf(a[kk].w, ww[kk][q].w, t);
+                        acc[i][q] += t;
+                    }
+            }
+        }
+#pragma unroll
+        for (int i = 0; i < W; ++i) {
+            const int win = win0 + i * wstep;
+#pragma unroll
+            for (int q = 0; q < 4; ++q) {
+                const float t = wave_sum(acc[i][q]);
+                if (lane == 0 && win < windows && n0 + q < nhi) samp[(int64_t)win * N + n0 + q] = t + (bias ? bias[n0 + q] : 0.f);
+            }
+        }
+    }
+}
+
+__device__ __forceinline__ void rvsa_sampling_bwd_win_body(const float* __restrict__ dsamp, const float* __restrict__ w, const float* __restrict__ avg,
+                                                           float* __restrict__ g, int C, int N, int win, int c4base, bool live_win, int tid,
+                                                           float* __restrict__ ds, float4* __restrict__ part) {
+    const int lane = tid & 63, q = tid >> 6;
+    const int c4 = c4base + lane;
+    const bool live = c4 < C / 4;
+    for (int n = tid; n < N; n += 256) ds[n] = dsamp[(int64_t)win * N + n];
+    __syncthreads();
+    const int nq = (N + 3) / 4, n0 = q * nq, n1 = (n0 + nq) < N ? (n0 + nq) : N;
+    float4 d = make_float4(0, 0, 0, 0);
+    if (live) {
+#pragma unroll 10
+        for (int n = n0; n < n1; ++n) {
+            const float4 ww = load4(w + (int64_t)n * C + 4 * c4);
+            const float t = ds[n];
+            d.x += t * ww.x; d.y += t * ww.y; d.z += t * ww.z; d.w += t * ww.w;
+        }
+    }
+    part[q * 64 + lane] = d;
+    __syncthreads();
+    if (!live || q || !live_win) return;
+    const float4 p0 = part[lane], p1 = part[64 + lane], p2 = part[128 + lane], p3 = part[192 + lane];
+    d = make_float4((p0.x + p1.x) + (p2.x + p3.x), (p0.y + p1.y) + (p2.y + p3.y), (p0.z + p1.z) + (p2.z + p3.z), (p0.w + p1.w) + (p2.w + p3.w));
+    const float4 a = load4(avg + (int64_t)win * C + 4 * c4);
+    const float k = 1.0f / 49.0f;
+    *reinterpret_cast<float4*>(g + (int64_t)win * C + 4 * c4) =
+        make_float4(d.x * (a.x > 0 ? k : 0.01f * k), d.y * (a.y > 0 ? k : 0.01f * k), d.z * (a.z > 0 ? k : 0.01f * k), d.w * (a.w > 0 ? k : 0.01f * k));
+}
+
+}
diff --git a/mtp_amd/engine.py b/mtp_amd/engine.py
--- a/mtp_amd/engine.py
+++ b/mtp_amd/engine.py
@@ -131,18 +131,27 @@
         s = torch.floor(keep + torch.rand(self.depth, 2, B, device=self.dev, dtype=F32)) / keep
         return [(s[i, 0], s[i, 1]) if live[i] else (None, None) for i in range(self.depth)]
 
+    @property
+    def _ride(self):
+        return self.act == torch.bfloat16 and not self.m.use_checkpoint
+
     def _block_fwd(self, i, x, B, Hp, Wp, dps, save):
         P, b, C, T, N = self.P, self._blk[i], self.C, x.shape[0], Hp * Wp
         pre = b.pre
         s = {}
         mean1, rstd1 = self._e(T, dtype=F32), self._e(T, dtype=F32)
         ln1 = ops.layernorm_fwd(x, P[pre + "norm1.weight"], P[pre + "norm1.bias"], self._e(T, C), mean1, rstd1)
+        rider = None
         if b.window:
             nh, nw = ops.rvsa_windows(Hp, Wp)
             R = B * nh * nw
             avg, pooled = self._e(R, C, dtype=F32), self._e(R, C, dtype=F32)
-            samp = ops.rvsa_sampling_fwd(ln1, b.wsamp, b.bsamp, avg, pooled, self._e(R, 5 * self.heads, dtype=F32), B, Hp, Wp)
-        qkv = ops.gemm_nt(ln1, b.wqkv, self._e(T, 3 * C), bias=P[pre + "attn.qkv.bias"])
+            samp = self._e(R, 5 * self.heads, dtype=F32)
+            if self._ride:
+                rider = ops.sampling_fwd_rider(ln1, b.wsamp, b.bsamp, avg, pooled, samp, B, Hp, Wp)
+            else:
+                ops.rvsa_sampling_fwd(ln1, b.wsamp, b.bsamp, avg, pooled, samp, B, Hp, Wp)
+        qkv = ops.gemm_nt(ln1, b.wqkv, self._e(T, 3 * C), bias=P[pre + "attn.qkv.bias"], rider=rider)
         o = self._e(T, C)
         if b.window:
             lse = self._e(R * self.heads * 49, dtype=F32)
@@ -212,10 +221,14 @@
             ops.full_attn_bwd(s["qkv"], s["o"], do, s["lse"], dqkv, rel_h, rel_w, drel_h, drel_w, B, Hp, Wp, self.heads, self.scale,
                               accumulate=True, defer=self._ln_parts)
         wq.add(dqkv, s["ln1"], G[pre + "attn.qkv.weight"], G[pre + "attn.qkv.bias"])
-        win_add = None
+        win_add = rider = None
         if b.window:
-            win_add = ops.rvsa_sampling_bwd_win(dsamp, b.wsamp, s["avg"], self._e(*s["avg"].shape, dtype=F32))
-        dln1 = ops.gemm_nt(dqkv, b.wqkvT, self._e(T, C))
+            win_add = self._e(*s["avg"].shape, dtype=F32)
+            if self._ride:
+                rider = ops.sampling_bwd_win_rider(dsamp, b.wsamp, s["avg"], win_add)
+            else:
+                ops.rvsa_sampling_bwd_win(dsamp, b.wsamp, s["avg"], win_add)
+        dln1 = ops.gemm_nt(dqkv, b.wqkvT, self._e(T, C), rider=rider)
         dx0, dx0_act = self._e(T, C, dtype=F32), self._e(T, C)
         self._ln_bwd(dln1, s["x"], s["mean1"], s["rstd1"], P[pre + "norm1.weight"], dx0, G[pre + "norm1.weight"], G[pre + "norm1.bias"],
                           dres=dx1, extra=extra, dx_copy=dx0_act, copy_scale=prev_scale, rows_per_sample=N,
diff --git a/mtp_amd/ops.py b/mtp_amd/ops.py
--- a/mtp_amd/ops.py
+++ b/mtp_amd/ops.py
@@ -69,10 +69,25 @@
     return g
 
 
+def sampling_fwd_rider(x, w, b, avg, pooled, samp, B, Hp, Wp):
+    r = _lib.NtRider(kind=_lib.NT_RIDER_SAMPLING_FWD, act_dtype=_dt(x), x=_p(x), w=_f32(w), bias=_f32(b), avg=_f32(avg), pooled=_f32(pooled), samp=_f32(samp),
+                     B=B, Hp=Hp, Wp=Wp, C=x.shape[-1], N=w.shape[0])
+    return r
+
+
+def sampling_bwd_win_rider(dsamp, w, avg, g):
+    r = _lib.NtRider(kind=_lib.NT_RIDER_SAMPLING_BWD_WIN, act_dtype=MTP_BF16, dsamp=_f32(dsamp), w=_f32(w), avg=_f32(avg), g=_f32(g),
+                     windows=avg.shape[0], C=avg.shape[1], N=w.shape[0])
+    return r
+
+
 def gemm_nt(a, w, out, epi=EPI_BIAS, bias=None, bias_mod=0, res=None, res_mod=0, rowscale=None, rows_per_sample=0,
-            aux=None, variant=0, n=None):
+            aux=None, variant=0, n=None, rider=None):
     g = _nt_args(a, w, out, epi, bias, bias_mod, res, res_mod, rowscale, rows_per_sample, aux, variant, n)
-    check(lib().mtp_gemm_nt(C.byref(g), _s()), "mtp_gemm_nt")
+    if rider is not None:
+        check(lib().mtp_gemm_nt_rider(C.byref(g), C.byref(rider), _s()), "mtp_gemm_nt_rider")
+    else:
+        check(lib().mtp_gemm_nt(C.byref(g), _s()), "mtp_gemm_nt")
     return out
 
 
```
